# chemprop/chemprop

Hardware: AMD Instinct MI355X
Metric: million directed-edge-updates/sec (depth=3, hidden=300) (higher is better)
Workload: dtype f32 (exact 3-term f16 split of fp32 operands, fp32 accumulate); 1 GPU; qm9-shaped synthetic molecules, 512 mols/GPU/step, BondMessagePassing depth=3 hidden=300, forward (plan K0 + K1..K5); mols_per_gpu=512, directed_edges_per_gpu=9120, parallelism=dp1 (molecule shards, no data-path collective), launch=eager

## Files before the change

### chemprop_amd/_lib.py

```python
from __future__ import annotations

import ctypes as C
import os
import shutil
import subprocess
from typing import Optional

_HERE = os.path.dirname(os.path.abspath(__file__))
_ROOT = os.path.dirname(_HERE)
CSRC = os.path.join(_HERE, "csrc")
INCLUDE = os.path.join(_ROOT, "include")
LIB_PATH = os.environ.get("DMPNN_LIB") or os.path.join(_HERE, "libdmpnn_gfx950.so")
SOURCES = ["dmpnn_abi.hip", "dmpnn_prepare.hip", "dmpnn_segment.hip", "dmpnn_gemm.hip", "dmpnn_gemm_p1.hip",
           "dmpnn_gemm_p2.hip", "dmpnn_gemm_p3.hip", "dmpnn_gemm_p4.hip", "dmpnn_gemm_s1.hip", "dmpnn_mega.hip", "dmpnn_mega16.hip", "dmpnn_mega16_lp.hip", "dmpnn_mega16_bwd.hip", "dmpnn_rows16.hip", "dmpnn_step16.hip", "dmpnn_bstep16.hip", "dmpnn_backward.hip", "dmpnn_molagg.hip", "dmpnn_collate.hip", "dmpnn_tiles_large.hip", "dmpnn_optim.hip", "dmpnn_wgrad16.hip", "dmpnn_head.hip", "dmpnn_vd.hip"]
HEADERS = ["dmpnn_common.hpp", "dmpnn_spill_impl.hpp", "dmpnn_gemm_impl.hpp", "dmpnn_mega_impl.hpp", "dmpnn_mega16_impl.hpp", "dmpnn_mega16_bwd_impl.hpp", "dmpnn_rows16_impl.hpp", "dmpnn_seg16.hpp", "dmpnn_step16_impl.hpp"]
ABI_VERSION = 15
PLAN_NOFFSETS = 15

EXPORTS = [
    "dmpnn_version", "dmpnn_debug_timestamps", "dmpnn_last_error_string", "dmpnn_last_launch_count", "dmpnn_plan_bytes",
    "dmpnn_plan_layout", "dmpnn_prepare", "dmpnn_prepare_light", "dmpnn_prepare_tiles", "dmpnn_message_fwd", "dmpnn_aggregate_fwd",
    "dmpnn_linear_fwd", "dmpnn_linear16_wsplit_bytes", "dmpnn_linear16_ok", "dmpnn_linear16_fwd", "dmpnn_update_fwd", "dmpnn_forward", "dmpnn_forward_can_fuse", "dmpnn_forward_wsplit_bytes", "dmpnn_forward_keep_bits_bytes", "dmpnn_forward_spill_bytes", "dmpnn_backward_ws_bytes", "dmpnn_backward", "dmpnn_message_bwd",
    "dmpnn_aggregate_bwd", "dmpnn_linear_wgrad_ws_bytes", "dmpnn_linear_wgrad",
    "dmpnn_molagg_ws_bytes", "dmpnn_molagg_bounds", "dmpnn_molagg_fwd", "dmpnn_molagg_bwd", "dmpnn_gather_rows", "dmpnn_collate", "dmpnn_pack_tiles", "dmpnn_max_tiles",
    "dmpnn_prepare_tiles_from_table", "dmpnn_prepare_with_batch", "dmpnn_tile_plan_any_size", "dmpnn_split_row_floats", "dmpnn_forward_can_fuse16", "dmpnn_adam_step",
    "dmpnn_full_plan_keeps_tiles", "dmpnn_head_ws_bytes", "dmpnn_head", "dmpnn_train_step", "dmpnn_forward_tiles", "dmpnn_forward_route", "dmpnn_dropout_keep",
    "dmpnn_clip_grad", "dmpnn_clip_grad_ws_bytes", "dmpnn_train_route", "dmpnn_forward_h0_bytes", "dmpnn_tile_waves", "dmpnn_debug_lds_poison",
    "dmpnn_vd_ws_bytes", "dmpnn_vd_forward", "dmpnn_vd_backward",
]

ACT = {"none": 0, "relu": 1, "leakyrelu": 2, "prelu": 3, "tanh": 4, "elu": 5}
F_UNDIRECTED = 1
F_FUSED = 2
F_MEGA = 4
F_KEEP = 8
F_SPLIT16 = 16
F_WSPLIT_READY = 32
F_LOADER_TILES = 64
F_STORE16 = 128
F_ATOM = 1024
F_TILE_PLAN = 2048
F_H0_RESIDUAL = 256
F_ROW_FINALIZE = 512
ROUTES = ("general", "general16", "fused", "fused16", "mega", "mega16")
PLAN_NOMEGA_MASK = 15
PLAN_NOFUSE_MASK = 7


class GemmArgs(C.Structure):
    _fields_ = [
        ("M", C.c_int64), ("N", C.c_int64), ("K1", C.c_int64), ("K2", C.c_int64),
        ("A1", C.c_void_p), ("lda1", C.c_int64), ("gather1", C.c_void_p), ("gather1_rows", C.c_int64),
        ("A2", C.c_void_p), ("lda2", C.c_int64),
        ("W", C.c_void_p), ("ldw", C.c_int64),
        ("bias", C.c_void_p),
        ("Cadd", C.c_void_p), ("ldcadd", C.c_int64),
        ("C", C.c_void_p), ("ldc", C.c_int64),
        ("Zpre", C.c_void_p), ("ldz", C.c_int64),
        ("act", C.c_int), ("act_slope", C.c_float), ("act_slope_ptr", C.c_void_p),
    ]


class FwdArgs(C.Structure):
    _fields_ = [
        ("plan", C.c_void_p), ("n_atoms", C.c_int64), ("n_edges", C.c_int64),
        ("d_v", C.c_int64), ("d_e", C.c_int64), ("d_h", C.c_int64), ("d_vd", C.c_int64),
        ("depth", C.c_int32), ("flags", C.c_uint32),
        ("act", C.c_int32), ("act_slope", C.c_float), ("act_slope_ptr", C.c_void_p),
        ("V", C.c_void_p), ("ldv", C.c_int64),
        ("E", C.c_void_p), ("lde", C.c_int64),
        ("V_d", C.c_void_p), ("ldvd", C.c_int64),
        ("W_i", C.c_void_p), ("b_i", C.c_void_p),
        ("W_h", C.c_void_p), ("b_h", C.c_void_p),
        ("W_o", C.c_void_p), ("b_o", C.c_void_p),
        ("W_d", C.c_void_p), ("b_d", C.c_void_p),
        ("ldh", C.c_int64), ("H0", C.c_void_p), ("Hs", C.c_void_p), ("n_hslots", C.c_int32),
        ("Ms", C.c_void_p), ("n_mslots", C.c_int32),
        ("Mv", C.c_void_p), ("Hv", C.c_void_p),
        ("out", C.c_void_p), ("ldout", C.c_int64),
        ("wsplit", C.c_void_p), ("wsplit_bytes", C.c_size_t),
        ("edge_index", C.c_void_p), ("rev_edge_index", C.c_void_p),
        ("n_tiles_launch", C.c_int64),
        ("spill_ws", C.c_void_p), ("spill_bytes", C.c_size_t),
        ("msplit", C.c_void_p), ("msplit_bytes", C.c_size_t),
        ("dropout_p", C.c_float), ("dropout_seed", C.c_uint64),
        ("keep_bits", C.c_void_p), ("keep_bits_bytes", C.c_size_t),
        ("h0_bytes", C.c_size_t),
    ]


class BwdArgs(C.Structure):
    _fields_ = [
        ("f", FwdArgs), ("gout", C.c_void_p), ("ldgout", C.c_int64),
        ("gW_i", C.c_void_p), ("gb_i", C.c_void_p), ("gW_h", C.c_void_p), ("gb_h", C.c_void_p),
        ("gW_o", C.c_void_p), ("gb_o", C.c_void_p), ("gW_d", C.c_void_p), ("gb_d", C.c_void_p),
        ("ws", C.c_void_p), ("ws_bytes", C.c_size_t),
        ("g_edge", C.c_void_p), ("ld_gedge", C.c_int64),
    ]


MAX_FFN_LAYERS = 8
MAX_COMPONENTS = 8
DROP_SITE_FFN = 0x10000
LOSS = {"mse": 0, "mae": 1, "bce": 2, "ce": 3, "mve": 4, "evidential": 5, "quantile": 6}
STEP_FORWARD, STEP_BACKWARD, STEP_UPDATE = 1, 2, 4


class HeadArgs(C.Structure):
    _fields_ = [
        ("n_atoms", C.c_int64), ("n_mols", C.c_int64), ("d_h", C.c_int64),
        ("batch", C.c_void_p),
        ("agg_mode", C.c_int32), ("agg_norm", C.c_float),
        ("bn_weight", C.c_void_p), ("bn_bias", C.c_void_p), ("bn_running_mean", C.c_void_p), ("bn_running_var", C.c_void_p),
        ("bn_eps", C.c_float), ("bn_momentum", C.c_float), ("bn_training", C.c_int32),
        ("n_layers", C.c_int32), ("act", C.c_int32), ("act_slope", C.c_float),
        ("W", C.c_void_p * MAX_FFN_LAYERS), ("b", C.c_void_p * MAX_FFN_LAYERS), ("dims", C.c_int64 * (MAX_FFN_LAYERS + 1)),
        ("loss", C.c_int32),
        ("targets", C.c_void_p), ("weights", C.c_void_p), ("task_weights", C.c_void_p), ("lt_mask", C.c_void_p), ("gt_mask", C.c_void_p),
        ("preds", C.c_void_p), ("loss_out", C.c_void_p),
        ("gW", C.c_void_p * MAX_FFN_LAYERS), ("gb", C.c_void_p * MAX_FFN_LAYERS), ("g_bn_weight", C.c_void_p), ("g_bn_bias", C.c_void_p),
        ("gHv", C.c_void_p), ("ldg", C.c_int64),
        ("ws", C.c_void_p), ("ws_bytes", C.c_size_t),
        ("bn_num_batches_tracked", C.c_void_p),
        ("n_classes", C.c_int32),
        ("evid_v_kl", C.c_float), ("evid_eps", C.c_float), ("quantile_alpha", C.c_float),
        ("X_d", C.c_void_p), ("ld_xd", C.c_int64),
        ("n_components", C.c_int32),
        ("ffn_dropout_p", C.c_float), ("ffn_dropout_seed", C.c_uint64),
    ]


class TrainRouteInfo(C.Structure):
    _fields_ = [("plan_kind", C.c_int32), ("route", C.c_int32), ("keep_rows", C.c_int32), ("keep_bits", C.c_int32), ("lean", C.c_int32)]


class StepComponent(C.Structure):
    _fields_ = [
        ("edge_index", C.c_void_p), ("rev_edge_index", C.c_void_p), ("batch", C.c_void_p), ("plan_bytes", C.c_size_t), ("plan_ready", C.c_int32),
        ("bwd", BwdArgs),
    ]


class VdArgs(C.Structure):
    _fields_ = [
        ("n_atoms", C.c_int64), ("d_h", C.c_int64), ("d_vd", C.c_int64),
        ("Hv", C.c_void_p), ("ldhv", C.c_int64),
        ("V_d", C.c_void_p), ("ldvd", C.c_int64),
        ("W_d", C.c_void_p), ("b_d", C.c_void_p),
        ("out", C.c_void_p), ("ldout", C.c_int64),
        ("gout", C.c_void_p), ("ldgout", C.c_int64),
        ("gHv", C.c_void_p), ("ldghv", C.c_int64),
        ("gW_d", C.c_void_p), ("gb_d", C.c_void_p),
        ("ws", C.c_void_p), ("ws_bytes", C.c_size_t),
    ]


VD_MAX_WIDTH = 544


class StepArgs(C.Structure):
    _fields_ = [
        ("edge_index", C.c_void_p), ("rev_edge_index", C.c_void_p), ("batch", C.c_void_p), ("plan_bytes", C.c_size_t), ("plan_ready", C.c_int32),
        ("stages", C.c_int32),
        ("bwd", BwdArgs), ("head", HeadArgs),
        ("p", C.c_void_p), ("g", C.c_void_p), ("m", C.c_void_p), ("v", C.c_void_p), ("n_params", C.c_int64),
        ("lr", C.c_float), ("beta1", C.c_float), ("beta2", C.c_float), ("eps", C.c_float), ("weight_decay", C.c_float),
        ("bias_corr1", C.c_float), ("sqrt_bias_corr2", C.c_float), ("grad_scale", C.c_float), ("dev_scalars", C.c_void_p),
        ("clip_val", C.c_float), ("clip_mode", C.c_int32), ("clip_ws", C.c_void_p),
        ("n_extra", C.c_int32), ("extra", C.POINTER(StepComponent)),
        ("vd", C.POINTER(VdArgs)),
    ]


def sources() -> list[str]:
    return [os.path.join(CSRC, s) for s in SOURCES if os.path.isfile(os.path.join(CSRC, s))]


def _stale() -> bool:
    if os.environ.get("DMPNN_LIB"):
        return False
    if not os.path.isfile(LIB_PATH):
        return True
    t = os.path.getmtime(LIB_PATH)
    deps = sources() + [os.path.join(CSRC, h) for h in HEADERS] + [os.path.join(INCLUDE, "dmpnn.h")]
    return any(os.path.getmtime(d) > t for d in deps if os.path.isfile(d))


def build(force: bool = False, verbose: bool = False, defines=(), out: Optional[str] = None) -> str:
    lib_path = out or LIB_PATH
    if not force and not _stale() and out is None:
        return LIB_PATH
    hipcc = shutil.which("hipcc") or "/opt/rocm/bin/hipcc"
    if not os.path.isfile(hipcc):
        raise RuntimeError("hipcc not found: cannot build libdmpnn_gfx950.so")
    import concurrent.futures as cf
    import tempfile

    flags = ["--offload-arch=gfx950", "-O3", "-std=c++17", "-fPIC", f"-I{INCLUDE}", f"-I{CSRC}", *[f"-D{d}" for d in defines]]
    with tempfile.TemporaryDirectory(prefix="dmpnn_build_") as tmp:
        def cc(src):
            obj = os.path.join(tmp, os.path.basename(src) + ".o")
            cmd = [hipcc, *flags, "-c", src, "-o", obj]
            if verbose:
                print(" ".join(cmd))
            r = subprocess.run(cmd, capture_output=True, text=True)
            if r.returncode != 0:
                raise RuntimeError(f"hipcc failed on {src} ({r.returncode}):\n{r.stdout}\n{r.stderr}")
            return obj

        with cf.ThreadPoolExecutor(max_workers=8) as ex:
            objs = list(ex.map(cc, sources()))
        linked = os.path.join(os.path.dirname(objs[0]), "libdmpnn.so")
        cmd = [hipcc, "--offload-arch=gfx950", "-shared", "-fPIC", *objs, "-o", linked]
        if verbose:
            print(" ".join(cmd))
        r = subprocess.run(cmd, capture_output=True, text=True)
        if r.returncode != 0:
            raise RuntimeError(f"hipcc link failed ({r.returncode}):\n{r.stdout}\n{r.stderr}")
        shutil.copyfile(linked, lib_path + ".tmp")
        os.chmod(lib_path + ".tmp", 0o755)
    os.replace(lib_path + ".tmp", lib_path)
    _clean_unbundle_temporaries(lib_path)
    return lib_path


def _clean_unbundle_temporaries(lib_path: str) -> int:
    import glob

    n = 0
    for f in glob.glob(glob.escape(lib_path) + ".*"):
        tail = f[len(lib_path) + 1:]
        if tail.split(".", 1)[0].isdigit() and ("hipv4-" in tail or "host-" in tail):
            try:
                os.remove(f)
                n += 1
            except OSError:
                pass
    return n


_lib: Optional[C.CDLL] = None


def load() -> C.CDLL:
    global _lib
    if _lib is not None:
        return _lib
    import torch

    if _stale() and (shutil.which("hipcc") or os.path.isfile("/opt/rocm/bin/hipcc")):
        build()
    if not os.path.isfile(LIB_PATH):
        raise RuntimeError(
            f"{LIB_PATH} is missing: run `python -c 'import __graft_entry__ as g; g.build()'` "
            "(the MI355X engine has no CPU / eager fallback)")
    lib = C.CDLL(LIB_PATH)
    lib.dmpnn_version.restype = C.c_int
    lib.dmpnn_last_error_string.restype = C.c_char_p
    lib.dmpnn_last_launch_count.restype = C.c_int
    lib.dmpnn_plan_bytes.restype = C.c_size_t
    lib.dmpnn_plan_bytes.argtypes = [C.c_int64, C.c_int64]
    lib.dmpnn_plan_layout.argtypes = [C.c_int64, C.c_int64, C.POINTER(C.c_int64)]
    lib.dmpnn_forward_can_fuse.argtypes = [C.POINTER(FwdArgs)]
    lib.dmpnn_prepare.argtypes = [C.c_void_p, C.c_void_p, C.c_int64, C.c_int64, C.c_void_p, C.c_size_t, C.c_void_p]
    lib.dmpnn_prepare_light.argtypes = lib.dmpnn_prepare.argtypes
    lib.dmpnn_prepare_tiles.argtypes = [C.c_void_p, C.c_void_p, C.c_void_p, C.c_int64, C.c_int64, C.c_void_p, C.c_size_t, C.c_void_p]
    lib.dmpnn_message_fwd.argtypes = [C.c_void_p, C.c_int64, C.c_int64, C.c_int64, C.c_void_p, C.c_int64,
                                      C.c_void_p, C.c_int64, C.c_int, C.c_float, C.c_void_p, C.c_uint, C.c_void_p]
    lib.dmpnn_aggregate_fwd.argtypes = [C.c_void_p, C.c_int64, C.c_int64, C.c_int64, C.c_void_p, C.c_int64,
                                        C.c_void_p, C.c_int64, C.c_int, C.c_float, C.c_void_p, C.c_void_p]
    lib.dmpnn_linear_fwd.argtypes = [C.POINTER(GemmArgs), C.c_void_p]
    lib.dmpnn_update_fwd.argtypes = [C.c_void_p, C.c_int64, C.c_int64, C.c_int64, C.c_void_p, C.c_int64, C.c_void_p, C.c_int64,
                                     C.c_void_p, C.c_void_p, C.c_void_p, C.c_int64, C.c_void_p, C.c_int64, C.c_void_p,
                                     C.c_int64, C.c_int, C.c_float, C.c_void_p, C.c_void_p]
    lib.dmpnn_forward.argtypes = [C.POINTER(FwdArgs), C.c_void_p]
    lib.dmpnn_backward_ws_bytes.argtypes = [C.POINTER(FwdArgs)]
    lib.dmpnn_backward.argtypes = [C.POINTER(BwdArgs), C.c_void_p]
    lib.dmpnn_message_bwd.argtypes = [C.c_void_p, C.c_int64, C.c_int64, C.c_int64, C.c_void_p, C.c_int64,
                                      C.c_void_p, C.c_int64, C.c_void_p]
    lib.dmpnn_aggregate_bwd.argtypes = lib.dmpnn_message_bwd.argtypes
    lib.dmpnn_linear_wgrad_ws_bytes.argtypes = [C.c_int64, C.c_int64, C.c_int64, C.c_int]
    lib.dmpnn_linear_wgrad.argtypes = [C.POINTER(GemmArgs), C.c_void_p, C.c_int64, C.c_void_p, C.c_int64,
                                       C.c_void_p, C.c_void_p, C.c_size_t, C.c_void_p]
    size_t_fns = ("dmpnn_plan_bytes", "dmpnn_backward_ws_bytes", "dmpnn_linear_wgrad_ws_bytes", "dmpnn_forward_wsplit_bytes", "dmpnn_forward_spill_bytes",
                  "dmpnn_forward_keep_bits_bytes",
                  "dmpnn_molagg_ws_bytes", "dmpnn_linear16_wsplit_bytes", "dmpnn_head_ws_bytes", "dmpnn_clip_grad_ws_bytes", "dmpnn_forward_h0_bytes", "dmpnn_vd_ws_bytes")
    lib.dmpnn_linear16_wsplit_bytes.argtypes = [C.c_int64, C.c_int64]
    lib.dmpnn_linear16_ok.argtypes = [C.POINTER(GemmArgs)]
    lib.dmpnn_linear16_fwd.argtypes = [C.POINTER(GemmArgs), C.c_void_p, C.c_size_t, C.c_int, C.c_void_p]
    lib.dmpnn_gather_rows.argtypes = [C.c_void_p, C.c_int64, C.c_int64, C.c_void_p, C.c_int64, C.c_int64, C.c_void_p, C.c_int64,
                                      C.c_void_p]
    lib.dmpnn_pack_tiles.argtypes = [C.c_void_p, C.c_void_p, C.c_int64, C.c_void_p, C.c_void_p, C.c_int64]
    lib.dmpnn_pack_tiles.restype = C.c_int64
    lib.dmpnn_max_tiles.argtypes = [C.c_int64, C.c_int64]
    lib.dmpnn_prepare_with_batch.argtypes = [C.c_void_p, C.c_void_p, C.c_void_p, C.c_int64, C.c_int64, C.c_void_p, C.c_size_t, C.c_void_p]
    lib.dmpnn_prepare_with_batch.restype = C.c_int
    lib.dmpnn_tile_plan_any_size.argtypes = [C.c_int64, C.c_int64]
    lib.dmpnn_max_tiles.restype = C.c_int64
    lib.dmpnn_prepare_tiles_from_table.argtypes = [C.c_void_p, C.c_void_p, C.c_int64, C.c_int64, C.c_int64, C.c_void_p, C.c_size_t,
                                                   C.c_void_p]
    lib.dmpnn_collate.argtypes = [C.c_void_p, C.c_void_p, C.c_int64, C.c_void_p, C.c_void_p, C.c_void_p, C.c_int64, C.c_int64,
                                  C.c_void_p, C.c_void_p, C.c_void_p, C.c_void_p]
    lib.dmpnn_molagg_ws_bytes.argtypes = [C.c_int64]
    lib.dmpnn_molagg_bounds.argtypes = [C.c_void_p, C.c_int64, C.c_int64, C.c_void_p, C.c_size_t, C.c_void_p]
    lib.dmpnn_molagg_fwd.argtypes = [C.c_void_p, C.c_int64, C.c_int64, C.c_int64, C.c_int64, C.c_void_p, C.c_int, C.c_float,
                                     C.c_void_p, C.c_int64, C.c_void_p]
    lib.dmpnn_molagg_bwd.argtypes = [C.c_void_p, C.c_int64, C.c_void_p, C.c_int64, C.c_int64, C.c_int64, C.c_void_p, C.c_int,
                                     C.c_float, C.c_void_p, C.c_int64, C.c_void_p]
    lib.dmpnn_forward_wsplit_bytes.argtypes = [C.POINTER(FwdArgs)]
    lib.dmpnn_forward_keep_bits_bytes.argtypes = [C.POINTER(FwdArgs)]
    lib.dmpnn_forward_spill_bytes.argtypes = [C.POINTER(FwdArgs)]
    lib.dmpnn_forward_h0_bytes.argtypes = [C.POINTER(FwdArgs)]
    lib.dmpnn_forward_can_fuse16.argtypes = [C.POINTER(FwdArgs)]
    lib.dmpnn_adam_step.argtypes = [C.c_void_p, C.c_void_p, C.c_void_p, C.c_void_p, C.c_int64, C.c_float, C.c_float, C.c_float, C.c_float,
                                    C.c_float, C.c_float, C.c_float, C.c_float, C.c_void_p, C.c_void_p]
    lib.dmpnn_train_route.argtypes = [C.POINTER(FwdArgs), C.c_int64, C.c_int32, C.c_int32, C.c_int32, C.c_int32, C.c_int32, C.POINTER(TrainRouteInfo)]
    lib.dmpnn_clip_grad.argtypes = [C.c_void_p, C.c_int64, C.c_float, C.c_int32, C.c_float, C.c_void_p, C.c_void_p]
    lib.dmpnn_dropout_keep.argtypes = [C.c_uint64, C.c_int32, C.c_int64, C.c_int64, C.c_float]
    lib.dmpnn_forward_route.argtypes = [C.POINTER(FwdArgs), C.c_int, C.c_int, C.c_int, C.c_int]
    lib.dmpnn_tile_waves.restype = C.c_int
    lib.dmpnn_tile_waves.argtypes = [C.c_int64, C.c_int64, C.c_int64, C.c_int64]
    lib.dmpnn_forward_tiles.argtypes = [C.POINTER(FwdArgs), C.c_void_p, C.c_void_p, C.c_void_p, C.c_int64, C.c_size_t, C.c_void_p]
    lib.dmpnn_full_plan_keeps_tiles.argtypes = [C.c_int64, C.c_int64]
    lib.dmpnn_head_ws_bytes.argtypes = [C.POINTER(HeadArgs)]
    lib.dmpnn_head.argtypes = [C.POINTER(HeadArgs), C.c_void_p, C.c_int64, C.c_void_p]
    lib.dmpnn_train_step.argtypes = [C.POINTER(StepArgs), C.c_void_p]
    lib.dmpnn_vd_ws_bytes.argtypes = [C.POINTER(VdArgs)]
    lib.dmpnn_vd_forward.argtypes = [C.POINTER(VdArgs), C.c_void_p]
    lib.dmpnn_vd_backward.argtypes = [C.POINTER(VdArgs), C.c_void_p]
    lib.dmpnn_split_row_floats.argtypes = [C.c_int64]
    lib.dmpnn_split_row_floats.restype = C.c_int64
    lib.dmpnn_debug_timestamps.argtypes = [C.c_void_p]
    for name in size_t_fns:
        getattr(lib, name).restype = C.c_size_t
    for name in EXPORTS:
        if name != "dmpnn_last_error_string" and name not in size_t_fns and name not in ("dmpnn_pack_tiles", "dmpnn_max_tiles", "dmpnn_split_row_floats"):
            getattr(lib, name).restype = C.c_int
    if lib.dmpnn_version() != ABI_VERSION:
        raise RuntimeError(f"libdmpnn ABI version {lib.dmpnn_version()} != {ABI_VERSION} (stale build?)")
    _lib = lib
    return lib


_ENV_DATA = getattr(os.environ, "_data", None)
_ENV_KEYS: dict = {}


def opt(name: str, default: str) -> str:
    if _ENV_DATA is None or os.name != "posix":
        return os.environ.get(name, default)
    k = _ENV_KEYS.get(name)
    if k is None:
        k = _ENV_KEYS[name] = name.encode()
    v = _ENV_DATA.get(k)
    return default if v is None else v.decode()


class DmpnnError(RuntimeError):
    pass


def check(rc: int, what: str) -> None:
    if rc != 0:
        msg = load().dmpnn_last_error_string().decode(errors="replace")
        raise DmpnnError(f"{what} failed (code {rc}): {msg}")
```

### chemprop_amd/csrc/dmpnn_abi.hip

```cpp
#include <stdarg.h>
#include <stdlib.h>
#include <string.h>

#include "dmpnn_common.hpp"
#include "dmpnn_mega16_impl.hpp"

namespace dmpnn {

static thread_local char g_err[512] = "";
static thread_local int g_launches = 0;

void set_error(const char* fmt, ...) {
    va_list ap;
    va_start(ap, fmt);
    vsnprintf(g_err, sizeof(g_err), fmt, ap);
    va_end(ap);
}
static __global__ __launch_bounds__(1024) void k_debug_lds_poison(unsigned pat, unsigned* sink) {
    extern __shared__ unsigned lds_words[];
    constexpr int n = (160 * 1024 - 64) / 4;
    for (int i = threadIdx.x; i < n; i += 1024) lds_words[i] = pat;
    __syncthreads();
    if (sink && lds_words[(threadIdx.x * 7) % n] == 0x12345u) sink[0] = 1;
}
static int g_lds_poison = -1;
static void debug_lds_poison() {
    if (g_lds_poison < 0) {
        const char* e = getenv("DMPNN_DEBUG_LDS_POISON");
        g_lds_poison = (e && e[0] == '1') ? 1 : 0;
    }
    if (!g_lds_poison) return;
    static const bool attr = hipFuncSetAttribute(reinterpret_cast<const void*>(&k_debug_lds_poison), hipFuncAttributeMaxDynamicSharedMemorySize, 160 * 1024 - 64) == hipSuccess;
    if (!attr) return;
    hipLaunchKernelGGL(k_debug_lds_poison, dim3(768), dim3(1024), 160 * 1024 - 64, static_cast<hipStream_t>(nullptr), 0x7FC07FC0u, static_cast<unsigned*>(nullptr));
    (void)hipGetLastError();
}
void count_launch(const char* name) {
    ++g_launches;
    debug_lds_poison();
    static const bool trace = [] {
        const char* e = getenv("DMPNN_TRACE");
        return e && e[0] == '1';
    }();
    if (trace) {
        fprintf(stderr, "[dmpnn] launch %d: %s ... ", g_launches, name);
        fflush(stderr);
        const hipError_t e = hipDeviceSynchronize();
        fprintf(stderr, "%s\n", e == hipSuccess ? "ok" : hipGetErrorString(e));
        fflush(stderr);
    }
}

static int check_graph_sizes(int64_t nV, int64_t nE) {
    DMPNN_CHECK_ARG(nV >= 0 && nE >= 0, "negative graph size (n_atoms=%lld n_edges=%lld)", (long long)nV, (long long)nE);
    DMPNN_CHECK_ARG(nV < (int64_t(1) << 31) - 64 && nE < (int64_t(1) << 31) - 64,
                    "graph too large for int32 indices (n_atoms=%lld n_edges=%lld)", (long long)nV, (long long)nE);
    return DMPNN_OK;
}

}

using namespace dmpnn;
namespace dmpnn { extern thread_local long long* g_debug_stamps; }

extern "C" {

int dmpnn_version(void) { return DMPNN_ABI_VERSION; }
void dmpnn_debug_lds_poison(int on) { dmpnn::g_lds_poison = on ? 1 : 0; }
int dmpnn_dropout_keep(uint64_t seed, int32_t site, int64_t row, int64_t col, float p) {
    if (!(p > 0.f && p < 1.f)) return p <= 0.f ? 1 : 0;
    return drop_hash((unsigned)(seed & 0xFFFFFFFFull), (unsigned)(seed >> 32), (unsigned)site, (unsigned)row, (unsigned)col) >= drop_threshold(p) ? 1 : 0;
}
int dmpnn_debug_timestamps(void* device_buf) {
    g_debug_stamps = static_cast<long long*>(device_buf);
    return DMPNN_OK;
}
const char* dmpnn_last_error_string(void) { return g_err; }
int dmpnn_last_launch_count(void) { return g_launches; }

size_t dmpnn_plan_bytes(int64_t n_atoms, int64_t n_edges) {
    if (n_atoms < 0 || n_edges < 0) return 0;
    return (size_t)plan_layout(n_atoms, n_edges).words * sizeof(int);
}

int dmpnn_plan_layout(int64_t n_atoms, int64_t n_edges, int64_t off[DMPNN_PLAN_NOFFSETS]) {
    DMPNN_CHECK_ARG(off != nullptr, "plan_layout: null output");
    DMPNN_TRY(check_graph_sizes(n_atoms, n_edges));
    const PlanLayout L = plan_layout(n_atoms, n_edges);
    off[0] = L.src; off[1] = L.dst; off[2] = L.rev; off[3] = L.row_ptr; off[4] = L.perm;
    off[5] = L.inv; off[6] = L.srcp; off[7] = L.dstp; off[8] = L.revp;
    off[9] = L.tile_row; off[10] = L.tile_atom; off[11] = L.max_tiles;
    off[12] = L.mtile_row; off[13] = L.mtile_atom; off[14] = L.max_mtiles;
    return DMPNN_OK;
}

static int prepare_impl(const int64_t* edge_index, const int64_t* rev, int64_t n_atoms, int64_t n_edges, void* plan,
                        size_t plan_bytes, int light, void* stream) {
    DMPNN_TRY(check_graph_sizes(n_atoms, n_edges));
    DMPNN_CHECK_ARG(plan != nullptr, "prepare: null plan");
    DMPNN_CHECK_ARG(n_edges == 0 || (edge_index && rev), "prepare: null index arrays");
    if (plan_bytes < dmpnn_plan_bytes(n_atoms, n_edges)) {
        set_error("prepare: plan buffer too small (%zu < %zu bytes)", plan_bytes, dmpnn_plan_bytes(n_atoms, n_edges));
        return DMPNN_ENOSPC;
    }
    DMPNN_CHECK_ARG(aligned16(plan), "prepare: plan must be 16-byte aligned");
    return launch_prepare(edge_index, rev, n_atoms, n_edges, static_cast<int*>(plan), light, static_cast<hipStream_t>(stream));
}
int dmpnn_prepare(const int64_t* edge_index, const int64_t* rev, int64_t n_atoms, int64_t n_edges, void* plan,
                  size_t plan_bytes, void* stream) {
    return prepare_impl(edge_index, rev, n_atoms, n_edges, plan, plan_bytes, 0, stream);
}
int dmpnn_prepare_light(const int64_t* edge_index, const int64_t* rev, int64_t n_atoms, int64_t n_edges, void* plan,
                        size_t plan_bytes, void* stream) {
    return prepare_impl(edge_index, rev, n_atoms, n_edges, plan, plan_bytes, 1, stream);
}

int dmpnn_prepare_tiles(const int64_t* edge_index, const int64_t* rev, const int64_t* batch, int64_t n_atoms, int64_t n_edges,
                        void* plan, size_t plan_bytes, void* stream) {
    if (batch && n_atoms > 0 && small_plan_fits(n_atoms, n_edges)) {
        DMPNN_TRY(check_graph_sizes(n_atoms, n_edges));
        DMPNN_CHECK_ARG(plan != nullptr && aligned16(plan), "prepare_tiles: plan must be a 16-byte aligned buffer");
        DMPNN_CHECK_ARG(n_edges == 0 || edge_index, "prepare_tiles: null edge_index");
        if (plan_bytes < dmpnn_plan_bytes(n_atoms, n_edges)) {
            set_error("prepare_tiles: plan buffer too small (%zu < %zu bytes)", plan_bytes, dmpnn_plan_bytes(n_atoms, n_edges));
            return DMPNN_ENOSPC;
        }
        return launch_prepare_tiles_batch(edge_index, batch, n_atoms, n_edges, static_cast<int*>(plan), static_cast<hipStream_t>(stream));
    }
    if (batch && dmpnn_tile_plan_any_size(n_atoms, n_edges) && !small_plan_fits(n_atoms, n_edges)) {
        DMPNN_TRY(check_graph_sizes(n_atoms, n_edges));
        DMPNN_CHECK_ARG(plan != nullptr && aligned16(plan), "prepare_tiles: plan must be a 16-byte aligned buffer");
        DMPNN_CHECK_ARG(n_edges == 0 || edge_index, "prepare_tiles: null edge_index");
        if (plan_bytes < dmpnn_plan_bytes(n_atoms, n_edges)) {
            set_error("prepare_tiles: plan buffer too small (%zu < %zu bytes)", plan_bytes, dmpnn_plan_bytes(n_atoms, n_edges));
            return DMPNN_ENOSPC;
        }
        return launch_prepare_tiles_large(edge_index, batch, n_atoms, n_edges, static_cast<int*>(plan), static_cast<hipStream_t>(stream));
    }
    return prepare_impl(edge_index, rev, n_atoms, n_edges, plan, plan_bytes, 2, stream);
}

}
namespace dmpnn {
int prepare_tiles_and_bounds(const int64_t* edge_index, const int64_t* rev, const int64_t* batch, int64_t n_atoms, int64_t n_edges, void* plan,
                             size_t plan_bytes, int* mol_bounds, int64_t n_mols, void* stream, bool* wrote_bounds,
                             const dmpnn_fwd_args* split_for, bool* did_split) {
    if (wrote_bounds) *wrote_bounds = false;
    if (did_split) *did_split = false;
    if (mol_bounds && (n_mols <= 0 || n_mols >= (1 << 30))) mol_bounds = nullptr;
    if ((mol_bounds || split_for) && batch && n_atoms > 0 && small_plan_fits(n_atoms, n_edges) && check_graph_sizes(n_atoms, n_edges) == DMPNN_OK &&
        plan != nullptr && aligned16(plan) && (n_edges == 0 || edge_index) && plan_bytes >= dmpnn_plan_bytes(n_atoms, n_edges)) {
        DMPNN_TRY(launch_prepare_tiles_batch(edge_index, batch, n_atoms, n_edges, static_cast<int*>(plan), static_cast<hipStream_t>(stream), mol_bounds,
                                             mol_bounds ? n_mols : 0, split_for, did_split));
        if (wrote_bounds) *wrote_bounds = mol_bounds != nullptr;
        return DMPNN_OK;
    }
    return dmpnn_prepare_tiles(edge_index, rev, batch, n_atoms, n_edges, plan, plan_bytes, stream);
}
}
extern "C" {

int dmpnn_tile_plan_any_size(int64_t n_atoms, int64_t n_edges) { return tiles_large_fits(n_atoms, n_edges) ? 1 : 0; }
int dmpnn_full_plan_keeps_tiles(int64_t n_atoms, int64_t n_edges) {
    if (n_atoms <= 0 || n_edges <= 0) return 0;
    if (small_plan_fits(n_atoms, n_edges)) return 1;
    return (tiles_large_fits(n_atoms, n_edges) && prepare_can_keep_mtiles(n_atoms, n_edges)) ? 1 : 0;
}

int dmpnn_prepare_with_batch(const int64_t* edge_index, const int64_t* rev, const int64_t* batch, int64_t n_atoms, int64_t n_edges,
                             void* plan, size_t plan_bytes, void* stream) {
    if (!batch || n_atoms <= 0 || n_edges <= 0 || small_plan_fits(n_atoms, n_edges) || !tiles_large_fits(n_atoms, n_edges) ||
        !prepare_can_keep_mtiles(n_atoms, n_edges))
        return prepare_impl(edge_index, rev, n_atoms, n_edges, plan, plan_bytes, 0, stream);
    DMPNN_TRY(check_graph_sizes(n_atoms, n_edges));
    DMPNN_CHECK_ARG(plan != nullptr && aligned16(plan), "prepare_with_batch: plan must be a 16-byte aligned buffer");
    DMPNN_CHECK_ARG(edge_index && rev, "prepare_with_batch: null index arrays");
    if (plan_bytes < dmpnn_plan_bytes(n_atoms, n_edges)) {
        set_error("prepare_with_batch: plan buffer too small (%zu < %zu bytes)", plan_bytes, dmpnn_plan_bytes(n_atoms, n_edges));
        return DMPNN_ENOSPC;
    }
    DMPNN_TRY(launch_prepare_tiles_large(edge_index, batch, n_atoms, n_edges, static_cast<int*>(plan), static_cast<hipStream_t>(stream)));
    return launch_prepare(edge_index, rev, n_atoms, n_edges, static_cast<int*>(plan), 0, static_cast<hipStream_t>(stream), true);
}

int dmpnn_message_fwd(const void* plan, int64_t n_atoms, int64_t n_edges, int64_t d_h, const float* Hin,
                      int64_t ld_in, float* M, int64_t ld_m, int act_on_load, float act_slope,
                      const float* act_slope_ptr, unsigned flags, void* stream) {
    DMPNN_TRY(check_graph_sizes(n_atoms, n_edges));
    DMPNN_CHECK_ARG(plan && d_h >= 0 && ld_in >= d_h && ld_m >= d_h, "message_fwd: bad arguments");
    DMPNN_CHECK_ARG(n_edges == 0 || (Hin && M), "message_fwd: null tensor");
    DMPNN_CHECK_ARG(act_on_load != DMPNN_ACT_PRELU || act_slope_ptr, "message_fwd: PReLU needs act_slope_ptr");
    return launch_message(plan_view(plan, n_atoms, n_edges), n_atoms, n_edges, d_h, Hin, ld_in, M, ld_m,
                          act_on_load, act_slope, act_slope_ptr, flags, static_cast<hipStream_t>(stream));
}

int dmpnn_aggregate_fwd(const void* plan, int64_t n_atoms, int64_t n_edges, int64_t d_h, const float* Hin,
                        int64_t ld_in, float* Mv, int64_t ld_mv, int act_on_load, float act_slope,
                        const float* act_slope_ptr, void* stream) {
    DMPNN_TRY(check_graph_sizes(n_atoms, n_edges));
    DMPNN_CHECK_ARG(plan && d_h >= 0 && ld_in >= d_h && ld_mv >= d_h, "aggregate_fwd: bad arguments");
    DMPNN_CHECK_ARG(n_atoms == 0 || Mv, "aggregate_fwd: null output");
    DMPNN_CHECK_ARG(n_edges == 0 || Hin, "aggregate_fwd: null input");
    DMPNN_CHECK_ARG(act_on_load != DMPNN_ACT_PRELU || act_slope_ptr, "aggregate_fwd: PReLU needs act_slope_ptr");
    return launch_aggregate(plan_view(plan, n_atoms, n_edges), n_atoms, n_edges, d_h, Hin, ld_in, Mv, ld_mv,
                            act_on_load, act_slope, act_slope_ptr, static_cast<hipStream_t>(stream));
}

int dmpnn_linear_fwd(const dmpnn_gemm_args* a, void* stream) {
    DMPNN_CHECK_ARG(a != nullptr, "linear_fwd: null args");
    DMPNN_CHECK_ARG(a->act != DMPNN_ACT_PRELU || a->act_slope_ptr, "linear_fwd: PReLU needs act_slope_ptr");
    if (a->M > 0 && a->N > 0 && a->K1 >= 0 && a->K2 >= 0) DMPNN_TRY(check_linear_lds(*a, "linear_fwd"));
    return launch_linear(*a, static_cast<hipStream_t>(stream));
}

int dmpnn_update_fwd(const void* plan, int64_t n_atoms, int64_t n_edges, int64_t d_h, const float* M, int64_t ld_m,
                     const float* H0, int64_t ld_h0, const float* W_h, const float* b_h, float* H_out, int64_t ld_hout,
                     float* M_next, int64_t ld_mnext, float* Mv, int64_t ld_mv, int act, float act_slope,
                     const float* act_slope_ptr, void* stream) {
    DMPNN_TRY(check_graph_sizes(n_atoms, n_edges));
    DMPNN_CHECK_ARG(plan && d_h > 0, "update_fwd: bad arguments");
    DMPNN_CHECK_ARG(n_edges == 0 || (M && H0 && W_h), "update_fwd: null tensor");
    DMPNN_CHECK_ARG(M_next || Mv || H_out, "update_fwd: no output");
    DMPNN_CHECK_ARG(act != DMPNN_ACT_PRELU || act_slope_ptr, "update_fwd: PReLU needs act_slope_ptr");
    DMPNN_CHECK_ARG(d_h % 4 == 0 && d_h <= 320, "update_fwd: d_h must be a multiple of 4 and <= 320 (got %lld)", (long long)d_h);
    {
        const struct { const void* p; int64_t ld; const char* name; } t[] = {
            {M, ld_m, "M"}, {H0, ld_h0, "H0"}, {H_out, ld_hout, "H_out"}, {M_next, ld_mnext, "M_next"}, {Mv, ld_mv, "Mv"}};
        for (const auto& x : t)
            DMPNN_CHECK_ARG(!x.p || (x.ld >= d_h && x.ld % 4 == 0 && aligned16(x.p)),
                            "update_fwd: %s must be 16-byte aligned with a leading dimension >= d_h that is a multiple of 4 (ld %lld)", x.name,
                            (long long)x.ld);
// ... 2 lines not shown
    if (n_edges == 0) {
        if (Mv && n_atoms > 0) {
            for (int64_t v = 0; v < n_atoms; ++v)
                if (hipMemsetAsync(Mv + v * ld_mv, 0, (size_t)d_h * sizeof(float), static_cast<hipStream_t>(stream)) != hipSuccess) {
                    set_error("update_fwd: memset failed");
                    return DMPNN_EHIP;
                }
        }
        return DMPNN_OK;
    }
    const int* plan_i = static_cast<const int*>(plan);
    const PlanLayout L = plan_layout(n_atoms, n_edges);
    dmpnn_gemm_args g;
    memset(&g, 0, sizeof(g));
    g.M = n_edges; g.N = d_h; g.K1 = d_h;
    g.A1 = M; g.lda1 = ld_m;
    g.W = W_h; g.ldw = d_h; g.bias = b_h;
    g.Cadd = H0; g.ldcadd = ld_h0;
    g.C = H_out; g.ldc = ld_hout;
    g.act = act; g.act_slope = act_slope; g.act_slope_ptr = act_slope_ptr;
    GemmExtra x;
    memset(&x, 0, sizeof(x));
    x.seg = true;
    x.tile_row = plan_i + L.tile_row; x.tile_atom = plan_i + L.tile_atom; x.n_tiles = (int)L.max_tiles;
    x.row_ptr = plan_i + L.row_ptr; x.revp = plan_i + L.revp;
    x.Mout = M_next; x.ldm = ld_mnext; x.Sout = Mv; x.lds = ld_mv;
    return launch_linear_ex(g, x, static_cast<hipStream_t>(stream));
}

static size_t steps16_wsplit_bytes(const dmpnn_fwd_args& a) {
    const int64_t h = a.d_h;
    size_t n = linear16_wsplit_bytes(h, a.d_v + a.d_e) + linear16_wsplit_bytes(h, h) + linear16_wsplit_bytes(h, a.d_v + h);
    n += linear16_wsplit_bytes(h + a.d_vd, h + a.d_vd) * ((a.W_d && a.d_vd > 0) ? 1 : 0);
    n += linear16_wsplit_bytes(h, h) + linear16_wsplit_bytes(h, a.d_v);
    return n;
}

size_t dmpnn_forward_wsplit_bytes(const dmpnn_fwd_args* a) {
    if (!a || a->d_h <= 0 || a->d_v <= 0 || a->d_e < 0) return 0;
    return (a->flags & DMPNN_F_MEGA) ? mega16_wsplit_bytes(*a) : steps16_wsplit_bytes(*a);
}

static bool keep_bits_apply(const dmpnn_fwd_args& a) {
    const unsigned need = DMPNN_F_TILE_PLAN | DMPNN_F_KEEP | DMPNN_F_MEGA | DMPNN_F_SPLIT16 | DMPNN_F_FUSED;
    return (a.flags & need) == need && (a.act == DMPNN_ACT_NONE || a.act == DMPNN_ACT_RELU || a.act == DMPNN_ACT_LEAKYRELU) &&
           !(a.dropout_p > 0.f) && !a.W_d && a.n_atoms > 0 && a.n_edges > 0;
}
size_t dmpnn_forward_keep_bits_bytes(const dmpnn_fwd_args* a) {
    if (!a) return 0;
    if ((a->flags & (DMPNN_F_FUSED | DMPNN_F_SPLIT16)) == (DMPNN_F_FUSED | DMPNN_F_SPLIT16) && !(a->flags & DMPNN_F_MEGA)) return fused16_lean_bits_bytes(*a);
    if (!keep_bits_apply(*a)) return 0;
    return (size_t)a->depth * (size_t)plan_layout(a->n_atoms, a->n_edges).max_mtiles * 256u * 8u;
}

size_t dmpnn_forward_h0_bytes(const dmpnn_fwd_args* a) { return a ? fused16_h0q_bytes(*a) : 0; }

size_t dmpnn_forward_spill_bytes(const dmpnn_fwd_args* a) {
    if (!a || a->n_atoms < 0 || a->n_edges < 0 || a->ldh <= 0) return 0;
    return (size_t)(3 * a->n_edges + a->n_atoms) * (size_t)a->ldh * sizeof(float);
}

static bool al_ptr(const void* p, int bytes) { return (reinterpret_cast<uintptr_t>(p) & (uintptr_t)(bytes - 1)) == 0; }

int dmpnn_forward_can_fuse(const dmpnn_fwd_args* a) {
    if (!a) return 0;
    const int64_t h = a->d_h, dv = a->d_v, de = a->d_e;
    if (a->flags & DMPNN_F_UNDIRECTED) return 0;
    if (h <= 0 || h % 4 != 0 || h > 320 || a->ldh % 4 != 0) return 0;
    if (dv % 2 != 0 || de % 2 != 0 || a->ldv % 2 != 0 || a->lde % 2 != 0) return 0;
    if (!al_ptr(a->V, 8) || !al_ptr(a->E, 8) || !al_ptr(a->W_i, 8) || !al_ptr(a->W_h, 16)) return 0;
    if (!al_ptr(a->H0, 16) || !al_ptr(a->Ms, 16) || !al_ptr(a->Mv, 16) || (a->Hs && !al_ptr(a->Hs, 16))) return 0;
    if (a->n_atoms * a->ldv * 4 > 0x7FFFFFFF || a->n_edges * a->lde * 4 > 0x7FFFFFFF) return 0;
    return mega_shapes_ok(*a) ? 2 : 1;
}

static const int64_t kSteps16MinEdges = 20000, kFused16MinEdges = 2048;

int dmpnn_tile_waves(int64_t n_atoms, int64_t n_edges, int64_t d_h, int64_t n_tiles) {
    dmpnn_fwd_args t;
    memset(&t, 0, sizeof(t));
    t.n_atoms = n_atoms; t.n_edges = n_edges; t.d_h = d_h;
    return tile_waves(t, n_tiles > 0 ? (int)n_tiles : (int)plan_layout(n_atoms, n_edges).max_mtiles);
}

int dmpnn_forward_route(const dmpnn_fwd_args* a, int keep, int max_level, int plan_kind, int arith) {
    if (!a || max_level < 0 || plan_kind < 0 || plan_kind > 2 || arith < 0 || arith > 1) return -1;
    const bool undirected = (a->flags & DMPNN_F_UNDIRECTED) != 0;
    int level = undirected ? 0 : dmpnn_forward_can_fuse(a);
    if (level > max_level) level = max_level;
    if (plan_kind == 2) return (level == 2 && arith == 0 && !(keep && a->W_d)) ? DMPNN_ROUTE_MEGA16 : -1;
    if (plan_kind == 1 && keep) return -1;
    const int64_t nE = a->n_edges, h = a->d_h;
    if (!keep && !undirected && arith == 0 && nE >= kFused16MinEdges && (level == 1 || (level == 0 && h > 320 && max_level >= 1))) {
        dmpnn_fwd_args t = *a;
        t.flags &= ~(unsigned)(DMPNN_F_KEEP | DMPNN_F_STORE16);
        if (fused16_shapes_ok(t)) return DMPNN_ROUTE_FUSED16;
    }
    if (keep && level == 1 && arith == 0 && nE >= kSteps16MinEdges && plan_kind == 0) {
        dmpnn_fwd_args t = *a;
        t.flags = (t.flags | DMPNN_F_FUSED | DMPNN_F_SPLIT16) & ~(unsigned)(DMPNN_F_MEGA | DMPNN_F_STORE16);
        if (fused16_lean_shapes(t)) return DMPNN_ROUTE_FUSED16;
    }
    if (level == 1 && arith == 0 && nE >= kSteps16MinEdges && plan_kind != 1) level = 0;
    if (level == 2) return arith == 0 ? DMPNN_ROUTE_MEGA16 : DMPNN_ROUTE_MEGA;
    if (level == 1) return DMPNN_ROUTE_FUSED;
    if (plan_kind == 1) return -1;
    return (arith == 0 && (h > 320 || nE >= kSteps16MinEdges)) ? DMPNN_ROUTE_GENERAL16 : DMPNN_ROUTE_GENERAL;
}

int dmpnn_train_route(const dmpnn_fwd_args* a, int64_t n_mols, int32_t have, int32_t oversize, int32_t max_level, int32_t arith,
                      int32_t keep_rows, dmpnn_train_route_info* out) {
    DMPNN_CHECK_ARG(a && out && max_level >= 0 && (arith == 0 || arith == 1) && keep_rows >= -1 && keep_rows <= 1, "train_route: bad arguments");
    memset(out, 0, sizeof(*out));
    const int64_t nV = a->n_atoms, nE = a->n_edges, h = a->d_h;
    const bool undirected = (a->flags & DMPNN_F_UNDIRECTED) != 0, atom = (a->flags & DMPNN_F_ATOM) != 0;
    const bool relu_class = a->act == DMPNN_ACT_RELU || a->act == DMPNN_ACT_LEAKYRELU;
    const bool builtin = a->act == DMPNN_ACT_NONE || relu_class || a->act == DMPNN_ACT_TANH || a->act == DMPNN_ACT_ELU;
    bool tiles = !undirected && !a->W_d && builtin && max_level >= 2 && arith == 0 && nE > 0 && nV > 0 && oversize != 1;
    if (a->dropout_p > 0.f && !relu_class) tiles = false;
    if (!(h > 0 && h % 4 == 0 && h <= 320 && a->d_v % 2 == 0 && a->d_e % 2 == 0)) tiles = false;
    if (atom && !(a->d_e >= 2 && a->d_e <= 16) ) tiles = false;
    const bool small = small_plan_fits(nV, nE), table = (have & 2) != 0, large = (have & 1) != 0 && tiles_large_fits(nV, nE);
    if (!(small || table || large)) tiles = false;
    if (!(n_mols > 0 && nE <= 30 * n_mols && (table || large || small))) tiles = false;
    out->plan_kind = tiles ? 2 : 0;
    int cap = max_level;
    if (oversize == 1 && cap > 1) cap = 1;
    dmpnn_fwd_args t = *a;
    if (table || large) t.flags |= DMPNN_F_LOADER_TILES;
    out->route = dmpnn_forward_route(&t, 1, cap, out->plan_kind, arith);
    if (out->route < 0 && out->plan_kind == 2) {
        out->plan_kind = 0;
        out->route = dmpnn_forward_route(&t, 1, cap, 0, arith);
    }
    const int64_t n_steps = a->depth > 1 ? a->depth - 1 : 0;
    const bool rows = keep_rows == 1 || (keep_rows < 0 && nE * n_steps >= DMPNN_KEEP_ROWS_MIN);
    out->keep_rows = (!atom && n_steps > 0 && h > 0 && h <= 320 && rows) ? 1 : 0;
    if (out->route == DMPNN_ROUTE_MEGA16) {
        out->keep_bits = (out->plan_kind == 2 && (relu_class || a->act == DMPNN_ACT_NONE) && !(a->dropout_p > 0.f)) ? 1 : 0;
    } else if (out->route == DMPNN_ROUTE_FUSED16) {
        dmpnn_fwd_args l = *a;
        l.flags = (l.flags | DMPNN_F_FUSED | DMPNN_F_SPLIT16) & ~(unsigned)(DMPNN_F_MEGA | DMPNN_F_STORE16);
        out->lean = fused16_lean_shapes(l) ? 1 : 0;
        out->keep_bits = out->lean;
    }
    return DMPNN_OK;
}

int dmpnn_forward_tiles(const dmpnn_fwd_args* a, const int64_t* batch, const int* tile_row, const int* tile_atom, int64_t n_tiles,
                        size_t plan_bytes, void* stream) {
    DMPNN_CHECK_ARG(a != nullptr && a->plan != nullptr, "forward_tiles: null args / plan");
    void* plan = const_cast<void*>(a->plan);
    bool did_split = false;
    if (tile_row && tile_atom && n_tiles > 0) {
        const dmpnn::PlanLayout L = dmpnn::plan_layout(a->n_atoms, a->n_edges);
        const bool ok = a->n_atoms >= 0 && a->n_edges >= 0 && a->n_atoms < (1ll << 31) && a->n_edges < (1ll << 31) &&
                        plan_bytes >= (size_t)L.words * sizeof(int) && n_tiles <= L.max_mtiles;
        if (ok) DMPNN_TRY(launch_tiles_from_table_split(tile_row, tile_atom, n_tiles, a->n_atoms, a->n_edges, static_cast<int*>(plan),
                                                        static_cast<hipStream_t>(stream), a, &did_split));
        if (!did_split)
            DMPNN_TRY(dmpnn_prepare_tiles_from_table(tile_row, tile_atom, n_tiles, a->n_atoms, a->n_edges, plan, plan_bytes, stream));
    } else
        DMPNN_TRY(prepare_tiles_and_bounds(a->edge_index, a->rev_edge_index, batch, a->n_atoms, a->n_edges, plan, plan_bytes, nullptr, 0, stream, nullptr, a, &did_split));
    if (!did_split) return dmpnn_forward(a, stream);
    dmpnn_fwd_args f = *a;
    f.flags |= DMPNN_F_WSPLIT_READY;
    return dmpnn_forward(&f, stream);
}

int dmpnn_forward(const dmpnn_fwd_args* a, void* stream) {
    g_launches = 0;
    DMPNN_CHECK_ARG(a != nullptr, "forward: null args");
    DMPNN_TRY(check_graph_sizes(a->n_atoms, a->n_edges));
    const int64_t nV = a->n_atoms, nE = a->n_edges, h = a->d_h, dv = a->d_v, de = a->d_e;
    DMPNN_CHECK_ARG(a->plan, "forward: null plan");
    DMPNN_CHECK_ARG(h > 0 && dv > 0 && de >= 0 && a->d_vd >= 0 && a->depth >= 1, "forward: bad dimensions");
    DMPNN_CHECK_ARG(a->act >= DMPNN_ACT_RELU && a->act <= DMPNN_ACT_ELU,
                    "forward: activation %d is not built in (chain the row kernels instead)", a->act);
    DMPNN_CHECK_ARG(a->act != DMPNN_ACT_PRELU || a->act_slope_ptr, "forward: PReLU needs act_slope_ptr");
    DMPNN_CHECK_ARG(a->W_i && a->W_h && a->W_o && a->b_o, "forward: null weight");
    DMPNN_CHECK_ARG(a->ldh >= h && a->ldv >= dv && a->lde >= de, "forward: leading dimension too small");
    DMPNN_CHECK_ARG(nV == 0 || (a->V && a->Mv && a->out), "forward: null V / Mv / out");
    DMPNN_CHECK_ARG(nE == 0 || (a->E && (a->H0 || (a->flags & DMPNN_F_MEGA))), "forward: null E / H0");
    const bool has_vd = a->W_d != nullptr;
    DMPNN_CHECK_ARG(!has_vd || (a->d_vd > 0 && a->V_d && a->b_d && a->Hv && a->ldvd >= a->d_vd),
                    "forward: W_d given but V_d / b_d / Hv / d_vd missing");
    DMPNN_CHECK_ARG(a->ldout >= h + (has_vd ? a->d_vd : 0), "forward: ldout too small");
    const bool fused = a->flags & DMPNN_F_FUSED;
    DMPNN_CHECK_ARG(!(a->flags & DMPNN_F_STORE16) || (fused && (a->flags & DMPNN_F_SPLIT16) && !(a->flags & (DMPNN_F_KEEP | DMPNN_F_ATOM))),
                    "forward: DMPNN_F_STORE16 only goes with the fused routes on the f16 pipe (DMPNN_F_FUSED | DMPNN_F_SPLIT16 [| DMPNN_F_MEGA]), inference, bond messages");
    const bool lean16 = fused && (a->flags & DMPNN_F_SPLIT16) && (a->flags & DMPNN_F_KEEP) && !(a->flags & DMPNN_F_MEGA) && a->keep_bits;
    if (a->depth > 1 && nE > 0 && !(a->flags & DMPNN_F_MEGA) && !lean16) {
        DMPNN_CHECK_ARG(a->Ms && a->n_mslots >= 1, "forward: missing Ms workspace");
        DMPNN_CHECK_ARG(fused || (a->Hs && a->n_hslots >= 1), "forward: missing Hs workspace");
    }

    if (a->flags & DMPNN_F_ATOM) {
        DMPNN_CHECK_ARG((a->flags & DMPNN_F_FUSED) && (a->flags & DMPNN_F_MEGA) && (a->flags & DMPNN_F_SPLIT16) &&
                        !has_vd && de >= 1 && de <= 16 && a->dropout_p == 0.f,
                        "forward: DMPNN_F_ATOM (atom messages) runs on the whole-forward tile kernel only (DMPNN_F_FUSED | DMPNN_F_MEGA | "
                        "DMPNN_F_SPLIT16, 1 <= d_e <= 16, no W_d, no dropout inside the kernels) — chain the row kernels otherwise");
        DMPNN_CHECK_ARG(!(a->flags & DMPNN_F_KEEP) || (de % 2 == 0 && dv % 2 == 0 && h % 2 == 0 &&
                        (a->depth < 2 || nE == 0 || (a->msplit && aligned16(a->msplit) && a->msplit_bytes >= (size_t)(a->depth - 1) * (size_t)nE * 16 * sizeof(float)))),
                        "forward: DMPNN_F_ATOM | DMPNN_F_KEEP needs even d_v / d_e / d_h and `msplit` >= (depth - 1) * n_edges * 64 bytes, 16-byte aligned");
    }
    if (a->dropout_p != 0.f) {
        DMPNN_CHECK_ARG(a->dropout_p > 0.f && a->dropout_p < 1.f, "forward: dropout_p must lie in [0, 1)");
        const bool tile_train = (a->flags & DMPNN_F_MEGA) && (a->flags & DMPNN_F_SPLIT16) && (a->flags & DMPNN_F_KEEP);
        DMPNN_CHECK_ARG(tile_train && !has_vd && (a->act == DMPNN_ACT_RELU || a->act == DMPNN_ACT_LEAKYRELU),
                        "forward: dropout inside the kernels needs the training forward of the tile kernel (DMPNN_F_MEGA | DMPNN_F_SPLIT16 | "
                        "DMPNN_F_KEEP), a ReLU-class activation and no W_d — run dropout between the row kernels otherwise");
    }
    hipStream_t s = static_cast<hipStream_t>(stream);
    const PlanView pv = plan_view(a->plan, nV, nE);
    const int64_t slot = nE * a->ldh;
    const int* plan_i = static_cast<const int*>(a->plan);

    if (fused && (a->flags & DMPNN_F_SPLIT16) && !(a->flags & DMPNN_F_MEGA)) {
        DMPNN_CHECK_ARG(fused16_shapes_ok(*a), "forward: DMPNN_F_FUSED | DMPNN_F_SPLIT16 given but the shapes do not allow it "
                        "(directed, d_h %% 4 == 0, d_h <= 640, even d_v / d_e; with DMPNN_F_KEEP: depth - 1 kept H / M slots and `msplit`)");
        DMPNN_CHECK_ARG(nE == 0 || (a->H0 && ((a->flags & DMPNN_F_KEEP) ? (a->Ms || a->depth == 1 || lean16) : (a->Ms && a->n_mslots >= 2))),
                        "forward(fused16): H0 and two split message slots (training: `msplit` + the kept fp32 slots) are required");
        DMPNN_CHECK_ARG(a->wsplit && a->wsplit_bytes >= steps16_wsplit_bytes(*a), "forward(fused16): wsplit workspace missing or too small");
        SplitWView w[6];
        unsigned char* wp = static_cast<unsigned char*>(a->wsplit);
        const bool ready = (a->flags & DMPNN_F_WSPLIT_READY) != 0;
        const float* Ws[6] = {a->W_i, a->W_h, a->W_o, has_vd ? a->W_d : nullptr, a->W_o + dv, a->W_o};
        const int64_t Ns[6] = {h, h, h, h + a->d_vd, h, h}, Ks[6] = {dv + de, h, dv + h, h + a->d_vd, h, dv};
        const int64_t Ls[6] = {dv + de, h, dv + h, h + a->d_vd, dv + h, dv + h};
        SplitWJob jobs[6];
        SplitWView views[6];
        int idx[6], nj = 0;
        for (int i = 0; i < 6; ++i) {
            if (!Ws[i]) continue;
            if (ready) w[i] = split_weights_view_of(wp, Ns[i], Ks[i]);
            else { jobs[nj] = SplitWJob{Ws[i], Ls[i], Ns[i], Ks[i], 0, wp}; idx[nj++] = i; }
            wp += linear16_wsplit_bytes(Ns[i], Ks[i]);
        }
        mega16::SplitArgs sp;
        const bool pend = nj > 0 && split_weights_args(jobs, nj, views, &sp);
        for (int k = 0; k < nj; ++k) w[idx[k]] = views[k];
        DMPNN_TRY(launch_fused16_forward(*a, w, has_vd ? a->Hv : a->out, has_vd ? a->ldh : a->ldout, s, pend ? &sp : nullptr));
        if (has_vd) {
            dmpnn_gemm_args g;
            memset(&g, 0, sizeof(g));
            g.M = nV; g.N = h + a->d_vd; g.K1 = h; g.K2 = a->d_vd;
            g.A1 = a->Hv; g.lda1 = a->ldh;
            g.A2 = a->V_d; g.lda2 = a->ldvd;
            g.W = a->W_d; g.ldw = h + a->d_vd; g.bias = a->b_d;
            g.C = a->out; g.ldc = a->ldout; g.act = DMPNN_ACT_NONE;
            if (linear16_ok(g)) DMPNN_TRY(launch_linear16_view(g, w[3], nullptr, 0, s));
            else DMPNN_TRY(launch_linear(g, s));
        }
        return DMPNN_OK;
    }
    if (fused) {
        DMPNN_CHECK_ARG(dmpnn_forward_can_fuse(a), "forward: DMPNN_F_FUSED given but the shapes / alignment do not allow it "
                        "(d_h %% 4, d_h <= 320, even d_v / d_e, directed); call dmpnn_forward_can_fuse first");
        const PlanLayout L = plan_layout(nV, nE);
        DMPNN_CHECK_ARG((a->flags & DMPNN_F_MEGA) || a->depth <= 2 || a->n_mslots >= 2,
                        "forward(fused): depth > 2 needs at least two message slots");
        if (a->flags & DMPNN_F_MEGA) {
            DMPNN_CHECK_ARG(mega_shapes_ok(*a), "forward: DMPNN_F_MEGA given but the shapes do not allow it");
            DMPNN_CHECK_ARG(!a->keep_bits || (keep_bits_apply(*a) && aligned16(a->keep_bits) && a->keep_bits_bytes >= dmpnn_forward_keep_bits_bytes(a)),
                            "forward: keep_bits needs DMPNN_F_TILE_PLAN | DMPNN_F_KEEP on the tile kernel (f16 pipe), a ReLU-class activation, no "
                            "dropout, no W_d, and dmpnn_forward_keep_bits_bytes() bytes");
            DMPNN_CHECK_ARG(!(a->flags & DMPNN_F_KEEP) || a->depth == 1 || nE == 0 ||
                            (a->Hs && a->n_hslots >= a->depth - 1 && a->n_mslots >= a->depth - 1),
                            "forward(mega, keep): needs depth-1 H and M slots");
            if (nV > 0) {
                if (a->flags & DMPNN_F_SPLIT16) DMPNN_TRY(launch_mega16_forward(*a, has_vd ? a->Hv : a->out, has_vd ? a->ldh : a->ldout, s));
                else DMPNN_TRY(launch_mega_forward(*a, has_vd ? a->Hv : a->out, has_vd ? a->ldh : a->ldout, s));
            }
            if (has_vd) {
                dmpnn_gemm_args g;
                memset(&g, 0, sizeof(g));
                g.M = nV; g.N = h + a->d_vd; g.K1 = h; g.K2 = a->d_vd;
                g.A1 = a->Hv; g.lda1 = a->ldh;
                g.A2 = a->V_d; g.lda2 = a->ldvd;
                g.W = a->W_d; g.ldw = h + a->d_vd; g.bias = a->b_d;
                g.C = a->out; g.ldc = a->ldout; g.act = DMPNN_ACT_NONE;
                DMPNN_TRY(launch_linear(g, s));
            }
            return DMPNN_OK;
        }
        GemmExtra x;
        memset(&x, 0, sizeof(x));
        x.seg = true;
        x.tile_row = plan_i + L.tile_row; x.tile_atom = plan_i + L.tile_atom; x.n_tiles = nE > 0 ? (int)L.max_tiles : 0;
        x.row_ptr = plan_i + L.row_ptr; x.revp = plan_i + L.revp;
        const int T = a->depth;
        if (nE == 0 && nV > 0) {
            hipError_t e = hipMemsetAsync(a->Mv, 0, (size_t)nV * a->ldh * sizeof(float), s);
            if (e != hipSuccess) { set_error("forward: memset failed: %s", hipGetErrorString(e)); return DMPNN_EHIP; }
        }
        if (nE > 0) {
            dmpnn_gemm_args g;
            memset(&g, 0, sizeof(g));
            g.M = nE; g.N = h; g.K1 = dv; g.K2 = de;
            g.A1 = a->V; g.lda1 = a->ldv; g.gather1 = plan_i + L.srcp; g.gather1_rows = nV;
            g.A2 = a->E; g.lda2 = a->lde;
            g.W = a->W_i; g.ldw = dv + de; g.bias = a->b_i;
            g.Zpre = a->H0; g.ldz = a->ldh;
            g.act = a->act; g.act_slope = a->act_slope; g.act_slope_ptr = a->act_slope_ptr;
            GemmExtra xi = x;
            xi.gather2 = plan_i + L.perm; xi.gather2_rows = nE;
            if (T > 1) { xi.Mout = a->Ms; xi.ldm = a->ldh; }
            else { xi.Sout = a->Mv; xi.lds = a->ldh; }
            DMPNN_TRY(launch_linear_ex(g, xi, s));
            for (int t = 1; t < T; ++t) {
                memset(&g, 0, sizeof(g));
                g.M = nE; g.N = h; g.K1 = h;
                g.A1 = a->Ms + ((t - 1) % a->n_mslots) * slot; g.lda1 = a->ldh;
                g.W = a->W_h; g.ldw = h; g.bias = a->b_h;
                g.Cadd = a->H0; g.ldcadd = a->ldh;
                g.C = a->Hs ? a->Hs + ((t - 1) % a->n_hslots) * slot : nullptr; g.ldc = a->ldh;
                g.act = a->act; g.act_slope = a->act_slope; g.act_slope_ptr = a->act_slope_ptr;
                GemmExtra xu = x;
                if (t < T - 1) { xu.Mout = a->Ms + (t % a->n_mslots) * slot; xu.ldm = a->ldh; }
                else { xu.Sout = a->Mv; xu.lds = a->ldh; }
// ... 111 lines not shown
```

### chemprop_amd/csrc/dmpnn_mega16.hip

```cpp
#include <algorithm>
#include <cstdlib>

#include "dmpnn_mega16_impl.hpp"

namespace dmpnn {
namespace mega16 {
DMPNN_DEFINE_MEGA16(1, true, true)
DMPNN_DEFINE_MEGA16(1, true, false)
DMPNN_DEFINE_MEGA16(1, false, true)
DMPNN_DEFINE_MEGA16(1, false, false)
DMPNN_DEFINE_MEGA16(2, true, true)
DMPNN_DEFINE_MEGA16(2, true, false)
DMPNN_DEFINE_MEGA16(2, false, true)
DMPNN_DEFINE_MEGA16(2, false, false)
DMPNN_DEFINE_MEGA16(5, true, true)
DMPNN_DEFINE_MEGA16(5, true, false)
DMPNN_DEFINE_MEGA16(5, false, true)
DMPNN_DEFINE_MEGA16(5, false, false)
DMPNN_DEFINE_MEGA16_NW(5, true, true, 8)
DMPNN_DEFINE_MEGA16_NW(5, true, false, 8)
DMPNN_DEFINE_MEGA16_NW(5, false, true, 8)
DMPNN_DEFINE_MEGA16_NW(5, false, false, 8)
#define DMPNN_DECLARE_MEGA16_LP(WN, SA, NW) template <> int launch_mega16<WN, SA, false, NW, true>(const Mega16K& g, int n_tiles, hipStream_t s);
DMPNN_DECLARE_MEGA16_LP(1, true, 4) DMPNN_DECLARE_MEGA16_LP(1, false, 4) DMPNN_DECLARE_MEGA16_LP(2, true, 4) DMPNN_DECLARE_MEGA16_LP(2, false, 4)
DMPNN_DECLARE_MEGA16_LP(5, true, 4) DMPNN_DECLARE_MEGA16_LP(5, false, 4) DMPNN_DECLARE_MEGA16_LP(5, true, 8) DMPNN_DECLARE_MEGA16_LP(5, false, 8)
#undef DMPNN_DECLARE_MEGA16_LP
}

thread_local long long* g_debug_stamps = nullptr;
thread_local AggRide g_agg_ride = {nullptr, 0, nullptr, nullptr, 0, 0, 0.f, false};

namespace {
inline size_t al256(size_t x) { return (x + 255) & ~size_t(255); }
struct WsLayout {
    size_t wi, wh, wom, wov, sc_i, sc_h, sc_o, whe, sc_e, total;
    int nc_i, nc_h, nc_v;
};
WsLayout ws_layout(const dmpnn_fwd_args& a) {
    WsLayout L;
    const size_t N = (size_t)a.d_h;
    const bool atom = (a.flags & DMPNN_F_ATOM) != 0;
    L.nc_i = (int)((a.d_v + (atom ? 0 : a.d_e) + 31) / 32); L.nc_h = (int)((a.d_h + 31) / 32); L.nc_v = (int)((a.d_v + 31) / 32);
    size_t o = 0;
    const size_t NT = (N + 15) / 16;
    L.wi = o; o += al256(NT * L.nc_i * 2048);
    L.wh = o; o += al256(NT * L.nc_h * 2048);
    L.wom = o; o += al256(NT * L.nc_h * 2048);
    L.wov = o; o += al256(NT * L.nc_v * 2048);
    L.sc_i = o; o += al256(N * 4);
    L.sc_h = o; o += al256(N * 4);
    L.sc_o = o; o += al256(N * 4);
    L.whe = o; o += atom ? al256(NT * 1 * 2048) : 0;
    L.sc_e = o; o += atom ? al256(N * 4) : 0;
    L.total = o;
    return L;
}
}

size_t mega16_wsplit_bytes(const dmpnn_fwd_args& a) {
    return ws_layout(a).total + ((a.flags & DMPNN_F_KEEP) ? mega16_bwd_wsplit_bytes(a.d_h) : 0);
}
size_t mega16_fwd_wsplit_bytes(const dmpnn_fwd_args& a) { return ws_layout(a).total; }

bool mega16_split_args(const dmpnn_fwd_args& a, mega16::SplitArgs* spp) {
    const WsLayout W = ws_layout(a);
    if (!a.wsplit || a.wsplit_bytes < W.total) return false;
    unsigned char* ws = static_cast<unsigned char*>(a.wsplit);
    const int N = (int)a.d_h, dv = (int)a.d_v, de = (int)a.d_e;
    mega16::SplitArgs& sp = *spp;
    memset(&sp, 0, sizeof(sp));
    sp.N = N; sp.n_jobs = 4;
    const bool atom = (a.flags & DMPNN_F_ATOM) != 0;
    const int ki = atom ? dv : dv + de, ldwh = atom ? N + de : N;
    sp.job[0] = mega16::SplitJob{a.W_i, ki, 0, ki, 0, ki, ws + W.wi, W.nc_i, reinterpret_cast<float*>(ws + W.sc_i)};
    sp.job[1] = mega16::SplitJob{a.W_h, ldwh, 0, N, 0, N, ws + W.wh, W.nc_h, reinterpret_cast<float*>(ws + W.sc_h)};
    sp.job[2] = mega16::SplitJob{a.W_o, dv + N, dv, N, 0, dv + N, ws + W.wom, W.nc_h, reinterpret_cast<float*>(ws + W.sc_o)};
    sp.job[3] = mega16::SplitJob{a.W_o, dv + N, 0, dv, 0, dv + N, ws + W.wov, W.nc_v, nullptr};
    if ((a.flags & DMPNN_F_KEEP) && a.wsplit_bytes >= W.total + mega16_bwd_wsplit_bytes(N)) {
        const size_t NT = (size_t)(N + 15) / 16, nch = (size_t)(N + 31) / 32;
        const size_t one = al256(NT * nch * 2048) + al256((size_t)N * 4);
        unsigned char* wb = ws + W.total;
        sp.job[4] = mega16::SplitJob{a.W_o + dv, dv + N, 0, N, 0, N, wb, (int)nch, reinterpret_cast<float*>(wb + al256(NT * nch * 2048)), 1};
        sp.job[5] = mega16::SplitJob{a.W_h, ldwh, 0, N, 0, N, wb + one, (int)nch, reinterpret_cast<float*>(wb + one + al256(NT * nch * 2048)), 1};
        sp.n_jobs = 6;
    }
    if (atom) {
        sp.job[sp.n_jobs] = mega16::SplitJob{a.W_h, ldwh, N, de, N, de, ws + W.whe, 1, reinterpret_cast<float*>(ws + W.sc_e)};
        ++sp.n_jobs;
    }
    return true;
}

bool mega16_keeps_rows(const dmpnn_fwd_args& a) {
    const unsigned need = DMPNN_F_FUSED | DMPNN_F_MEGA | DMPNN_F_SPLIT16 | DMPNN_F_KEEP;
    if ((a.flags & need) != need || (a.flags & DMPNN_F_ATOM) || a.depth < 2 || a.n_edges <= 0 || a.d_h > 320) return false;
    const size_t bytes = (size_t)(a.depth - 1) * (size_t)a.n_edges * (size_t)(split_row_floats(a.d_h) * 4);
    return a.msplit && aligned16(a.msplit) && a.msplit_bytes >= bytes;
}

int tile_waves(const dmpnn_fwd_args& a, int n_tiles) {
    static const int forced = [] { const char* e = getenv("DMPNN_TILE_WAVES"); return e ? atoi(e) : 0; }();
    if (forced == 4 || forced == 8) return forced;
    if (a.d_h <= 128 || a.d_h > 320) return 4;
    static const int n_cu = [] {
        int dev = 0, n = 0;
        if (hipGetDevice(&dev) != hipSuccess || hipDeviceGetAttribute(&n, hipDeviceAttributeMultiprocessorCount, dev) != hipSuccess || n <= 0) n = 256;
        return n;
    }();
    if (n_tiles <= n_cu) return 8;
    const int64_t est = std::max<int64_t>((a.n_edges + 39) / 40, (a.n_atoms + 19) / 20);
    return est + est / 16 <= n_cu ? 8 : 4;
}

int launch_mega16_forward(const dmpnn_fwd_args& a, float* out, int64_t ldout, hipStream_t s) {
    const int64_t nV = a.n_atoms, nE = a.n_edges;
    const WsLayout W = ws_layout(a);
    if (!a.wsplit || a.wsplit_bytes < W.total) {
        set_error("forward(split16): wsplit workspace missing or too small (%zu < %zu bytes)", a.wsplit_bytes, W.total);
        return DMPNN_ENOSPC;
    }
    unsigned char* ws = static_cast<unsigned char*>(a.wsplit);
    const int N = (int)a.d_h, dv = (int)a.d_v, de = (int)a.d_e;
    if (!(a.flags & DMPNN_F_WSPLIT_READY)) {
        mega16::SplitArgs sp;
        if (!mega16_split_args(a, &sp)) { set_error("forward(split16): wsplit workspace missing or too small"); return DMPNN_ENOSPC; }
        hipLaunchKernelGGL(mega16::k_split_weights, dim3((unsigned)(((N + 15) / 16) * 4 * sp.n_jobs)), dim3(256), 0, s, sp);
        DMPNN_CHECK_LAUNCH("k_split_weights");
    }

    const PlanLayout L = plan_layout(nV, nE);
    const int* plan_i = static_cast<const int*>(a.plan);
    mega16::Mega16K G;
    memset(&G, 0, sizeof(G));
    mega::MegaK& g = G.m;
    g.mtile_row = plan_i + L.mtile_row; g.mtile_atom = plan_i + L.mtile_atom; g.row_ptr = plan_i + L.row_ptr;
    g.srcp = plan_i + L.srcp; g.perm = plan_i + L.perm; g.revp = plan_i + L.revp;
    g.flags = plan_i + DMPNN_HDR_FLAGS; g.poison_mask = kPlanNoMega;
    g.nV = (int)nV; g.nE = (int)nE; g.d_v = dv; g.d_e = (a.flags & DMPNN_F_ATOM) ? 0 : de; g.h = N; g.depth = a.depth;
    g.V = a.V; g.ldv = (int)a.ldv; g.E = a.E ? a.E : a.V; g.lde = (int)a.lde;
    g.v_bytes = (unsigned)(nV * a.ldv * 4); g.e_bytes = a.E ? (unsigned)(nE * a.lde * 4) : 0u;
    g.W_i = a.W_i; g.b_i = a.b_i; g.W_h = a.W_h; g.b_h = a.b_h; g.W_o = a.W_o; g.b_o = a.b_o;
    g.act = a.act; g.slope = a.act_slope; g.slope_ptr = a.act_slope_ptr;
    g.out = out; g.ldout = (int)ldout;
    g.ldh = (int)a.ldh; g.slot = (long long)nE * a.ldh;
    if (a.flags & DMPNN_F_KEEP) { g.H0 = a.H0; g.Hs = a.Hs; g.Ms = a.Ms; g.Mv = a.Mv; }
    if ((a.flags & DMPNN_F_KEEP) && a.keep_bits) {
        G.keep_bits = static_cast<unsigned long long*>(a.keep_bits);
        G.bits_slot = (long long)L.max_mtiles * 256;
    }
    g.spill = (a.spill_ws && a.spill_bytes >= dmpnn_forward_spill_bytes(&a) && aligned16(a.spill_ws)) ? a.spill_ws : nullptr;
    G.Wi = mega16::SplitW{ws + W.wi, reinterpret_cast<const float*>(ws + W.sc_i), W.nc_i};
    G.Wh = mega16::SplitW{ws + W.wh, reinterpret_cast<const float*>(ws + W.sc_h), W.nc_h};
    G.WoM = mega16::SplitW{ws + W.wom, reinterpret_cast<const float*>(ws + W.sc_o), W.nc_h};
    G.WoV = mega16::SplitW{ws + W.wov, reinterpret_cast<const float*>(ws + W.sc_o), W.nc_v};
    if (a.flags & DMPNN_F_ATOM) {
        G.WhE = mega16::SplitW{ws + W.whe, reinterpret_cast<const float*>(ws + W.sc_e), 1};
        G.atom_de = de;
        if ((a.flags & DMPNN_F_KEEP) && a.depth > 1 && nE > 0) {
            G.atom_me = static_cast<float*>(a.msplit);
            G.me_slot = (long long)nE * mega16::kAtomK;
        }
    }
    if (mega16_keeps_rows(a)) {
        G.Mrows = static_cast<unsigned char*>(a.msplit);
        G.tsr = (int)(split_row_floats(a.d_h) * 4);
        G.mrow_slot = (long long)nE * G.tsr;
    }
    g.dbg = g_debug_stamps;
    if ((a.flags & DMPNN_F_KEEP) && g_agg_ride.Hm && g_agg_ride.n_mols > 0 && out == a.out && N % 4 == 0) {
        G.agg_Hm = g_agg_ride.Hm; G.agg_ld = g_agg_ride.ld; G.agg_batch = reinterpret_cast<const long long*>(g_agg_ride.batch);
        G.agg_bounds = g_agg_ride.table; G.agg_done = g_agg_ride.table + 2 * g_agg_ride.n_mols + 4; G.agg_n_mols = g_agg_ride.n_mols;
        G.agg_mode = g_agg_ride.mode; G.agg_norm = g_agg_ride.norm;
        g_agg_ride.taken = true;
    }
    if (a.dropout_p > 0.f && a.dropout_p < 1.f) {
        g.drop_thr = drop_threshold(a.dropout_p); g.drop_scale = 1.f / (1.f - a.dropout_p);
        g.seed_lo = (unsigned)(a.dropout_seed & 0xFFFFFFFFull); g.seed_hi = (unsigned)(a.dropout_seed >> 32);
    }
    g.edge_index = reinterpret_cast<const long long*>(a.edge_index);
    g.rev64 = reinterpret_cast<const long long*>(a.rev_edge_index);
    const int n_tiles = (a.n_tiles_launch > 0 && a.n_tiles_launch < L.max_mtiles) ? (int)a.n_tiles_launch : (int)L.max_mtiles;
    const bool sa = !(a.act == DMPNN_ACT_TANH || a.act == DMPNN_ACT_ELU), kp = (a.flags & DMPNN_F_KEEP) != 0;
    const int wn = a.d_h <= 64 ? 1 : (a.d_h <= 128 ? 2 : 5);
    if (a.flags & DMPNN_F_STORE16) {
        if (wn == 1) return sa ? mega16::launch_mega16<1, true, false, 4, true>(G, n_tiles, s) : mega16::launch_mega16<1, false, false, 4, true>(G, n_tiles, s);
        if (wn == 2) return sa ? mega16::launch_mega16<2, true, false, 4, true>(G, n_tiles, s) : mega16::launch_mega16<2, false, false, 4, true>(G, n_tiles, s);
        if (tile_waves(a, n_tiles) == 8)
            return sa ? mega16::launch_mega16<5, true, false, 8, true>(G, n_tiles, s) : mega16::launch_mega16<5, false, false, 8, true>(G, n_tiles, s);
        return sa ? mega16::launch_mega16<5, true, false, 4, true>(G, n_tiles, s) : mega16::launch_mega16<5, false, false, 4, true>(G, n_tiles, s);
    }
#define DMPNN_PICK(WN) (sa ? (kp ? mega16::launch_mega16<WN, true, true>(G, n_tiles, s) : mega16::launch_mega16<WN, true, false>(G, n_tiles, s)) \
                           : (kp ? mega16::launch_mega16<WN, false, true>(G, n_tiles, s) : mega16::launch_mega16<WN, false, false>(G, n_tiles, s)))
    if (wn == 1) return DMPNN_PICK(1);
    if (wn == 2) return DMPNN_PICK(2);
    if (tile_waves(a, n_tiles) == 8)
        return sa ? (kp ? mega16::launch_mega16<5, true, true, 8>(G, n_tiles, s) : mega16::launch_mega16<5, true, false, 8>(G, n_tiles, s))
                  : (kp ? mega16::launch_mega16<5, false, true, 8>(G, n_tiles, s) : mega16::launch_mega16<5, false, false, 8>(G, n_tiles, s));
    return DMPNN_PICK(5);
#undef DMPNN_PICK
}

}
```

### chemprop_amd/csrc/dmpnn_mega16_impl.hpp

```cpp
#pragma once

#include <type_traits>

#include "dmpnn_mega_impl.hpp"

namespace dmpnn {
namespace mega16 {

using gemm::BK;
using gemm::f32x4;
using gemm::kOOB;
using gemm::kThreads;
using gemm::rsrc_t;
using gemm::u32x4;
using gemm::u32x2;
using mega::RT_A;
using mega::RT_E;

typedef _Float16 h8 __attribute__((ext_vector_type(8)));
typedef _Float16 h4 __attribute__((ext_vector_type(4)));
typedef _Float16 h2 __attribute__((ext_vector_type(2)));


struct SplitW {
    const unsigned char* p;
    const float* inv_scale;
    int nc;
};

struct Mega16K {
    mega::MegaK m;
    SplitW Wi, Wh, WoM, WoV;
    SplitW WhE; int atom_de;
    float* atom_me; long long me_slot;
    unsigned char* Mrows; int tsr; long long mrow_slot;
    unsigned long long* keep_bits; long long bits_slot;
    float* agg_Hm; int agg_ld; const long long* agg_batch; const int* agg_bounds; int* agg_done; int agg_n_mols; int agg_mode; float agg_norm;
};

template <int I, int N, class F>
__device__ __forceinline__ void static_for(F&& f) {
    if constexpr (I < N) {
        f(std::integral_constant<int, I>{});
        static_for<I + 1, N>(f);
    }
}

__device__ __forceinline__ float scale_for(float maxabs) {
    if (!(maxabs > 0.f) || !(maxabs < 3.0e38f)) return 1.f;
    int e;
    frexpf(maxabs, &e);
    const int k = 14 - e;
    return ldexpf(1.f, k > 126 ? 126 : (k < -126 ? -126 : k));
}
__device__ __forceinline__ void store_keep4(float* p, float4 v) {
#if defined(DMPNN_NT_KEEP)
    __builtin_nontemporal_store(f32x4{v.x, v.y, v.z, v.w}, reinterpret_cast<f32x4*>(p));
#else
    *reinterpret_cast<float4*>(p) = v;
#endif
}
__device__ __forceinline__ void split2(float x0, float x1, float s, unsigned& hi, unsigned& lo) {
    const float a = x0 * s, b = x1 * s;
    const h2 h = h2{(_Float16)a, (_Float16)b};
    const h2 l = h2{(_Float16)(a - (float)h[0]), (_Float16)(b - (float)h[1])};
    hi = __builtin_bit_cast(unsigned, h); lo = __builtin_bit_cast(unsigned, l);
}
__device__ __forceinline__ void split4(float4 x, float s, h4& hi, h4& lo) {
    unsigned h0, l0, h1, l1;
    split2(x.x, x.y, s, h0, l0);
    split2(x.z, x.w, s, h1, l1);
    hi = __builtin_bit_cast(h4, u32x2{h0, h1});
    lo = __builtin_bit_cast(h4, u32x2{l0, l1});
}
__device__ __forceinline__ float rcp_pow2_exact(float s) { return __uint_as_float(0x7F000000u - __float_as_uint(s)); }

struct SplitJob {
    const float* W; int ldw; int col0; int K;
    int scale_col0, scale_K;
    unsigned char* out; int nc; float* inv_scale;
    int tr;
    int N;
};
struct SplitArgs {
    SplitJob job[8];
    int n_jobs, N;
};
__device__ __forceinline__ void split_weights_wave(const SplitArgs& a, int wave, int lane) {
    const int Np = (a.N + 15) & ~15;
    const int j = wave / Np, n = wave - j * Np;
    if (j >= a.n_jobs) return;
    const SplitJob& J = a.job[j];
    const int NJ = J.N > 0 ? J.N : a.N;
    if (n >= ((NJ + 15) & ~15)) return;
    const bool live = n < NJ;
    const long long rs = J.tr ? 1 : J.ldw, ks = J.tr ? J.ldw : 1;
    const float* row = J.W + (long long)(live ? n : 0) * rs;
    float mx = 0.f;
    for (int k = lane; k < J.scale_K; k += 64) mx = fmaxf(mx, fabsf(row[(J.scale_col0 + k) * ks]));
    for (int off = 32; off > 0; off >>= 1) mx = fmaxf(mx, __shfl_xor(mx, off));
    const float s = live ? scale_for(mx) : 0.f;
    if (lane == 0 && J.inv_scale && live) J.inv_scale[n] = 1.f / s;
    _Float16* out = reinterpret_cast<_Float16*>(J.out);
    const int T = n >> 4, li = n & 15;
    for (int k = lane; k < J.nc * 32; k += 64) {
        const float x = (k < J.K && live) ? row[(J.col0 + k) * ks] * s : 0.f;
        const _Float16 hi = (_Float16)x;
        const _Float16 lo = (_Float16)(x - (float)hi);
        const int c = k >> 5, kk = k & 31, lg = kk >> 3, j = kk & 7;
        const long long base = (((long long)T * J.nc + c) * 2) * 512 + (lg * 16 + li) * 8 + j;
        out[base] = hi;
        out[base + 512] = lo;
    }
}
static __global__ __launch_bounds__(256) void k_split_weights(SplitArgs a) {
    split_weights_wave(a, blockIdx.x * 4 + (threadIdx.x >> 6), threadIdx.x & 63);
}

__device__ __forceinline__ void rows_to_sr(const float* src, long long ld, long long row0, int nrows, int N, unsigned char* dst, int ts,
                                           int wave, int lane, int n_waves) {
    for (int r = wave; r < nrows; r += n_waves) {
        const float* x = src + (row0 + r) * ld;
        float v[8];
        float mx = 0.f;
#pragma unroll
        for (int j = 0; j < 8; ++j) {
            const int c = lane + 64 * j;
            v[j] = c < N ? x[c] : 0.f;
            mx = fmaxf(mx, fabsf(v[j]));
        }
        for (int off = 32; off > 0; off >>= 1) mx = fmaxf(mx, __shfl_xor(mx, off));
        const float sc = scale_for(mx);
        unsigned char* o = dst + (row0 + r) * ts;
#pragma unroll
        for (int j = 0; j < 8; ++j) {
            const int c = lane + 64 * j;
            if (c < N) {
                const float y = v[j] * sc;
                const _Float16 hi = (_Float16)y;
                *reinterpret_cast<_Float16*>(o + (c >> 5) * 128 + (c & 31) * 2) = hi;
                *reinterpret_cast<_Float16*>(o + (c >> 5) * 128 + 64 + (c & 31) * 2) = (_Float16)(y - (float)hi);
            }
        }
        if (lane == 0) *reinterpret_cast<float4*>(o + (ts - 16)) = make_float4(sc, mx > 0.f ? 0.f : 1.f, 0.f, 0.f);
    }
}

#if !defined(DMPNN_TILE8_BRING)
#define DMPNN_TILE8_BRING 1
#endif
template <int WN>
constexpr size_t tile_region_bytes() {
    constexpr size_t ts = 64 * WN * 4 + 16, tsg = 4 * 128 + 16;
    return (size_t)kMegaBM * (ts > tsg ? ts : tsg);
}
constexpr int kAtomK = 16;
constexpr size_t kAtomLds = (size_t)(kMegaBM + kMegaBA) * kAtomK * sizeof(float);
template <int WN>
constexpr size_t lds_bytes() {
    return tile_region_bytes<WN>() + (size_t)(3 * kMegaBM + kMegaBA + 24) * sizeof(int) + 10 * 64 * 16;
}
template <int WN>
constexpr size_t lds_bytes_atom() { return lds_bytes<WN>() + kAtomLds; }

template <int WN, bool SA, bool KEEP, int NW = 4, bool LP = false>
__global__ __launch_bounds__(64 * NW, 2) void k_mpnn_tile16(Mega16K G) {
    static_assert(!(LP && KEEP), "the hi-halves-alone form is inference only");
    static_assert(NW == 4 || (NW == 8 && WN == 5), "the 8-wave form splits 20 column tiles 3+3+3+3+2+2+2+2");
    const mega::MegaK& g = G.m;
    constexpr int KT = 64 * NW;
    constexpr int JR = 16 / NW;
    constexpr int BM = kMegaBM, BA = kMegaBA, BN = 64 * WN, LDC = BN + 4, QN = BN / 4;
    constexpr int TS = BN * 4 + 16;
    constexpr int ITEMS = (BM * QN + KT - 1) / KT;
    extern __shared__ __attribute__((aligned(16))) unsigned char lds[];
    unsigned char* T16 = lds;
    static_assert(LDC * 4 == TS, "the fp32 tile and the split A tile have the same footprint");
    constexpr int META_OFF = (int)tile_region_bytes<WN>();
    float* T = reinterpret_cast<float*>(lds);
    int* revl = reinterpret_cast<int*>(lds + META_OFF);
    int* aor = revl + BM;
    int* asrc = aor + BM;
    int* rp = asrc + BM;
    unsigned* maxbits = reinterpret_cast<unsigned*>(rp + BA + 1);
    h8* cfrag = reinterpret_cast<h8*>(lds + META_OFF + (((3 * BM + BA + 1 + 8) * 4 + 15) / 16) * 16);

    using T_ = std::true_type;
    using F_ = std::false_type;
    int tid = threadIdx.x, lane = tid & 63, wave = tid >> 6;
    int li = lane & 15, lg = lane >> 4;
    int kq = tid & 7;
    auto launder = [&]() {
        asm volatile("" : "+v"(tid));
        lane = tid & 63; wave = tid >> 6; li = lane & 15; lg = lane >> 4; kq = tid & 7;
    };
#if !defined(DMPNN_NO_KERNARG_WARM)
    warm_kernargs<(int)sizeof(Mega16K)>();
#endif
    int n_stamp = 0;
    auto stamp = [&]() {
        if (g.dbg && blockIdx.x == 0 && threadIdx.x == 0 && n_stamp < 32) g.dbg[n_stamp] = (long long)__builtin_readcyclecounter();
        ++n_stamp;
    };
    stamp();
    const int t = blockIdx.x;
    int rs = g.mtile_row[t], re = g.mtile_row[t + 1];
    int va = g.mtile_atom[t], vb = g.mtile_atom[t + 1];
    int hdr_light = g.flags[DMPNN_HDR_LIGHT], hdr_flags = g.flags[0], hdr_tiles = g.flags[DMPNN_HDR_NMTILES];
    asm volatile("" : "+v"(rs), "+v"(re), "+v"(va), "+v"(vb), "+v"(hdr_light), "+v"(hdr_flags), "+v"(hdr_tiles));
    rs = __builtin_amdgcn_readfirstlane(rs); re = __builtin_amdgcn_readfirstlane(re);
    va = __builtin_amdgcn_readfirstlane(va); vb = __builtin_amdgcn_readfirstlane(vb);
    hdr_light = __builtin_amdgcn_readfirstlane(hdr_light); hdr_flags = __builtin_amdgcn_readfirstlane(hdr_flags);
    hdr_tiles = __builtin_amdgcn_readfirstlane(hdr_tiles);
    const int nrows = re - rs, na = vb - va;
    const int N = g.h, qn = N >> 2;
    const bool lean = hdr_light == 2;
    const bool poison = (hdr_flags & (lean ? kPlanNoMegaLean : g.poison_mask)) != 0 || (lean && g.nE > 0 && (!g.edge_index || !g.rev64)) ||
                        hdr_tiles > (int)gridDim.x;
    if (poison) {
        const float nanv = __int_as_float(0x7fc00000);
        const long long total = (long long)g.nV * N;
        for (long long i = (long long)blockIdx.x * KT + tid; i < total; i += (long long)gridDim.x * KT)
            g.out[(i / N) * g.ldout + (i % N)] = nanv;
        return;
    }
    if (na <= 0 || nrows < 0 || va < 0 || vb > g.nV || rs < 0 || re > g.nE) return;
    if (nrows > BM || na > BA) {
        if (NW > 4 && threadIdx.x >= kThreads) return;
        const mega::MegaK& gs = spill::fresh_kernargs<Mega16K>()->m;
        if ((KEEP && gs.drop_thr) || G.atom_de) {
            const float nanv = __int_as_float(0x7fc00000);
            for (int i = tid; i < na * N; i += kThreads) gs.out[(long long)(va + i / N) * gs.ldout + (i % N)] = nanv;
            if constexpr (KEEP) {
                if (gs.Hs)
                    for (int i = tid; i < nrows * N; i += kThreads)
                        for (int sl = 0; sl < gs.depth - 1; ++sl) gs.Hs[(long long)sl * gs.slot + (long long)(rs + i / N) * gs.ldh + (i % N)] = nanv;
            }
            return;
        }
        spill::forward(mega::spill_view(gs, gs.flags[DMPNN_HDR_LIGHT] == 2, rs, nrows, va, na, gs.slope_ptr ? *gs.slope_ptr : gs.slope),
                       reinterpret_cast<float*>(lds));
        if constexpr (KEEP) {
            const Mega16K& Gs = *spill::fresh_kernargs<Mega16K>();
            if (Gs.Mrows && gs.Ms) {
                __threadfence_block();
                __syncthreads();
                for (int sl = 0; sl < gs.depth - 1; ++sl)
                    rows_to_sr(gs.Ms + (long long)sl * gs.slot, gs.ldh, rs, nrows, gs.h, Gs.Mrows + (long long)sl * Gs.mrow_slot, Gs.tsr,
                               (int)(threadIdx.x >> 6), (int)(threadIdx.x & 63), kThreads / 64);
            }
        }
        return;
    }
    const float slope = g.slope_ptr ? *g.slope_ptr : g.slope;
    const float neg_slope = g.act == DMPNN_ACT_NONE ? 1.f : (g.act == DMPNN_ACT_RELU ? 0.f : slope);
    constexpr bool simple_act = SA;

    int revl_v = 0, rp_v = 0, aor_v = 0, asrc_v = 0;
    bool row_bad = false;
    unsigned ro1[JR * RT_E], ro2[JR * RT_E];
    {
        int i1[JR * RT_E], i2[JR * RT_E];
        if (lean && nrows > 0) {
            const int e = rs + (tid < nrows ? tid : 0);
            const long long es = g.edge_index[e], ed = g.edge_index[(long long)g.nE + e], er = g.rev64[e];
            const long long r_l = er - rs, d_l = ed - va, s_l = es - va;
            row_bad = tid < nrows && (r_l < 0 || r_l >= nrows || d_l < 0 || d_l >= na || s_l < 0 || s_l >= na);
            revl_v = (tid < nrows && !row_bad) ? (int)r_l : 0;
            aor_v = (tid < nrows && !row_bad) ? (int)d_l : 0;
            asrc_v = (tid < nrows && !row_bad) ? (int)s_l : 0;
#pragma unroll
            for (int j = 0; j < JR * RT_E; ++j) {
                const int r = wave + NW * j;
                const long long sj = g.edge_index[r < nrows ? rs + r : rs];
                i1[j] = (sj >= 0 && sj < g.nV) ? (int)sj : 0;
                i2[j] = rs + r;
            }
        } else if (lean) {
#pragma unroll
            for (int j = 0; j < JR * RT_E; ++j) { i1[j] = 0; i2[j] = 0; }
        } else {
            revl_v = tid < nrows ? g.revp[rs + tid] - rs : 0;
            rp_v = g.row_ptr[va + (tid <= na ? tid : na)] - rs;
#pragma unroll
            for (int j = 0; j < JR * RT_E; ++j) {
                const int r = wave + NW * j;
                i1[j] = g.srcp[r < nrows ? rs + r : 0];
                i2[j] = g.perm[r < nrows ? rs + r : 0];
            }
        }
#pragma unroll
        for (int j = 0; j < JR * RT_E; ++j) {
            const bool ok = wave + NW * j < nrows;
            ro1[j] = ok ? (unsigned)i1[j] * (unsigned)g.ldv * 4u : kOOB;
            ro2[j] = ok ? (unsigned)i2[j] * (unsigned)g.lde * 4u : kOOB;
        }
    }
    const rsrc_t rVg = gemm::make_rsrc(g.V, g.v_bytes), rEg = gemm::make_rsrc(g.E, g.e_bytes);
    u32x2 a_grp[JR * RT_E];
    {
        const int k = lane * 2;
        const unsigned k1o = k < g.d_v ? (unsigned)k * 4u : kOOB;
        const unsigned k2o = (k >= g.d_v && k < g.d_v + g.d_e) ? (unsigned)(k - g.d_v) * 4u : kOOB;
#pragma unroll
        for (int j = 0; j < JR * RT_E; ++j)
            a_grp[j] = __builtin_amdgcn_raw_buffer_load_b64(rVg, gemm::join_off(ro1[j], k1o), 0, 0) |
                       __builtin_amdgcn_raw_buffer_load_b64(rEg, gemm::join_off(ro2[j], k2o), 0, 0);
    }
    unsigned pf_word[4] = {0u, 0u, 0u, 0u};
#if defined(DMPNN_META_STAMPS)
    stamp();
#endif
    if (tid < BM) { revl[tid] = revl_v; asrc[tid] = asrc_v; if (lean) aor[tid] = aor_v; }
    if (tid <= BA) rp[tid] = rp_v;
    if (tid < 8) maxbits[tid] = 0u;
    __syncthreads();
#if defined(DMPNN_META_STAMPS)
    stamp();
#endif
    if (row_bad) atomicOr(&maxbits[5], 1u);
    if (!lean && tid < na)
        for (int r = rp[tid]; r < rp[tid + 1]; ++r) aor[r] = tid;
    __syncthreads();
#if defined(DMPNN_META_STAMPS)
    stamp();
#endif
    int ar[12];
    {
        const int4 q0 = *reinterpret_cast<const int4*>(aor + lg * 4), q1 = *reinterpret_cast<const int4*>(aor + 16 + lg * 4),
                   q2 = *reinterpret_cast<const int4*>(aor + 32 + lg * 4);
        const int qa[12] = {q0.x, q0.y, q0.z, q0.w, q1.x, q1.y, q1.z, q1.w, q2.x, q2.y, q2.z, q2.w};
#pragma unroll
        for (int i = 0; i < 12; ++i) ar[i] = ((i >> 2) * 16 + lg * 4 + (i & 3)) < nrows ? qa[i] : -2;
    }
    for (int f = wave; f < 10; f += NW) {
        const bool agg = f >= 6;
        const int ff = agg ? f - 6 : f, jt = ff >> 1, ks = ff & 1;
        const int j = jt * 16 + li;
        int a_t = -1, rv = -1;
        if (agg) {
            a_t = j < na ? j : -1;
        } else if (j < nrows) {
            rv = revl[j];
            a_t = lean ? asrc[j] : aor[rv];
        }
        if (G.atom_de) rv = -1;
        unsigned hb[8];
#pragma unroll
        for (int sl = 0; sl < 8; ++sl) {
            const int row = ks == 0 ? (sl < 4 ? lg * 4 + sl : 16 + lg * 4 + (sl - 4)) : (sl < 4 ? 32 + lg * 4 + sl : -2);
            const int av = ks == 0 ? ar[sl] : (sl < 4 ? ar[8 + sl] : -2);
            const bool in = av == a_t, isrev = row == rv;
            hb[sl] = in ? (isrev ? 0u : 0x3C00u) : (isrev ? 0xBC00u : 0u);
        }
        const u32x4 pk = {hb[0] | (hb[1] << 16), hb[2] | (hb[3] << 16), hb[4] | (hb[5] << 16), hb[6] | (hb[7] << 16)};
        cfrag[f * 64 + lane] = __builtin_bit_cast(h8, pk);
    }
    __syncthreads();

    auto wave_max = [&](float v) -> float {
        int u = (int)__float_as_uint(v);
        u = max(u, __builtin_amdgcn_update_dpp(0, u, 0xB1, 0xf, 0xf, true));
        u = max(u, __builtin_amdgcn_update_dpp(0, u, 0x4E, 0xf, 0xf, true));
        u = max(u, __builtin_amdgcn_update_dpp(0, u, 0x141, 0xf, 0xf, true));
        u = max(u, __builtin_amdgcn_update_dpp(0, u, 0x140, 0xf, 0xf, true));
        const int m = max(max(__builtin_amdgcn_readlane(u, 0), __builtin_amdgcn_readlane(u, 16)),
                          max(__builtin_amdgcn_readlane(u, 32), __builtin_amdgcn_readlane(u, 48)));
        return __uint_as_float((unsigned)m);
    };
    int scale_phase = 0;
    float tile_mx = 0.f;
    auto tile_scale = [&](float local_max) -> float {
        const int slot = scale_phase & 3;
        local_max = wave_max(local_max);
        if (lane == 0) atomicMax(&maxbits[slot], __float_as_uint(local_max));
        __syncthreads();
        const float mx = __uint_as_float(maxbits[slot]);
        tile_mx = mx;
// ... 288 lines not shown
    };
    auto store_bits = [&](auto rt_c, const f32x4 (&y)[decltype(rt_c)::value][WL], int slot) {
        constexpr int RT = decltype(rt_c)::value;
        static_assert(RT * WL * 4 <= 64, "one word per lane");
        unsigned lo = 0u, hi = 0u;
        static_for<0, RT * WL * 4>([&](auto ic) {
            constexpr int idx = decltype(ic)::value, r = idx & 3, ct = (idx >> 2) % WL, rt = (idx >> 2) / WL;
            const unsigned long long b = __ballot(y[rt][ct][r] > 0.f);
            unsigned l = lo, h = hi;
            const unsigned bl = (unsigned)b, bh = (unsigned)(b >> 32);
            asm volatile("s_nop 4\n\tv_writelane_b32 %0, %1, %2" : "+v"(l) : "s"(bl), "n"(idx));
            asm volatile("v_writelane_b32 %0, %1, %2" : "+v"(h) : "s"(bh), "n"(idx));
            lo = l; hi = h;
        });
        launder();
        if (lane < RT * WL * 4) {
            const int q = lane >> 2, gct = ct0() + q % WL, rt_ = q / WL;
            const int word = NW == 4 ? wave * 64 + lane : (gct / WN) * 64 + (rt_ * WN + gct % WN) * 4 + (lane & 3);
            G.keep_bits[(long long)slot * G.bits_slot + (long long)t * 256 + word] = ((unsigned long long)hi << 32) | lo;
        }
    };
    auto tile_to_global = [&](float* dst, long long row0, int ld, int n_r) {
        launder();
#pragma unroll
        for (int j = 0; j < ITEMS; ++j) {
            const int it = tid + KT * j;
            const int r = it / QN, q = it - r * QN;
            if (r < n_r && q < qn)
                store_keep4(dst + (row0 + r) * ld + 4 * q, *reinterpret_cast<const float4*>(T + r * LDC + 4 * q));
        }
    };
    static_assert(RT_E == 3 && RT_A == 2, "segment MFMAs are laid out for 48-row / 32-atom tiles");
    auto segment_mfma = [&](const f32x4 (&H)[RT_E][WL], bool last, float* keep, int keep_ld, unsigned char* keep_rows) -> float {
        launder();
        float hm = 0.f;
#pragma unroll
        for (int rt = 0; rt < RT_E; ++rt)
#pragma unroll
            for (int ct = 0; ct < WL; ++ct)
#pragma unroll
                for (int r = 0; r < 4; ++r) hm = fmaxf(hm, fabsf(H[rt][ct][r]));
        const float sH = scale_for(wave_max(hm));
        const h8* Cf = cfrag + lane + (last ? 6 * 64 : 0);
        h8 cf[RT_E][2];
#pragma unroll
        for (int jt = 0; jt < RT_E; ++jt)
#pragma unroll
            for (int ks = 0; ks < 2; ++ks) cf[jt][ks] = Cf[((jt < RT_A || !last ? jt : 0) * 2 + ks) * 64];
        f32x4 m[WL][RT_E];
#pragma unroll
        for (int ct = 0; ct < WL; ++ct) {
            h8 ah0, al0, ah1, al1;
            {
                unsigned wh0[4], wl0[4], wh1[4] = {0u, 0u, 0u, 0u}, wl1[4] = {0u, 0u, 0u, 0u};
                split2(H[0][ct][0], H[0][ct][1], sH, wh0[0], wl0[0]);
                split2(H[0][ct][2], H[0][ct][3], sH, wh0[1], wl0[1]);
                split2(H[1][ct][0], H[1][ct][1], sH, wh0[2], wl0[2]);
                split2(H[1][ct][2], H[1][ct][3], sH, wh0[3], wl0[3]);
                split2(H[2][ct][0], H[2][ct][1], sH, wh1[0], wl1[0]);
                split2(H[2][ct][2], H[2][ct][3], sH, wh1[1], wl1[1]);
                ah0 = __builtin_bit_cast(h8, u32x4{wh0[0], wh0[1], wh0[2], wh0[3]}); al0 = __builtin_bit_cast(h8, u32x4{wl0[0], wl0[1], wl0[2], wl0[3]});
                ah1 = __builtin_bit_cast(h8, u32x4{wh1[0], wh1[1], wh1[2], wh1[3]}); al1 = __builtin_bit_cast(h8, u32x4{wl1[0], wl1[1], wl1[2], wl1[3]});
            }
#pragma unroll
            for (int jt = 0; jt < RT_E; ++jt) {
                f32x4 z = f32x4{0.f, 0.f, 0.f, 0.f};
                if (jt < RT_A || !last) {
                    z = __builtin_amdgcn_mfma_f32_16x16x32_f16(ah0, cf[jt][0], z, 0, 0, 0);
                    z = __builtin_amdgcn_mfma_f32_16x16x32_f16(ah1, cf[jt][1], z, 0, 0, 0);
                    if constexpr (!LP) {
                        z = __builtin_amdgcn_mfma_f32_16x16x32_f16(al0, cf[jt][0], z, 0, 0, 0);
                        z = __builtin_amdgcn_mfma_f32_16x16x32_f16(al1, cf[jt][1], z, 0, 0, 0);
                    }
                }
                m[ct][jt] = z;
            }
        }
        stamp();
        const float isH = rcp_pow2_exact(sH);
        float mx = 0.f;
#pragma unroll
        for (int ct = 0; ct < WL; ++ct)
#pragma unroll
            for (int jt = 0; jt < RT_E; ++jt)
#pragma unroll
                for (int r = 0; r < 4; ++r) {
                    m[ct][jt][r] *= isH;
                    mx = fmaxf(mx, fabsf(m[ct][jt][r]));
                }
        const float s = tile_scale(mx);
        stamp();
        const int n_keep = last ? na : nrows;
        const long long keep0 = last ? va : rs;
#pragma unroll
        for (int ct = 0; ct < WL; ++ct) {
            const int col4 = (ct0() + ct) * 16 + lg * 4;
#pragma unroll
            for (int jt = 0; jt < RT_E; ++jt) {
                if (jt < RT_A || !last) {
                    const int row = jt * 16 + li;
                    const float4 v = make_float4(m[ct][jt][0], m[ct][jt][1], m[ct][jt][2], m[ct][jt][3]);
                    h4 hi, lo;
                    split4(v, s, hi, lo);
                    unsigned char* p = T16 + row * TS + (col4 >> 5) * 128 + (col4 & 31) * 2;
                    *reinterpret_cast<h4*>(p) = hi;
                    if constexpr (!LP) *reinterpret_cast<h4*>(p + 64) = lo;
                    if constexpr (KEEP) {
                        if (!keep_rows && keep && row < n_keep && col4 < N) store_keep4(keep + (keep0 + row) * keep_ld + col4, v);
                    }
                }
            }
        }
        if constexpr (KEEP) {
            if (keep_rows) {
                if (wave == 0 && lg == 0) {
#pragma unroll
                    for (int jt = 0; jt < RT_E; ++jt)
                        *reinterpret_cast<float4*>(T16 + (jt * 16 + li) * TS + (TS - 16)) = make_float4(s, tile_mx > 0.f ? 0.f : 1.f, 0.f, 0.f);
                }
                rows_pending = keep_rows + keep0 * TS;
                rows_pending_n = n_keep;
            }
        }
        return s;
    };

    using RE = std::integral_constant<int, RT_E>;
    using RA = std::integral_constant<int, RT_A>;
    const int T_steps = g.depth;

    f32x4 h0[RT_E][WL];
    {
        stamp();
        const ColConst cc = col_consts(G.Wi.inv_scale, g.b_i);
        zero_acc(RE{}, h0);
        float s_prev = 0.f;
        for (int grp = 0; grp * 4 < G.Wi.nc; ++grp) {
            if (grp > 0) ga_load(RE{}, T_{}, grp, g.d_v, g.d_e, rVg, rEg, ro1, ro2, a_grp);
            s_prev = ga_stage(RE{}, h0, a_grp, s_prev);
            if (grp == 0) stamp();
            const int ncg = G.Wi.nc - grp * 4 < 4 ? G.Wi.nc - grp * 4 : 4;
            contract(RE{}, h0, Ag, TSG, ncg, grp * 4, G.Wi);
        }
        unscale(RE{}, h0, rcp_pow2_exact(s_prev), cc);
        stamp();
    }
#if !defined(DMPNN_NO_L2_WARM)
#if !defined(DMPNN_L2_WARM_MIN_TILES)
#define DMPNN_L2_WARM_MIN_TILES 96
#define DMPNN_L2_WARM_MAX_TILES 256
#endif
    if (g.depth > 1 && hdr_tiles >= DMPNN_L2_WARM_MIN_TILES && hdr_tiles <= DMPNN_L2_WARM_MAX_TILES && t < 256) {
        launder();
        const unsigned nl = (unsigned)(((N + 15) / 16) * G.Wh.nc * 16);
        const rsrc_t rWh = gemm::make_rsrc(G.Wh.p, nl * 128u), rWo = gemm::make_rsrc(G.WoM.p, nl * 128u);
        const unsigned share = (unsigned)(((hdr_tiles < 256 ? hdr_tiles : 256) + 7) >> 3) * (unsigned)KT;
        unsigned line = (unsigned)(t >> 3) * (unsigned)KT + (unsigned)tid;
#pragma unroll
        for (int k = 0; k < 2; ++k, line += share) {
            const unsigned oh = line < nl ? line * 128u : kOOB, oo = (line >= nl && line < 2u * nl) ? (line - nl) * 128u : kOOB;
            pf_word[2 * k] = __builtin_bit_cast(unsigned, __builtin_amdgcn_raw_buffer_load_b32(rWh, oh, 0, 0));
            pf_word[2 * k + 1] = __builtin_bit_cast(unsigned, __builtin_amdgcn_raw_buffer_load_b32(rWo, oo, 0, 0));
        }
    }
#endif
    if (KEEP && G.keep_bits) {
        store_bits(RE{}, h0, 0);
    } else if (KEEP && g.H0) {
        __syncthreads();
        frag_to_tile(RE{}, h0);
        __syncthreads();
        tile_to_global(g.H0, rs, g.ldh, nrows);
    }
    float sA;
    {
        f32x4 y[RT_E][WL];
#pragma unroll
        for (int rt = 0; rt < RT_E; ++rt)
#pragma unroll
            for (int ct = 0; ct < WL; ++ct) y[rt][ct] = h0[rt][ct];
        act_frags(RE{}, F_{}, y, y);
        sA = segment_mfma(y, T_steps == 1, T_steps == 1 ? g.Mv : (G.Mrows ? nullptr : g.Ms), g.ldh, T_steps == 1 ? nullptr : G.Mrows);
    }
    stamp();
    if (G.atom_de) {
        const int de = G.atom_de;
        float* Et = reinterpret_cast<float*>(cfrag + 10 * 64);
        float* SE = Et + BM * kAtomK;
        for (int i = tid; i < BM * kAtomK; i += KT) {
            const int r = i / kAtomK, k = i - r * kAtomK;
            float v = 0.f;
            if (r < nrows && k < de) {
                const long long e = lean ? (long long)(rs + r) : (long long)g.perm[rs + r];
                v = g.E[e * g.lde + k];
            }
            Et[i] = v;
        }
        __syncthreads();
        for (int i = tid; i < BA * kAtomK; i += KT) {
            const int a_ = i / kAtomK, k = i - a_ * kAtomK;
            float sum = 0.f;
            if (a_ < na && k < de)
                for (int r = 0; r < nrows; ++r)
                    if (aor[r] == a_) sum += Et[r * kAtomK + k];
            SE[i] = sum;
        }
        __syncthreads();
        launder();
        if constexpr (KEEP) {
            if (G.atom_me) {
                for (int i = tid; i < nrows * kAtomK; i += KT) {
                    const int r = i / kAtomK, k = i - r * kAtomK;
                    const float v = SE[(lean ? asrc[r] : aor[revl[r]]) * kAtomK + k];
                    for (int sl = 0; sl < T_steps - 1; ++sl) G.atom_me[(long long)sl * G.me_slot + (long long)(rs + r) * kAtomK + k] = v;
                }
            }
        }
        float xv[RT_E][8];
        float mx = 0.f;
#pragma unroll
        for (int rt = 0; rt < RT_E; ++rt) {
            const int row = rt * 16 + li;
            const int a_s = row < nrows ? (lean ? asrc[row] : aor[revl[row]]) : -1;
#pragma unroll
            for (int j = 0; j < 8; ++j) {
                const int k = lg * 8 + j;
                xv[rt][j] = (a_s >= 0 && k < kAtomK) ? SE[a_s * kAtomK + (k < kAtomK ? k : 0)] : 0.f;
                mx = fmaxf(mx, fabsf(xv[rt][j]));
            }
        }
        const float sE = tile_scale(mx);
        h8 eh[RT_E], el[RT_E];
#pragma unroll
        for (int rt = 0; rt < RT_E; ++rt)
#pragma unroll
            for (int j = 0; j < 8; ++j) {
                const float x = xv[rt][j] * sE;
                const _Float16 hi = (_Float16)x;
                eh[rt][j] = hi; el[rt][j] = (_Float16)(x - (float)hi);
            }
        unsigned offE[WL];
        bfrag_offsets(G.WhE, offE);
        h8 wh[WL], wl[WL];
        load_bfrags(gemm::make_rsrc(G.WhE.p, (unsigned)(((N + 15) / 16) * G.WhE.nc * 2048)), offE, 0, wh, wl);
        const ColConst ce = col_consts(G.WhE.inv_scale, nullptr);
#pragma unroll
        for (int ct = 0; ct < WL; ++ct)
#pragma unroll
            for (int rt = 0; rt < RT_E; ++rt) {
                f32x4 z = f32x4{0.f, 0.f, 0.f, 0.f};
                z = __builtin_amdgcn_mfma_f32_16x16x32_f16(eh[rt], wh[ct], z, 0, 0, 0);
                z = __builtin_amdgcn_mfma_f32_16x16x32_f16(eh[rt], wl[ct], z, 0, 0, 0);
                z = __builtin_amdgcn_mfma_f32_16x16x32_f16(el[rt], wh[ct], z, 0, 0, 0);
                const float isw = ce.isw[ct] / sE;
#pragma unroll
                for (int r = 0; r < 4; ++r) h0[rt][ct][r] += z[r] * isw;
            }
    }

    for (int step = 1; step < T_steps; ++step) {
        f32x4 acc[RT_E][WL];
        zero_acc(RE{}, acc);
        const ColConst cc = col_consts(G.Wh.inv_scale, g.b_h);
        contract(RE{}, acc, T16, TS, (N + BK - 1) / BK, 0, G.Wh);
        stamp();
        unscale(RE{}, acc, rcp_pow2_exact(sA), cc);
        act_frags(RE{}, T_{}, acc, h0);
        dropout_frags(RE{}, acc, (unsigned)(step - 1), rs, true);
        stamp();
        if (KEEP && G.keep_bits) {
            store_bits(RE{}, acc, step);
        } else if (KEEP && g.Hs) {
            __syncthreads();
            frag_to_tile(RE{}, acc);
            __syncthreads();
            tile_to_global(g.Hs + (long long)(step - 1) * g.slot, rs, g.ldh, nrows);
        }
        const bool last = step == T_steps - 1;
        sA = segment_mfma(acc, last, last ? g.Mv : ((g.Ms && !G.Mrows) ? g.Ms + (long long)step * g.slot : nullptr), g.ldh,
                          (last || !G.Mrows) ? nullptr : G.Mrows + (long long)step * G.mrow_slot);
        stamp();
    }

    {
        f32x4 acc[RT_A][WL];
        zero_acc(RA{}, acc);
        const ColConst cc = col_consts(G.WoM.inv_scale, g.b_o);
        const rsrc_t rV = gemm::make_rsrc(g.V + (long long)va * g.ldv, (unsigned)(na * g.ldv) * 4u);
        const rsrc_t rnull = gemm::make_rsrc(g.W_o, 0);
        unsigned rov[JR * RT_A];
#pragma unroll
        for (int j = 0; j < JR * RT_A; ++j) rov[j] = wave + NW * j < na ? (unsigned)(wave + NW * j) * (unsigned)g.ldv * 4u : kOOB;
        u32x2 v_grp[JR * RT_A];
        ga_load(RA{}, F_{}, 0, g.d_v, 0, rV, rnull, rov, rov, v_grp);
        contract(RA{}, acc, T16, TS, (N + BK - 1) / BK, 0, G.WoM);
        stamp();
        float sV = sA;
        for (int grp = 0; grp * 4 < G.WoV.nc; ++grp) {
            if (grp > 0) ga_load(RA{}, F_{}, grp, g.d_v, 0, rV, rnull, rov, rov, v_grp);
            sV = ga_stage(RA{}, acc, v_grp, sV);
            if (grp == 0) stamp();
            const int ncg = G.WoV.nc - grp * 4 < 4 ? G.WoV.nc - grp * 4 : 4;
            contract(RA{}, acc, Ag, TSG, ncg, grp * 4, G.WoV);
        }
        stamp();
        unscale(RA{}, acc, rcp_pow2_exact(sV), cc);
        act_frags(RA{}, F_{}, acc, acc);
        dropout_frags(RA{}, acc, (unsigned)(T_steps - 1), va, false);
        if (maxbits[5]) {
#pragma unroll
            for (int rt = 0; rt < RT_A; ++rt)
#pragma unroll
                for (int ct = 0; ct < WL; ++ct) acc[rt][ct] = f32x4{__int_as_float(0x7fc00000), __int_as_float(0x7fc00000), __int_as_float(0x7fc00000), __int_as_float(0x7fc00000)};
        }
        if ((pf_word[0] ^ pf_word[1] ^ pf_word[2] ^ pf_word[3]) == 0x7fdead01u) maxbits[7] = 1u;
        __syncthreads();
        frag_to_tile(RA{}, acc);
        __syncthreads();
        tile_to_global(g.out, va, g.ldout, na);
        stamp();
        if constexpr (KEEP) {
            if (G.agg_Hm) {
                const long long m0 = G.agg_batch[va], m1 = G.agg_batch[vb - 1];
                if (m0 >= 0 && m1 < G.agg_n_mols && m1 - m0 < BA) {
                    const int nm = (int)(m1 - m0) + 1;
                    for (int it = tid; it < nm * QN; it += KT) {
                        const int ml = it / QN, q = it - ml * QN;
                        if (q >= qn) continue;
                        const long long m = m0 + ml;
                        const int f = G.agg_bounds[m] - va, e = G.agg_bounds[G.agg_n_mols + m] - va;
                        if (f < 0 || e > na || e <= f) continue;
                        float4 sacc = *reinterpret_cast<const float4*>(T + f * LDC + 4 * q);
                        for (int a = f + 1; a < e; ++a) {
                            const float4 x = *reinterpret_cast<const float4*>(T + a * LDC + 4 * q);
                            sacc.x += x.x; sacc.y += x.y; sacc.z += x.z; sacc.w += x.w;
                        }
                        if (G.agg_mode == DMPNN_MOLAGG_MEAN) { const float n = (float)(e - f); sacc.x /= n; sacc.y /= n; sacc.z /= n; sacc.w /= n; }
                        if (G.agg_mode == DMPNN_MOLAGG_NORM) { sacc.x /= G.agg_norm; sacc.y /= G.agg_norm; sacc.z /= G.agg_norm; sacc.w /= G.agg_norm; }
                        *reinterpret_cast<float4*>(G.agg_Hm + m * G.agg_ld + 4 * q) = sacc;
                        if (q == 0) G.agg_done[m] = 1;
                    }
                }
            }
        }
    }
    };
    if constexpr (NW == 4) {
        body(std::integral_constant<int, WN>{});
    } else {
        if (__builtin_amdgcn_readfirstlane((int)(threadIdx.x >> 6)) < 4) body(std::integral_constant<int, 3>{});
        else body(std::integral_constant<int, 2>{});
    }
}

template <int WN, bool SA, bool KEEP, int NW = 4, bool LP = false>
int launch_mega16(const Mega16K& g, int n_tiles, hipStream_t s);

#define DMPNN_DEFINE_MEGA16(WN, SA, KEEP) DMPNN_DEFINE_MEGA16_NW(WN, SA, KEEP, 4)
#define DMPNN_DEFINE_MEGA16_NW(WN, SA, KEEP, NW) DMPNN_DEFINE_MEGA16_LP(WN, SA, KEEP, NW, false)
#define DMPNN_DEFINE_MEGA16_LP(WN, SA, KEEP, NW, LP)                                                       \
    template <>                                                                                            \
    int launch_mega16<WN, SA, KEEP, NW, LP>(const Mega16K& g, int n_tiles, hipStream_t s) {                \
        const size_t lds = g.atom_de ? lds_bytes_atom<WN>() : lds_bytes<WN>();                             \
        static bool attr_set = false;                                                                      \
        if (!attr_set) {                                                                                   \
            hipError_t e = hipFuncSetAttribute(reinterpret_cast<const void*>(&k_mpnn_tile16<WN, SA, KEEP, NW, LP>),      \
                                               hipFuncAttributeMaxDynamicSharedMemorySize, (int)lds_bytes_atom<WN>()); \
            if (e != hipSuccess) {                                                                         \
                set_error("hipFuncSetAttribute(k_mpnn_tile16<%d>, %zu B LDS): %s", WN, lds, hipGetErrorString(e)); \
                return DMPNN_EHIP;                                                                         \
            }                                                                                              \
            attr_set = true;                                                                               \
        }                                                                                                  \
        hipLaunchKernelGGL((k_mpnn_tile16<WN, SA, KEEP, NW, LP>), dim3((unsigned)n_tiles), dim3(64 * NW), lds, s, g);   \
        DMPNN_CHECK_LAUNCH("k_mpnn_tile16");                                                               \
        return DMPNN_OK;                                                                                   \
    }

}
}
```

### chemprop_amd/csrc/dmpnn_prepare.hip

```cpp
#include <atomic>
#include <limits.h>

#include "dmpnn_common.hpp"
#include "dmpnn_mega16_impl.hpp"

namespace dmpnn {

extern thread_local long long* g_debug_stamps;

namespace {

constexpr int kBlock = 256;

__global__ void k_plan_init(int* __restrict__ plan, int64_t cursor_off, int nV, int nE, int keep_mtiles) {
    const int64_t tid = blockIdx.x * (int64_t)blockDim.x + threadIdx.x;
    if (tid < DMPNN_HDR_WORDS) {
        int v = 0;
        if (tid == DMPNN_HDR_NATOMS) v = nV;
        if (tid == DMPNN_HDR_NEDGES) v = nE;
        if (keep_mtiles) {
            if (tid == DMPNN_HDR_FLAGS) v = plan[tid] & PLAN_NO_PIECE_TILES;
            if (tid == DMPNN_HDR_NMTILES || tid == DMPNN_HDR_NSPILL) v = plan[tid];
        }
        plan[tid] = v;
// ... 107 lines not shown
    if (e < nE) {
        const int d = plan[L.dst + e];
        const int pos = atomicAdd(&plan[L.cursor + d], 1);
        plan[L.perm + pos] = e;
    }
}

__global__ void k_sort_rows(int* __restrict__ plan, PlanLayout L, int nV) {
    const int v = blockIdx.x * blockDim.x + threadIdx.x;
    int n = 0;
    if (v < nV) {
        const int b = plan[L.row_ptr + v];
        n = plan[L.row_ptr + v + 1] - b;
        int* row = plan + L.perm + b;
        for (int i = 1; i < n; ++i) {
            const int key = row[i];
            int j = i - 1;
            while (j >= 0 && row[j] > key) {
                row[j + 1] = row[j];
                --j;
            }
            row[j + 1] = key;
        }
    }
    int m = n;
    for (int off = 32; off > 0; off >>= 1) m = max(m, __shfl_xor(m, off));
    if ((threadIdx.x & 63) == 0 && m > 0) atomicMax(&plan[DMPNN_HDR_MAXDEG], m);
}

__global__ void k_inverse(int* __restrict__ plan, PlanLayout L, int nE) {
    const int i = blockIdx.x * blockDim.x + threadIdx.x;
    if (i < nE) plan[L.inv + plan[L.perm + i]] = i;
}

struct TileGeom {
    int b0, n_tiles;
};
__device__ __forceinline__ TileGeom tile_geom(int maxdeg, int nE) {
    TileGeom g;
    const int md = maxdeg < 1 ? 1 : maxdeg;
    g.b0 = kFusedBM - md + 1;
    g.n_tiles = (md > kFusedMaxDeg || nE == 0) ? 0 : (nE + g.b0 - 1) / g.b0;
    return g;
}
__device__ __forceinline__ int tile_of(int row_start, const TileGeom& g) {
    const int t = row_start / g.b0;
    return t < g.n_tiles - 1 ? t : g.n_tiles - 1;
}
__device__ __forceinline__ void write_tiles(int* __restrict__ plan, const PlanLayout& L, const int* __restrict__ row_ptr,
                                            int nV, int nE, const TileGeom& g, int i, int n_threads) {
    int* tile_row = plan + L.tile_row;
    int* tile_atom = plan + L.tile_atom;
    const int slots = (int)L.max_tiles + 2;
    if (g.n_tiles == 0) {
        for (int t = i; t < slots; t += n_threads) { tile_row[t] = nE; tile_atom[t] = nV; }
        return;
    }
    for (int v = i; v < nV; v += n_threads) {
        const int rs = row_ptr[v];
        const int tv = tile_of(rs, g);
        const int tp = v == 0 ? -1 : tile_of(row_ptr[v - 1], g);
        for (int t = tp + 1; t <= tv; ++t) { tile_row[t] = rs; tile_atom[t] = v; }
    }
    const int tl = nV > 0 ? tile_of(row_ptr[nV - 1], g) : -1;
    for (int t = tl + 1 + i; t < slots; t += n_threads) { tile_row[t] = nE; tile_atom[t] = nV; }
}

__global__ void k_rows_tiles(int* __restrict__ plan, PlanLayout L, int nV, int nE, int keep_mtiles) {
    const int i = blockIdx.x * blockDim.x + threadIdx.x;
    const int n_threads = gridDim.x * blockDim.x;
    const int maxdeg = plan[DMPNN_HDR_MAXDEG];
    const TileGeom g = tile_geom(maxdeg, nE);
    for (int r = i; r < nE; r += n_threads) {
        const int e = plan[L.perm + r];
        plan[L.srcp + r] = plan[L.src + e];
        plan[L.dstp + r] = plan[L.dst + e];
        plan[L.revp + r] = plan[L.inv + plan[L.rev + e]];
        plan[L.ident + r] = r;
    }
    write_tiles(plan, L, plan + L.row_ptr, nV, nE, g, i, n_threads);
    if (keep_mtiles) {
        const int* matom = plan + L.mtile_atom;
        const int* mrow = plan + L.mtile_row;
        const int* row_ptr = plan + L.row_ptr;
        const int nmt = plan[DMPNN_HDR_NMTILES];
        int bad = 0;
        for (int t = i; t < (int)L.max_mtiles + 2; t += n_threads) {
            const int a = matom[t];
            if (a < 0 || a > nV || mrow[t] != row_ptr[a]) bad = 1;
        }
        if (nmt > 0) {
            for (int r = i; r < nE; r += n_threads) {
                const int e = plan[L.perm + r];
                const int d = plan[L.dst + e], sa = plan[L.src + e];
                int lo = 0, hi = nmt;
                while (hi - lo > 1) {
                    const int mid = (lo + hi) >> 1;
                    if (matom[mid] <= d) lo = mid; else hi = mid;
                }
                if (sa < matom[lo] || sa >= matom[lo + 1]) bad = 1;
            }
        }
        if (bad) atomicOr(&plan[DMPNN_HDR_FLAGS], PLAN_NO_PIECE_TILES);
    } else {
        for (int t = i; t < (int)L.max_mtiles + 2; t += n_threads) { plan[L.mtile_row + t] = nE; plan[L.mtile_atom + t] = nV; }
    }
    if (i == 0) {
        plan[DMPNN_HDR_NTILES] = g.n_tiles;
        plan[DMPNN_HDR_TILE_STRIDE] = g.b0;
        if (!keep_mtiles) plan[DMPNN_HDR_NMTILES] = 0;
        atomicOr(&plan[DMPNN_HDR_FLAGS], (keep_mtiles ? 0 : PLAN_NO_PIECE_TILES) | (maxdeg > kFusedMaxDeg ? PLAN_HUGE_DEGREE : 0));
    }
}

constexpr int kSmallThreads = 1024;
constexpr int kSmallMaxAtoms = 6144;
constexpr int kSmallMaxEdges = 10240;
constexpr int kSmallItems = kSmallMaxAtoms / kSmallThreads;
constexpr int kSmallEPT = kSmallMaxEdges / kSmallThreads;
typedef unsigned short u16;


template <bool MAX>
__device__ __forceinline__ void block_scan_inclusive(int* a, int n, int* wave_tot, int tid) {
    const int lane = tid & 63, wid = tid >> 6;
    int v[kSmallItems];
    const int i0 = tid * kSmallItems;
    int run = MAX ? INT_MIN : 0;
#pragma unroll
    for (int j = 0; j < kSmallItems; ++j) {
        const int x = (i0 + j < n) ? a[i0 + j] : (MAX ? INT_MIN : 0);
        run = MAX ? max(run, x) : run + x;
        v[j] = run;
    }
    int inc = run;
#pragma unroll
    for (int off = 1; off < 64; off <<= 1) {
        const int t = __shfl_up(inc, off);
        if (lane >= off) inc = MAX ? max(inc, t) : inc + t;
    }
    __syncthreads();
    if (lane == 63) wave_tot[wid] = inc;
    __syncthreads();
    int base = MAX ? INT_MIN : 0;
    for (int w = 0; w < wid; ++w) base = MAX ? max(base, wave_tot[w]) : base + wave_tot[w];
    const int prev = __shfl_up(inc, 1);
    const int excl = lane == 0 ? base : (MAX ? max(base, prev) : base + prev);
#pragma unroll
    for (int j = 0; j < kSmallItems; ++j)
        if (i0 + j < n) a[i0 + j] = MAX ? max(excl, v[j]) : excl + v[j];
    __syncthreads();
}

template <class RowOf, class Other>
__device__ __forceinline__ int pack_pieces(int* __restrict__ plan, const PlanLayout& L, const int* X, int np, RowOf&& row_of,
                                           int* Y, int* bad_s, int* spill_s, int nV, int nE, int tid, Other&& other_work,
                                           long long* dbg, int n_st) {
    auto stamp = [&]() {
        if (dbg && tid == 0 && n_st < 12) dbg[n_st] = (long long)__builtin_readcyclecounter();
        ++n_st;
    };
    int* mrow = plan + L.mtile_row;
    int* matom = plan + L.mtile_atom;
    const int slots = (int)L.max_mtiles + 2;
    int nx[kSmallItems];
#pragma unroll
    for (int j = 0; j < kSmallItems; ++j) {
        const int p = tid + kSmallThreads * j;
        nx[j] = np;
        if (p < np) {
            const int v = X[p], r0 = row_of(p);
            int q = p + 1;
#if !defined(DMPNN_PACK_ROWS)
#define DMPNN_PACK_ROWS kMegaBM
#endif
            if (X[q] - v > kMegaBA || row_of(q) - r0 > kMegaBM) {
                atomicAdd(spill_s, 1);
            } else {
                while (q < np && X[q + 1] - v <= kMegaBA && row_of(q + 1) - r0 <= DMPNN_PACK_ROWS) ++q;
            }
            nx[j] = q;
        }
    }
    __syncthreads();
#pragma unroll
    for (int j = 0; j < kSmallItems; ++j) {
        const int p = tid + kSmallThreads * j;
        if (p <= np) Y[p] = (p < np ? nx[j] : np);
    }
    __syncthreads();
    stamp();
    constexpr int kMaxBlocks = kSmallMaxAtoms / 64 + 1;
    __shared__ int ntile_s;
    __shared__ int blk_cnt[kMaxBlocks];
    __shared__ unsigned long long blk_mask[kMaxBlocks];
    if (tid == 0) ntile_s = 0;
    __syncthreads();
    const int lane = tid & 63, wave = __builtin_amdgcn_readfirstlane(tid >> 6);
    const int nblk = (np + 63) >> 6;
    const bool walk = *bad_s == 0;
    if (walk) {
        for (int blk = wave; blk < nblk; blk += kSmallThreads / 64) {
            const int base = blk * 64, p = base + lane;
            const int my_nx = p < np ? Y[p] : np;
            const int lim = (base + 64 < np ? base + 64 : np);
            unsigned long long mask = 0ull;
            int es = base;
            while (es < lim) {
                mask |= 1ull << (es - base);
                es = __builtin_amdgcn_readlane(my_nx, es - base);
            }
            if (lane == 0) { blk_mask[blk] = mask; blk_cnt[blk] = __popcll(mask); }
        }
    }
#if defined(DMPNN_K0_STAMPS2)
    stamp();
#endif
    __syncthreads();
#if defined(DMPNN_K0_STAMPS2)
    stamp();
#endif
    if (walk) {
        for (int blk = wave; blk < nblk; blk += kSmallThreads / 64) {
            int rank = 0;
            for (int b2 = lane; b2 < blk; b2 += 64) rank += blk_cnt[b2];
            for (int off = 32; off > 0; off >>= 1) rank += __shfl_xor(rank, off);
            const unsigned long long mask = blk_mask[blk];
            const int p = blk * 64 + lane;
            const bool on = (mask >> lane) & 1ull;
            const int r = rank + __popcll(mask & ((1ull << lane) - 1ull));
            if (on && r < (int)L.max_mtiles) {
                mrow[r] = row_of(p);
                matom[r] = X[p];
            }
            if (blk == nblk - 1 && lane == 0) {
                const int total = rank + __popcll(mask);
                if (total > (int)L.max_mtiles) atomicOr(bad_s, 1);
                ntile_s = total;
            }
        }
    }
#if defined(DMPNN_K0_STAMPS2)
    stamp();
#endif
    other_work(tid, kSmallThreads);
#if defined(DMPNN_K0_STAMPS2)
    stamp();
#endif
    __syncthreads();
    stamp();
    const int n_tiles = ntile_s;
    const bool bad = *bad_s != 0;
    if (bad) {
        for (int t = tid; t < slots; t += kSmallThreads) { mrow[t] = nE; matom[t] = nV; }
        return -1;
    }
    for (int t = n_tiles + tid; t < slots; t += kSmallThreads) { mrow[t] = nE; matom[t] = nV; }
    return n_tiles;
}

template <class Other>
__device__ __forceinline__ int build_piece_tiles(int* __restrict__ plan, const PlanLayout& L, const int* rowp, int* X,
                                                 int* Y, int* wave_tot, int* bad_s, int* spill_s, int nV, int nE, int tid,
                                                 Other&& other_work, long long* dbg = nullptr) {
    int n_st = 0;
    auto stamp = [&]() {
        if (dbg && tid == 0 && n_st < 12) dbg[n_st] = (long long)__builtin_readcyclecounter();
        ++n_st;
    };
    stamp();
    const int n_words = (nV + 31) >> 5;
    const unsigned char* covb = reinterpret_cast<const unsigned char*>(Y);
    unsigned* stw = reinterpret_cast<unsigned*>(Y + (nV + 3) / 4 + 1);
    int* wrank = reinterpret_cast<int*>(stw) + 2 * ((nV + 63) >> 6);
    for (int u0 = (tid >> 6) * 64; u0 < nV; u0 += kSmallThreads) {
        const int u = u0 + (tid & 63);
        const unsigned long long m = __ballot(u < nV && covb[u] == 0);
        if ((tid & 63) == 0) { stw[u0 >> 5] = (unsigned)m; stw[(u0 >> 5) + 1] = (unsigned)(m >> 32); }
    }
    __syncthreads();
    const unsigned my_starts = tid < n_words ? stw[tid] : 0u;
    stamp();
    __shared__ int np_s;
    {
        const int lane = tid & 63, w = tid >> 6;
        const int pc = __popc(my_starts);
        int inc = pc;
#pragma unroll
        for (int off = 1; off < 64; off <<= 1) {
            const int t = __shfl_up(inc, off);
            if (lane >= off) inc += t;
        }
        if (lane == 63) wave_tot[w] = inc;
        __syncthreads();
        int base = 0;
        for (int k = 0; k < w; ++k) base += wave_tot[k];
        if (tid < n_words) wrank[tid] = base + inc - pc;
        if (tid == n_words - 1) np_s = base + inc;
        if (n_words == 0 && tid == 0) np_s = 0;
    }
    __syncthreads();
    stamp();
    const int np = np_s;
    if (tid < n_words) {
        int p = wrank[tid];
        unsigned bits = my_starts;
        while (bits) {
            const int bpos = __ffs(bits) - 1;
            bits &= bits - 1u;
            X[p++] = tid * 32 + bpos;
        }
    }
    if (tid == 0) X[np] = nV;
    __syncthreads();
    stamp();
    return pack_pieces(plan, L, X, np, [&](int p) { return rowp[X[p]]; }, Y, bad_s, spill_s, nV, nE, tid, other_work, dbg, n_st);
}

__global__ __launch_bounds__(kSmallThreads) void k_prepare_small(const int64_t* __restrict__ edge_index,
                                                                const int64_t* __restrict__ rev64,
                                                                int* __restrict__ plan, PlanLayout L, int nV, int nE,
                                                                int light, long long* dbg) {
    extern __shared__ __attribute__((aligned(16))) int lds_i[];
    int n_stamp = 0;
    auto stamp = [&]() {
        if (dbg && threadIdx.x == 0 && n_stamp < 16) dbg[n_stamp] = (long long)__builtin_readcyclecounter();
        ++n_stamp;
    };
    stamp();
    int* cnt = lds_i;
    int* rowp = lds_i + nV + 2;
    u16* src16 = reinterpret_cast<u16*>(rowp + nV + 2);
    u16* dst16 = src16 + nE;
    u16* rev16 = dst16 + nE;
    u16* perm16 = rev16 + nE;
    u16* inv16 = perm16 + nE;
    int* Ybuf = reinterpret_cast<int*>(lds_i) + 2 * (nV + 2) + (5 * nE + 1) / 2;
    __shared__ int wave_tot[kSmallThreads / 64];
    __shared__ int flags_s, maxdeg_s, piece_bad_s, spill_s;
    const int tid = threadIdx.x, lane = tid & 63, wid = tid >> 6;
    for (int i = tid; i < nV; i += kSmallThreads) cnt[i] = 0;
    if (tid == 0) { flags_s = 0; maxdeg_s = 0; piece_bad_s = 0; spill_s = 0; }
    const bool lean = light == 2;
    unsigned char* covb = reinterpret_cast<unsigned char*>(Ybuf);
    if (lean)
        for (int w = tid; w < (nV + 3) / 4 + 1; w += kSmallThreads) Ybuf[w] = 0;

    int64_t s64[kSmallEPT], d64[kSmallEPT], r64[kSmallEPT];
#pragma unroll
    for (int j = 0; j < kSmallEPT; ++j) { s64[j] = 0; d64[j] = 0; r64[j] = 0; }
    if (nE > 0) {
#pragma unroll
        for (int j = 0; j < kSmallEPT; ++j) {
            const int e = tid + kSmallThreads * j;
            const int ec = e < nE ? e : 0;
            s64[j] = edge_index[ec];
            d64[j] = edge_index[(int64_t)nE + ec];
            if (light != 2) r64[j] = rev64[ec];
        }
    }
    __syncthreads();
    stamp();
    int bad = 0;
#pragma unroll
    for (int j = 0; j < kSmallEPT; ++j) {
        const int e = tid + kSmallThreads * j;
        int64_t s = s64[j], d = d64[j], r = r64[j];
        if (e < nE) {
            if (s < 0 || s >= nV || d < 0 || d >= nV || r < 0 || r >= nE) {
                bad |= PLAN_RANGE_ERROR | PLAN_ASYMMETRIC;
                s = s < 0 ? 0 : (s >= nV ? nV - 1 : s);
                d = d < 0 ? 0 : (d >= nV ? nV - 1 : d);
                r = r < 0 ? 0 : (r >= nE ? nE - 1 : r);
            }
            atomicAdd(&cnt[(int)d], 1);
            src16[e] = (u16)s;
            dst16[e] = (u16)d;
            rev16[e] = (u16)r;
        }
    }
    __syncthreads();
    if (lean) {
        for (int e = tid; e < nE; e += kSmallThreads) {
            const int sa = src16[e], da = dst16[e];
            if (sa < da) {
                for (int u = sa + 1; u <= da; ++u) covb[u] = 1;
            }
        }
    }
    stamp();
    if (!lean)
        for (int e = tid; e < nE; e += kSmallThreads) {
            const int r = rev16[e];
            if (rev16[r] != e || src16[r] != dst16[e] || dst16[r] != src16[e]) bad |= PLAN_ASYMMETRIC;
        }
    if (lean) bad &= ~PLAN_ASYMMETRIC;
    if (bad) atomicOr(&flags_s, bad);
    stamp();
    {
        int v[kSmallItems];
        int tot = 0;
        const int i0 = tid * kSmallItems;
#pragma unroll
        for (int j = 0; j < kSmallItems; ++j) {
            v[j] = (i0 + j < nV) ? cnt[i0 + j] : 0;
            tot += v[j];
        }
        int inc = tot;
#pragma unroll
        for (int off = 1; off < 64; off <<= 1) {
            const int t = __shfl_up(inc, off);
            if (lane >= off) inc += t;
        }
        if (lane == 63) wave_tot[wid] = inc;
        __syncthreads();
        int wave_base = 0;
        for (int w = 0; w < wid; ++w) wave_base += wave_tot[w];
        int run = wave_base + inc - tot;
        int md = 0;
#pragma unroll
        for (int j = 0; j < kSmallItems; ++j) {
            if (i0 + j < nV) {
                rowp[i0 + j] = run;
                cnt[i0 + j] = run;
                if (!lean) plan[L.row_ptr + i0 + j] = run;
            }
            run += v[j];
            md = max(md, v[j]);
        }
        if (tid == kSmallThreads - 1) { rowp[nV] = run; if (!lean) plan[L.row_ptr + nV] = run; }
        for (int off = 32; off > 0; off >>= 1) md = max(md, __shfl_xor(md, off));
        if (lane == 0 && md > 0) atomicMax(&maxdeg_s, md);
    }
    __syncthreads();
    stamp();
    if (!lean) {
    for (int w = tid; w < (nV + 3) / 4 + 1; w += kSmallThreads) Ybuf[w] = 0;
    for (int e = tid; e < nE; e += kSmallThreads) {
        const int pos = atomicAdd(&cnt[dst16[e]], 1);
        perm16[pos] = (u16)e;
    }
    }
    __syncthreads();
    stamp();
    if (!lean)
    for (int v = tid; v < nV; v += kSmallThreads) {
        const int b = rowp[v];
        const int n = rowp[v + 1] - b;
        u16* row = perm16 + b;
        int far = v;
        if (n <= 4) {
            const int last = n > 0 ? n - 1 : 0;
            unsigned e0 = row[0 <= last ? 0 : last], e1 = row[1 <= last ? 1 : last], e2 = row[2 <= last ? 2 : last], e3 = row[3 <= last ? 3 : last];
            e0 = n > 0 ? e0 : 0xffffu; e1 = n > 1 ? e1 : 0xffffu; e2 = n > 2 ? e2 : 0xffffu; e3 = n > 3 ? e3 : 0xffffu;
            unsigned t;
#define DMPNN_CSWAP(x, y) t = min(x, y); y = max(x, y); x = t
            DMPNN_CSWAP(e0, e1); DMPNN_CSWAP(e2, e3); DMPNN_CSWAP(e0, e2); DMPNN_CSWAP(e1, e3); DMPNN_CSWAP(e1, e2);
#undef DMPNN_CSWAP
            const unsigned ee[4] = {e0, e1, e2, e3};
#pragma unroll
            for (int k = 0; k < 4; ++k) {
                if (k < n) {
                    row[k] = (u16)ee[k];
                    inv16[ee[k]] = (u16)(b + k);
                    far = max(far, (int)src16[ee[k]]);
                }
            }
        } else {
            for (int i = 1; i < n; ++i) {
                const u16 key = row[i];
                int j = i - 1;
                while (j >= 0 && row[j] > key) {
                    row[j + 1] = row[j];
                    --j;
                }
                row[j + 1] = key;
            }
            for (int k = 0; k < n; ++k) {
                inv16[row[k]] = (u16)(b + k);
                far = max(far, (int)src16[row[k]]);
            }
        }
        for (int u = v + 1; u <= far; ++u) covb[u] = 1;
    }
    __syncthreads();
    stamp();
    stamp();
    TileGeom g = tile_geom(maxdeg_s, nE);
    if (lean) g.n_tiles = 0;
    auto outputs = [&](int i0, int n_thr) {
        for (int i = i0; i < (lean ? 0 : nE); i += n_thr) {
            const int e = perm16[i];
            plan[L.perm + i] = e;
            plan[L.srcp + i] = src16[e];
            plan[L.revp + i] = inv16[rev16[e]];
            if (!light) {
                plan[L.src + i] = src16[i];
                plan[L.dst + i] = dst16[i];
                plan[L.rev + i] = rev16[i];
                plan[L.inv + i] = inv16[i];
                plan[L.dstp + i] = dst16[e];
                plan[L.ident + i] = i;
            }
        }
        write_tiles(plan, L, rowp, nV, nE, g, i0, n_thr);
    };
    stamp();
    stamp();
    const int n_mtiles = build_piece_tiles(plan, L, rowp, cnt, Ybuf, wave_tot, &piece_bad_s, &spill_s, nV, nE, tid, outputs, dbg ? dbg + 16 : nullptr);
    stamp();
    if (tid < DMPNN_HDR_WORDS) {
        int v = 0;
        if (tid == DMPNN_HDR_FLAGS) v = flags_s | (maxdeg_s > kFusedMaxDeg ? PLAN_HUGE_DEGREE : 0) | (n_mtiles < 0 ? PLAN_NO_PIECE_TILES : 0) | (lean ? PLAN_TILES_ONLY : 0);
        if (tid == DMPNN_HDR_NMTILES) v = n_mtiles < 0 ? 0 : n_mtiles;
        if (tid == DMPNN_HDR_NSPILL) v = n_mtiles < 0 ? 0 : spill_s;
        if (tid == DMPNN_HDR_LIGHT) v = light;
        if (tid == DMPNN_HDR_MAXDEG) v = maxdeg_s;
        if (tid == DMPNN_HDR_NATOMS) v = nV;
        if (tid == DMPNN_HDR_NEDGES) v = nE;
        if (tid == DMPNN_HDR_NTILES) v = g.n_tiles;
        if (tid == DMPNN_HDR_TILE_STRIDE) v = g.b0;
        plan[tid] = v;
    }
}


__device__ __forceinline__ void tiles_batch_finish(int* fa, int* fe, int* Y, int nm, int* bad_sp, int* flags_sp, int* spill_sp, int* __restrict__ plan,
                                                   const PlanLayout& L, int nV, int nE, long long* dbg, int n_stamp, int* __restrict__ mol_bounds,
                                                   int n_mols_out);
__device__ __forceinline__ void prepare_tiles_batch_body(int* lds_i, const int64_t* __restrict__ edge_index,
                                                         const int64_t* __restrict__ batch,
                                                         int* __restrict__ plan, const PlanLayout& L, int nV, int nE,
                                                         long long* dbg, int* __restrict__ mol_bounds, int n_mols_out) {
    int n_stamp = 0;
    auto stamp = [&]() {
        if (dbg && threadIdx.x == 0 && n_stamp < 16) dbg[n_stamp] = (long long)__builtin_readcyclecounter();
        ++n_stamp;
    };
    stamp();
    int* fa = lds_i;
    int* fe = fa + nV + 2;
    int* Y = fe + nV + 2;
    u16* bm = reinterpret_cast<u16*>(Y + nV + 2);
    u16* mb = bm + nV + (nV & 1);
    __shared__ int bad_s, flags_s, nm_s, spill_s;
    const int tid = threadIdx.x;
    if (tid == 0) { bad_s = 0; flags_s = 0; nm_s = 0; spill_s = 0; }
    int64_t d64[kSmallEPT], b64[kSmallItems];
    int bad = 0;
#pragma unroll
    for (int j = 0; j < kSmallItems; ++j) {
        const int v = tid + kSmallThreads * j;
        b64[j] = batch[v < nV ? v : 0];
    }
#pragma unroll
    for (int j = 0; j < kSmallEPT; ++j) d64[j] = 0;
    if (nE > 0) {
#pragma unroll
        for (int j = 0; j < kSmallEPT; ++j) {
            const int e = tid + kSmallThreads * j;
            d64[j] = edge_index[(int64_t)nE + (e < nE ? e : 0)];
        }
    }
#pragma unroll
    for (int j = 0; j < kSmallItems; ++j) {
        const int v = tid + kSmallThreads * j;
        if (v < nV) {
            if (b64[j] < 0 || b64[j] >= nV) { bad |= PLAN_RANGE_ERROR; b64[j] = 0; }
            bm[v] = (u16)b64[j];
        }
    }
    __syncthreads();
#pragma unroll
    for (int j = 0; j < kSmallEPT; ++j) {
        const int e = tid + kSmallThreads * j;
        if (e < nE) {
            const bool ok = d64[j] >= 0 && d64[j] < nV;
            if (!ok) bad |= PLAN_RANGE_ERROR;
            mb[e] = bm[ok ? (int)d64[j] : 0];
        }
    }
    __syncthreads();
    stamp();
    for (int v = tid + 1; v < nV; v += kSmallThreads)
        if (bm[v] < bm[v - 1]) bad |= PLAN_NO_PIECE_TILES;
    for (int e = tid + 1; e < nE; e += kSmallThreads)
        if (mb[e] < mb[e - 1]) bad |= PLAN_NO_PIECE_TILES;
    if (bad) atomicOr(&flags_s, bad);
    if (tid == 0) nm_s = nV > 0 ? (int)bm[nV - 1] + 1 : 0;
    __syncthreads();
    stamp();
    const int nm = nm_s;
    for (int m = tid; m <= nm; m += kSmallThreads) {
        int lo = 0, hi = nV, lo2 = 0, hi2 = nE;
        while (lo < hi || lo2 < hi2) {
            const int mid = (lo + hi) >> 1, mid2 = (lo2 + hi2) >> 1;
            const int x = lo < hi ? (int)bm[mid] : 0, y = lo2 < hi2 ? (int)mb[mid2] : 0;
            if (lo < hi) { if (x < m) lo = mid + 1; else hi = mid; }
            if (lo2 < hi2) { if (y < m) lo2 = mid2 + 1; else hi2 = mid2; }
        }
        fa[m] = lo;
        fe[m] = lo2;
    }
    if ((flags_s & (PLAN_NO_PIECE_TILES | PLAN_RANGE_ERROR)) && tid == 0) bad_s = 1;
    __syncthreads();
    stamp();
    tiles_batch_finish(fa, fe, Y, nm, &bad_s, &flags_s, &spill_s, plan, L, nV, nE, dbg, n_stamp, mol_bounds, n_mols_out);
}

__device__ __forceinline__ void tiles_batch_finish(int* fa, int* fe, int* Y, int nm, int* bad_sp, int* flags_sp, int* spill_sp, int* __restrict__ plan,
                                                   const PlanLayout& L, int nV, int nE, long long* dbg, int n_stamp, int* __restrict__ mol_bounds,
                                                   int n_mols_out) {
    const int tid = threadIdx.x;
    auto stamp = [&]() {
        if (dbg && threadIdx.x == 0 && n_stamp < 16) dbg[n_stamp] = (long long)__builtin_readcyclecounter();
        ++n_stamp;
    };
    int& bad_s = *bad_sp; int& flags_s = *flags_sp; int& spill_s = *spill_sp;
    if (mol_bounds) {
        for (int m = tid; m < n_mols_out; m += kSmallThreads) {
            mol_bounds[m] = m <= nm ? fa[m] : nV;
            mol_bounds[n_mols_out + m] = m + 1 <= nm ? fa[m + 1] : nV;
            mol_bounds[2 * n_mols_out + 4 + m] = 0;
        }
        if (tid == 0)
            mol_bounds[2 * n_mols_out] = ((flags_s & PLAN_RANGE_ERROR) || nm > n_mols_out ? 1 : 0) | ((flags_s & PLAN_NO_PIECE_TILES) ? 2 : 0);
    }
    TileGeom g;
    g.b0 = kFusedBM; g.n_tiles = 0;
    auto rest = [&](int i0, int n_thr) { write_tiles(plan, L, fe, nV, nE, g, i0, n_thr); };
    const int n_mtiles = pack_pieces(plan, L, fa, nm, [&](int p) { return fe[p]; }, Y, &bad_s, &spill_s, nV, nE, tid, rest, dbg ? dbg + 16 : nullptr, 3);
    stamp();
    if (tid < DMPNN_HDR_WORDS) {
        int v = 0;
        if (tid == DMPNN_HDR_FLAGS) v = (flags_s & PLAN_RANGE_ERROR) | (n_mtiles < 0 ? PLAN_NO_PIECE_TILES : 0) | PLAN_TILES_ONLY;
        if (tid == DMPNN_HDR_NMTILES) v = n_mtiles < 0 ? 0 : n_mtiles;
        if (tid == DMPNN_HDR_NSPILL) v = n_mtiles < 0 ? 0 : spill_s;
        if (tid == DMPNN_HDR_LIGHT) v = 2;
        if (tid == DMPNN_HDR_NATOMS) v = nV;
        if (tid == DMPNN_HDR_NEDGES) v = nE;
        if (tid == DMPNN_HDR_TILE_STRIDE) v = g.b0;
        plan[tid] = v;
    }
}
__global__ __launch_bounds__(kSmallThreads) void k_prepare_tiles_batch(const int64_t* __restrict__ edge_index, const int64_t* __restrict__ batch,
                                                                      int* __restrict__ plan, PlanLayout L, int nV, int nE,
                                                                      long long* dbg, int* __restrict__ mol_bounds, int n_mols_out) {
    extern __shared__ __attribute__((aligned(16))) int lds_i[];
    prepare_tiles_batch_body(lds_i, edge_index, batch, plan, L, nV, nE, dbg, mol_bounds, n_mols_out);
}
__global__ __launch_bounds__(kSmallThreads) void k_prepare_tiles_batch_split(const int64_t* __restrict__ edge_index, const int64_t* __restrict__ batch,
                                                                            int* __restrict__ plan, PlanLayout L, int nV, int nE,
                                                                            long long* dbg, int* __restrict__ mol_bounds, int n_mols_out,
                                                                            mega16::SplitArgs sp) {
    extern __shared__ __attribute__((aligned(16))) int lds_i[];
    if (blockIdx.x == 0) prepare_tiles_batch_body(lds_i, edge_index, batch, plan, L, nV, nE, dbg, mol_bounds, n_mols_out);
    else mega16::split_weights_wave(sp, ((int)blockIdx.x - 1) * (kSmallThreads / 64) + (int)(threadIdx.x >> 6), (int)(threadIdx.x & 63));
}


constexpr unsigned kBoundsTag = 0x6b30a11du;
constexpr int kBoundsMaxSpins = 4096;
struct MultiScratch { int64_t aoff, eoff, done, end; int n_bounds; unsigned tag; };
static MultiScratch multi_scratch(const PlanLayout& L, int64_t nV, int64_t nE) {
    MultiScratch S;
    S.n_bounds = (int)(((nV > nE ? nV : nE) + 1 + kSmallThreads - 1) / kSmallThreads);
    S.tag = 0u;
    int64_t o = (L.src + 1) & ~int64_t(1);
    S.aoff = o; o += align4(2 * (nV + 2));
    S.eoff = o; o += align4(2 * (nV + 2));
    S.done = o; o += align4(2 * (int64_t)S.n_bounds);
    S.end = o;
    return S;
}
__device__ __forceinline__ void st_agent(int* p, int v) { __hip_atomic_store(p, v, __ATOMIC_RELAXED, __HIP_MEMORY_SCOPE_AGENT); }
__device__ __forceinline__ int ld_agent(const int* p) { return __hip_atomic_load(p, __ATOMIC_RELAXED, __HIP_MEMORY_SCOPE_AGENT); }
__device__ __forceinline__ void st_tagged(int* base, int m, unsigned tag, int v) {
    __hip_atomic_store(reinterpret_cast<unsigned long long*>(base) + m, ((unsigned long long)tag << 32) | (unsigned)v, __ATOMIC_RELAXED, __HIP_MEMORY_SCOPE_AGENT);
}

__device__ __forceinline__ void tiles_bounds_block(const int64_t* __restrict__ edge_index, const int64_t* __restrict__ batch, int* __restrict__ plan,
                                                   const MultiScratch& S, int nV, int nE, int b) {
    __shared__ int bad_blk;
    if (threadIdx.x == 0) bad_blk = 0;
    __syncthreads();
    const int i = b * kSmallThreads + (int)threadIdx.x;
    const int64_t last = batch[nV - 1];
    const int n_mols = last < 0 ? 0 : (last >= nV ? nV : (int)last + 1);
    int* aoff = plan + S.aoff;
    int* eoff = plan + S.eoff;
    const int64_t* dst = edge_index + nE;
    int bad = 0;
    auto clampm = [&](int64_t m) -> int { return m < 0 ? 0 : (m >= n_mols ? (n_mols > 0 ? n_mols - 1 : 0) : (int)m); };
    const int64_t bm = i < nV ? batch[i] : 0, bp = (i > 0 && i < nV) ? batch[i - 1] : -1;
    int64_t d = (i < nE) ? dst[i] : 0, dp = (i > 0 && i <= nE && nE > 0) ? dst[i - 1] : 0;
    if (i < nE && (d < 0 || d >= nV)) { bad |= PLAN_RANGE_ERROR; d = 0; }
    if (dp < 0 || dp >= nV) dp = 0;
    const int64_t em64 = i < nE ? batch[d] : 0, ep64 = (i > 0 && i <= nE && nE > 0) ? batch[dp] : -1;
    if (i < nV) {
        if (bm < 0 || bm >= nV) bad |= PLAN_RANGE_ERROR;
        if (bm < bp || bm > last) bad |= PLAN_NO_PIECE_TILES;
        const int m = clampm(bm), pm = i > 0 ? clampm(bp) : -1;
        for (int mm = pm + 1; mm <= m; ++mm) st_tagged(aoff, mm, S.tag, i);
    } else if (i == nV) {
        st_tagged(aoff, n_mols, S.tag, nV);
    }
    if (i < nE) {
        if (em64 < ep64) bad |= PLAN_NO_PIECE_TILES;
        const int m = clampm(em64), pm = i > 0 ? clampm(ep64) : -1;
        for (int mm = pm + 1; mm <= m; ++mm) st_tagged(eoff, mm, S.tag, i);
    } else if (i == nE) {
        const int pm = nE > 0 ? clampm(ep64) : -1;
        for (int mm = pm + 1; mm <= n_mols; ++mm) st_tagged(eoff, mm, S.tag, nE);
    }
    if (bad) atomicOr(&bad_blk, bad);
    asm volatile("s_waitcnt vmcnt(0)" ::: "memory");
    __syncthreads();
    if (threadIdx.x == 0)
        __hip_atomic_store(reinterpret_cast<unsigned long long*>(plan + S.done) + b, ((unsigned long long)S.tag << 32) | (unsigned)bad_blk,
                           __ATOMIC_RELAXED, __HIP_MEMORY_SCOPE_AGENT);
}

__device__ __forceinline__ void tiles_pack_block(int* lds_i, const int64_t* __restrict__ batch, int* __restrict__ plan, const PlanLayout& L,
                                                 const MultiScratch& S, int nV, int nE, long long* dbg, int* __restrict__ mol_bounds, int n_mols_out) {
    int n_stamp = 0;
    auto stamp = [&]() {
        if (dbg && threadIdx.x == 0 && n_stamp < 16) dbg[n_stamp] = (long long)__builtin_readcyclecounter();
        ++n_stamp;
    };
    stamp();
    int* fa = lds_i;
    int* fe = fa + nV + 2;
    int* Y = fe + nV + 2;
    __shared__ int bad_s, flags_s, spill_s;
    const int tid = threadIdx.x;
    if (tid == 0) { bad_s = 0; flags_s = 0; spill_s = 0; }
    const int64_t last = batch[nV - 1];
    const int nm = last < 0 ? 0 : (last >= nV ? nV : (int)last + 1);
    __syncthreads();
    unsigned long long* done = reinterpret_cast<unsigned long long*>(plan + S.done);
    {
        unsigned long long* a64 = reinterpret_cast<unsigned long long*>(plan + S.aoff);
        unsigned long long* e64 = reinterpret_cast<unsigned long long*>(plan + S.eoff);
        for (int m = tid; m <= nm; m += kSmallThreads) {
            unsigned long long wa = 0ull, we = 0ull;
            int spins = 0;
            for (;;) {
                wa = __hip_atomic_load(a64 + m, __ATOMIC_RELAXED, __HIP_MEMORY_SCOPE_AGENT);
                we = __hip_atomic_load(e64 + m, __ATOMIC_RELAXED, __HIP_MEMORY_SCOPE_AGENT);
                if (((unsigned)(wa >> 32) == S.tag && (unsigned)(we >> 32) == S.tag) || ++spins >= kBoundsMaxSpins) break;
                __builtin_amdgcn_s_sleep(2);
            }
            const bool ok = (unsigned)(wa >> 32) == S.tag && (unsigned)(we >> 32) == S.tag;
            if (!ok) atomicOr(&flags_s, PLAN_NO_PIECE_TILES);
            fa[m] = ok ? (int)(unsigned)wa : 0;
            fe[m] = ok ? (int)(unsigned)we : 0;
            __hip_atomic_store(a64 + m, 0ull, __ATOMIC_RELAXED, __HIP_MEMORY_SCOPE_AGENT);
            __hip_atomic_store(e64 + m, 0ull, __ATOMIC_RELAXED, __HIP_MEMORY_SCOPE_AGENT);
        }
    }
    __syncthreads();
    stamp();
    __syncthreads();
    stamp();
    {
        int bad = 0;
        for (int m = tid; m <= nm; m += kSmallThreads) {
            const int a = fa[m], e = fe[m];
            if (a < 0 || a > nV || e < 0 || e > nE) bad = 1;
            if (m > 0 && (fa[m - 1] > a || fe[m - 1] > e)) bad = 1;
        }
        if (bad) atomicOr(&flags_s, PLAN_NO_PIECE_TILES);
    }
    __syncthreads();
    if ((flags_s & (PLAN_NO_PIECE_TILES | PLAN_RANGE_ERROR)) && tid == 0) bad_s = 1;
    __syncthreads();
    stamp();
    unsigned long long w_early = 0ull;
    if (tid < S.n_bounds) w_early = __hip_atomic_load(done + tid, __ATOMIC_RELAXED, __HIP_MEMORY_SCOPE_AGENT);
    tiles_batch_finish(fa, fe, Y, nm, &bad_s, &flags_s, &spill_s, plan, L, nV, nE, dbg, n_stamp, mol_bounds, n_mols_out);
    __shared__ int late_s;
    if (tid == 0) late_s = 0;
    __syncthreads();
    if (tid < S.n_bounds) {
        unsigned long long w = w_early;
        int spins = 0;
        while ((unsigned)(w >> 32) != S.tag && ++spins < kBoundsMaxSpins) {
            __builtin_amdgcn_s_sleep(8);
            w = __hip_atomic_load(done + tid, __ATOMIC_RELAXED, __HIP_MEMORY_SCOPE_AGENT);
        }
        if ((unsigned)(w >> 32) != S.tag) atomicOr(&late_s, PLAN_NO_PIECE_TILES);
        else if ((unsigned)w) atomicOr(&late_s, (int)((unsigned)w & (PLAN_NO_PIECE_TILES | PLAN_RANGE_ERROR)));
        __hip_atomic_store(done + tid, 0ull, __ATOMIC_RELAXED, __HIP_MEMORY_SCOPE_AGENT);
    }
    __syncthreads();
    if (tid == 0 && (late_s & ~flags_s)) {
        plan[DMPNN_HDR_FLAGS] |= late_s & (PLAN_NO_PIECE_TILES | PLAN_RANGE_ERROR);
        if (late_s & PLAN_NO_PIECE_TILES) { plan[DMPNN_HDR_NMTILES] = 0; plan[DMPNN_HDR_NSPILL] = 0; }
        if (mol_bounds) mol_bounds[2 * n_mols_out] |= ((late_s & PLAN_RANGE_ERROR) ? 1 : 0) | ((late_s & PLAN_NO_PIECE_TILES) ? 2 : 0);
    }
}

__global__ __launch_bounds__(kSmallThreads) void k_prepare_tiles_batch_multi(const int64_t* __restrict__ edge_index, const int64_t* __restrict__ batch,
                                                                            int* __restrict__ plan, PlanLayout L, MultiScratch S, int nV, int nE,
                                                                            long long* dbg, int* __restrict__ mol_bounds, int n_mols_out,
                                                                            mega16::SplitArgs sp) {
    extern __shared__ __attribute__((aligned(16))) int lds_i[];
    const int b = (int)blockIdx.x;
    if (b < S.n_bounds) tiles_bounds_block(edge_index, batch, plan, S, nV, nE, b);
    else if (b + 1 < (int)gridDim.x) mega16::split_weights_wave(sp, (b - S.n_bounds) * (kSmallThreads / 64) + (int)(threadIdx.x >> 6), (int)(threadIdx.x & 63));
    else tiles_pack_block(lds_i, batch, plan, L, S, nV, nE, dbg, mol_bounds, n_mols_out);
}

__global__ __launch_bounds__(256) void k_tiles_from_table_split(const int* __restrict__ tile_row, const int* __restrict__ tile_atom, int n_tiles,
                                                                int nV, int nE, int* __restrict__ plan, PlanLayout L, mega16::SplitArgs sp) {
    if (blockIdx.x == 0) tiles_from_table_body(tile_row, tile_atom, n_tiles, nV, nE, plan, L);
    else mega16::split_weights_wave(sp, ((int)blockIdx.x - 1) * 4 + (int)(threadIdx.x >> 6), (int)(threadIdx.x & 63));
}

}

int launch_tiles_from_table_split(const int* tile_row, const int* tile_atom, int64_t n_tiles, int64_t nV, int64_t nE, int* plan, hipStream_t s,
                                  const dmpnn_fwd_args* split_for, bool* did_split) {
    *did_split = false;
    mega16::SplitArgs sp;
    if (!split_for || !(split_for->flags & DMPNN_F_MEGA) || !(split_for->flags & DMPNN_F_SPLIT16) || (split_for->flags & DMPNN_F_WSPLIT_READY) ||
        !mega16_split_args(*split_for, &sp))
        return DMPNN_OK;
    const PlanLayout L = plan_layout(nV, nE);
    const int waves = ((sp.N + 15) & ~15) * sp.n_jobs;
    hipLaunchKernelGGL(k_tiles_from_table_split, dim3((unsigned)(1 + (waves + 3) / 4)), dim3(256), 0, s, tile_row, tile_atom, (int)n_tiles, (int)nV,
                       (int)nE, plan, L, sp);
    DMPNN_CHECK_LAUNCH("k_tiles_from_table_split");
    *did_split = true;
    return DMPNN_OK;
}

static size_t tiles_batch_lds_bytes(int64_t nV, int64_t nE) {
    return ((size_t)(3 * (nV + 2)) * 4 + (size_t)(nV + 1 + nE + 2) * 2 + 31) & ~size_t(15);
}

int launch_prepare_tiles_batch(const int64_t* edge_index, const int64_t* batch, int64_t nV64, int64_t nE64, int* plan, hipStream_t s,
                               int* mol_bounds, int64_t n_mols, const dmpnn_fwd_args* split_for, bool* did_split) {
    const int nV = (int)nV64, nE = (int)nE64;
    const PlanLayout L = plan_layout(nV, nE);
    if (did_split) *did_split = false;
    mega16::SplitArgs sp;
    {
        const char* k0e = getenv("DMPNN_K0_SINGLE");
        const bool multi_off = k0e && atoi(k0e) != 0;
        MultiScratch S = multi_scratch(L, nV, nE);
        static std::atomic<unsigned> launch_no{0u};
        S.tag = kBoundsTag ^ (launch_no.fetch_add(1u, std::memory_order_relaxed) * 0x9E3779B1u);
        if (S.tag == 0u) S.tag = kBoundsTag;
        if (!multi_off && nV > 0 && S.end <= L.tile_row) {
            const bool split = split_for && did_split && (split_for->flags & DMPNN_F_MEGA) && (split_for->flags & DMPNN_F_SPLIT16) &&
                               !(split_for->flags & DMPNN_F_WSPLIT_READY) && mega16_split_args(*split_for, &sp);
            if (!split) memset(&sp, 0, sizeof(sp));
            static bool attr3_set = false;
            if (!attr3_set) {
                hipError_t e = hipFuncSetAttribute(reinterpret_cast<const void*>(&k_prepare_tiles_batch_multi),
                                                   hipFuncAttributeMaxDynamicSharedMemorySize, 160 * 1024 - 2048);
                if (e != hipSuccess) {
                    set_error("hipFuncSetAttribute(k_prepare_tiles_batch_multi): %s", hipGetErrorString(e));
                    return DMPNN_EHIP;
                }
                attr3_set = true;
            }
            const int waves = split ? ((sp.N + 15) & ~15) * sp.n_jobs : 0, wpb = kSmallThreads / 64;
            const size_t lds = ((size_t)(3 * (nV + 2)) * 4 + 31) & ~size_t(15);
            hipLaunchKernelGGL(k_prepare_tiles_batch_multi, dim3((unsigned)(S.n_bounds + (waves + wpb - 1) / wpb + 1)), dim3(kSmallThreads), lds, s,
                               edge_index, batch, plan, L, S, nV, nE, g_debug_stamps ? g_debug_stamps + 32 : nullptr, mol_bounds, (int)n_mols, sp);
            DMPNN_CHECK_LAUNCH("k_prepare_tiles_batch_multi");
            if (split) *did_split = true;
            return DMPNN_OK;
        }
    }
    if (split_for && did_split && (split_for->flags & DMPNN_F_MEGA) && (split_for->flags & DMPNN_F_SPLIT16) && !(split_for->flags & DMPNN_F_WSPLIT_READY) &&
        mega16_split_args(*split_for, &sp)) {
        static bool attr2_set = false;
        if (!attr2_set) {
            hipError_t e = hipFuncSetAttribute(reinterpret_cast<const void*>(&k_prepare_tiles_batch_split),
                                               hipFuncAttributeMaxDynamicSharedMemorySize, 160 * 1024 - 2048);
            if (e != hipSuccess) {
                set_error("hipFuncSetAttribute(k_prepare_tiles_batch_split): %s", hipGetErrorString(e));
                return DMPNN_EHIP;
            }
            attr2_set = true;
        }
        const int waves = ((sp.N + 15) & ~15) * sp.n_jobs, wpb = kSmallThreads / 64;
        hipLaunchKernelGGL(k_prepare_tiles_batch_split, dim3((unsigned)(1 + (waves + wpb - 1) / wpb)), dim3(kSmallThreads), tiles_batch_lds_bytes(nV, nE), s,
                           edge_index, batch, plan, L, nV, nE, g_debug_stamps ? g_debug_stamps + 32 : nullptr, mol_bounds, (int)n_mols, sp);
        DMPNN_CHECK_LAUNCH("k_prepare_tiles_batch_split");
        *did_split = true;
        return DMPNN_OK;
    }
    static bool attr_set = false;
    if (!attr_set) {
        hipError_t e = hipFuncSetAttribute(reinterpret_cast<const void*>(&k_prepare_tiles_batch),
                                           hipFuncAttributeMaxDynamicSharedMemorySize, 160 * 1024 - 2048);
        if (e != hipSuccess) {
            set_error("hipFuncSetAttribute(k_prepare_tiles_batch): %s", hipGetErrorString(e));
            return DMPNN_EHIP;
        }
        attr_set = true;
    }
    hipLaunchKernelGGL(k_prepare_tiles_batch, dim3(1), dim3(kSmallThreads), tiles_batch_lds_bytes(nV, nE), s, edge_index, batch, plan,
                       L, nV, nE, g_debug_stamps ? g_debug_stamps + 32 : nullptr, mol_bounds, (int)n_mols);
    DMPNN_CHECK_LAUNCH("k_prepare_tiles_batch");
    return DMPNN_OK;
}

bool prepare_can_keep_mtiles(int64_t nV, int64_t nE) {
    const PlanLayout L = plan_layout(nV, nE);
    return (nV + kScanThreads * kScanItems - 1) / (kScanThreads * kScanItems) <= L.max_tiles + 2;
}

int launch_prepare(const int64_t* edge_index, const int64_t* rev, int64_t nV64, int64_t nE64,
                   int* plan, int light, hipStream_t s, bool keep_mtiles) {
    const int nV = (int)nV64, nE = (int)nE64;
    const PlanLayout L = plan_layout(nV, nE);
    if (small_plan_fits(nV, nE)) {
        const size_t lds = small_plan_lds_bytes(nV, nE);
        static bool attr_set = false;
        if (!attr_set) {
            hipError_t e = hipFuncSetAttribute(reinterpret_cast<const void*>(&k_prepare_small),
                                               hipFuncAttributeMaxDynamicSharedMemorySize, 160 * 1024 - 2048);
            if (e != hipSuccess) {
                set_error("hipFuncSetAttribute(k_prepare_small): %s", hipGetErrorString(e));
                return DMPNN_EHIP;
            }
            attr_set = true;
        }
        hipLaunchKernelGGL(k_prepare_small, dim3(1), dim3(kSmallThreads), lds, s, edge_index, rev, plan, L, nV, nE, light,
                           g_debug_stamps ? g_debug_stamps + 32 : nullptr);
        DMPNN_CHECK_LAUNCH("k_prepare_small");
        return DMPNN_OK;
    }
    {
        const int64_t n = nV > DMPNN_HDR_WORDS ? nV : DMPNN_HDR_WORDS;
        int grid = (int)((n + kBlock - 1) / kBlock);
        if (grid > 2048) grid = 2048;
        hipLaunchKernelGGL(k_plan_init, dim3(grid), dim3(kBlock), 0, s, plan, L.cursor, nV, nE, keep_mtiles ? 1 : 0);
        DMPNN_CHECK_LAUNCH("k_plan_init");
    }
    if (nE > 0) {
        const int grid = (nE + kBlock - 1) / kBlock;
        hipLaunchKernelGGL(k_convert_count, dim3(grid), dim3(kBlock), 0, s, edge_index, rev, plan, L, nV, nE);
        DMPNN_CHECK_LAUNCH("k_convert_count");
    }
    {
        const int nblk = nV > 0 ? (nV + kScanThreads * kScanItems - 1) / (kScanThreads * kScanItems) : 1;
        int* part = plan + (keep_mtiles ? L.tile_row : L.mtile_row);
        if (nblk > 1) {
            hipLaunchKernelGGL(k_scan_totals, dim3(nblk), dim3(kScanThreads), 0, s, plan, L, nV, part);
            DMPNN_CHECK_LAUNCH("k_scan_totals");
        }
        hipLaunchKernelGGL(k_scan, dim3(nblk), dim3(kScanThreads), 0, s, plan, L, nV, part);
        DMPNN_CHECK_LAUNCH("k_scan");
    }
    if (nE > 0) {
        const int grid = (nE + kBlock - 1) / kBlock;
        hipLaunchKernelGGL(k_fill, dim3(grid), dim3(kBlock), 0, s, plan, L, nE);
        DMPNN_CHECK_LAUNCH("k_fill");
        const int gridv = (nV + kBlock - 1) / kBlock;
        hipLaunchKernelGGL(k_sort_rows, dim3(gridv), dim3(kBlock), 0, s, plan, L, nV);
        DMPNN_CHECK_LAUNCH("k_sort_rows");
        hipLaunchKernelGGL(k_inverse, dim3(grid), dim3(kBlock), 0, s, plan, L, nE);
        DMPNN_CHECK_LAUNCH("k_inverse");
    }
    {
        const int64_t n = nV > nE ? nV : nE;
// ... 11 lines not shown
```

### include/dmpnn.h

```cpp
#ifndef DMPNN_H
#define DMPNN_H

#include <stddef.h>
#include <stdint.h>

#ifdef __cplusplus
extern "C" {
#endif

#define DMPNN_ABI_VERSION 15

enum dmpnn_status {
    DMPNN_OK = 0,
    DMPNN_EINVAL = -1,
    DMPNN_EHIP = -2,
    DMPNN_ENOSPC = -3
};

enum dmpnn_activation {
    DMPNN_ACT_NONE = 0,
    DMPNN_ACT_RELU = 1,
    DMPNN_ACT_LEAKYRELU = 2,
    DMPNN_ACT_PRELU = 3,
    DMPNN_ACT_TANH = 4,
// ... 114 lines not shown
                        size_t plan_bytes, void* stream);
int dmpnn_forward_can_fuse(const dmpnn_fwd_args* a);
enum dmpnn_route { DMPNN_ROUTE_GENERAL = 0, DMPNN_ROUTE_GENERAL16 = 1, DMPNN_ROUTE_FUSED = 2, DMPNN_ROUTE_FUSED16 = 3,
                   DMPNN_ROUTE_MEGA = 4, DMPNN_ROUTE_MEGA16 = 5 };
int dmpnn_forward_route(const dmpnn_fwd_args* a, int keep, int max_level, int plan_kind, int arith);
int dmpnn_tile_waves(int64_t n_atoms, int64_t n_edges, int64_t d_h, int64_t n_tiles);

#define DMPNN_KEEP_ROWS_MIN 4096
typedef struct dmpnn_train_route_info {
    int32_t plan_kind;
    int32_t route;
    int32_t keep_rows;
    int32_t keep_bits;
    int32_t lean;
} dmpnn_train_route_info;
int dmpnn_train_route(const dmpnn_fwd_args* a, int64_t n_mols, int32_t have, int32_t oversize, int32_t max_level, int32_t arith,
                      int32_t keep_rows, dmpnn_train_route_info* out);

typedef struct dmpnn_bwd_args {
    dmpnn_fwd_args f;
    const float* gout; int64_t ldgout;
    float* gW_i; float* gb_i; float* gW_h; float* gb_h;
    float* gW_o; float* gb_o; float* gW_d; float* gb_d;
    float* ws; size_t ws_bytes;
    const float* g_edge; int64_t ld_gedge;
} dmpnn_bwd_args;
size_t dmpnn_backward_ws_bytes(const dmpnn_fwd_args* f);
int dmpnn_backward(const dmpnn_bwd_args* a, void* stream);

int dmpnn_message_bwd(const void* plan, int64_t n_atoms, int64_t n_edges, int64_t d_h,
                      const float* gM, int64_t ld_gm, float* gH, int64_t ld_gh, void* stream);
int dmpnn_aggregate_bwd(const void* plan, int64_t n_atoms, int64_t n_edges, int64_t d_h,
                        const float* gMv, int64_t ld_gmv, float* gH, int64_t ld_gh, void* stream);
size_t dmpnn_linear_wgrad_ws_bytes(int64_t M, int64_t N, int64_t K, int has_bias);
int dmpnn_linear_wgrad(const dmpnn_gemm_args* g, const float* gZ, int64_t ldgz, float* gW, int64_t ldgw,
                       float* gb, void* ws, size_t ws_bytes, void* stream);

enum dmpnn_molagg_mode { DMPNN_MOLAGG_SUM = 0, DMPNN_MOLAGG_MEAN = 1, DMPNN_MOLAGG_NORM = 2 };
size_t dmpnn_molagg_ws_bytes(int64_t n_mols);
int dmpnn_molagg_bounds(const int64_t* batch, int64_t n_atoms, int64_t n_mols, void* ws, size_t ws_bytes, void* stream);
int dmpnn_molagg_fwd(const float* H, int64_t ldh, int64_t n_atoms, int64_t d_h, int64_t n_mols, const void* ws, int mode,
                     float norm, float* out, int64_t ldo, void* stream);
int dmpnn_molagg_bwd(const float* gout, int64_t ldg, const int64_t* batch, int64_t n_atoms, int64_t d_h, int64_t n_mols,
                     const void* ws, int mode, float norm, float* gH, int64_t ldgh, void* stream);

int dmpnn_gather_rows(const float* X, int64_t ldx, int64_t n_src, const int* idx, int64_t n_out, int64_t d,
                      float* out, int64_t ldo, void* stream);

int dmpnn_collate(const int* atom_off, const int* edge_off, int64_t n_mols, const int* src, const int* dst, const int* rev,
                  int64_t n_atoms, int64_t n_edges, int64_t* edge_index, int64_t* rev_edge_index, int64_t* batch,
                  void* stream);

int64_t dmpnn_pack_tiles(const int* atom_off, const int* edge_off, int64_t n_mols, int* tile_row, int* tile_atom, int64_t cap);
int64_t dmpnn_max_tiles(int64_t n_atoms, int64_t n_edges);
int dmpnn_prepare_tiles_from_table(const int* tile_row, const int* tile_atom, int64_t n_tiles, int64_t n_atoms,
                                   int64_t n_edges, void* plan, size_t plan_bytes, void* stream);

int dmpnn_adam_step(float* p, const float* g, float* m, float* v, int64_t n, float lr, float beta1, float beta2, float eps,
                    float weight_decay, float bias_corr1, float sqrt_bias_corr2, float grad_scale, const float* dev_scalars,
                    void* stream);

enum dmpnn_clip_mode { DMPNN_CLIP_NORM = 0, DMPNN_CLIP_VALUE = 1 };
size_t dmpnn_clip_grad_ws_bytes(void);
int dmpnn_clip_grad(float* g, int64_t n, float clip_val, int32_t mode, float grad_scale, float* ws, void* stream);

#define DMPNN_MAX_FFN_LAYERS 8
#define DMPNN_MAX_COMPONENTS 8
#define DMPNN_DROP_SITE_FFN 0x10000
enum dmpnn_loss { DMPNN_LOSS_MSE = 0, DMPNN_LOSS_MAE = 1,
                  DMPNN_LOSS_BCE = 2,
                  DMPNN_LOSS_CE = 3,
                  DMPNN_LOSS_MVE = 4,
                  DMPNN_LOSS_EVIDENTIAL = 5,
                  DMPNN_LOSS_QUANTILE = 6  };
typedef struct dmpnn_head_args {
    int64_t n_atoms, n_mols, d_h;
    const int64_t* batch;
    int32_t agg_mode; float agg_norm;
    const float* bn_weight; const float* bn_bias;
    float* bn_running_mean; float* bn_running_var;
    float bn_eps, bn_momentum; int32_t bn_training;
    int32_t n_layers; int32_t act; float act_slope;
    const float* W[DMPNN_MAX_FFN_LAYERS];
    const float* b[DMPNN_MAX_FFN_LAYERS];
    int64_t dims[DMPNN_MAX_FFN_LAYERS + 1];
    int32_t loss;
    const float* targets;
    const float* weights;
    const float* task_weights;
    const unsigned char* lt_mask; const unsigned char* gt_mask;
    float* preds;
    float* loss_out;
    float* gW[DMPNN_MAX_FFN_LAYERS]; float* gb[DMPNN_MAX_FFN_LAYERS];
    float* g_bn_weight; float* g_bn_bias;
    float* gHv; int64_t ldg;
    void* ws; size_t ws_bytes;
    int64_t* bn_num_batches_tracked;
    int32_t n_classes;
    float evid_v_kl, evid_eps;
    float quantile_alpha;
    const float* X_d; int64_t ld_xd;
    int32_t n_components;
    float ffn_dropout_p; uint64_t ffn_dropout_seed;
} dmpnn_head_args;
size_t dmpnn_head_ws_bytes(const dmpnn_head_args* h);
int dmpnn_head(const dmpnn_head_args* h, const float* Hv, int64_t ldhv, void* stream);

enum dmpnn_step_stage {
    DMPNN_STEP_FORWARD = 1,
    DMPNN_STEP_BACKWARD = 2,
    DMPNN_STEP_UPDATE = 4
};
typedef struct dmpnn_step_component {
    const int64_t* edge_index; const int64_t* rev_edge_index; const int64_t* batch; size_t plan_bytes; int32_t plan_ready;
    dmpnn_bwd_args bwd;
} dmpnn_step_component;

#define DMPNN_VD_MAX_WIDTH 544
typedef struct dmpnn_vd_args {
    int64_t n_atoms, d_h, d_vd;
    const float* Hv;  int64_t ldhv;
    const float* V_d; int64_t ldvd;
    const float* W_d; const float* b_d;
    float* out; int64_t ldout;
    const float* gout; int64_t ldgout;
    float* gHv; int64_t ldghv;
    float* gW_d; float* gb_d;
    void* ws; size_t ws_bytes;
} dmpnn_vd_args;
size_t dmpnn_vd_ws_bytes(const dmpnn_vd_args* a);
int dmpnn_vd_forward(const dmpnn_vd_args* a, void* stream);
int dmpnn_vd_backward(const dmpnn_vd_args* a, void* stream);

typedef struct dmpnn_step_args {
    const int64_t* edge_index; const int64_t* rev_edge_index; const int64_t* batch; size_t plan_bytes; int32_t plan_ready;
    int32_t stages;
    dmpnn_bwd_args bwd;
    dmpnn_head_args head;
    float* p; const float* g; float* m; float* v; int64_t n_params;
    float lr, beta1, beta2, eps, weight_decay, bias_corr1, sqrt_bias_corr2, grad_scale; const float* dev_scalars;
    float clip_val; int32_t clip_mode; float* clip_ws;
    int32_t n_extra; const dmpnn_step_component* extra;
    const dmpnn_vd_args* vd;
} dmpnn_step_args;
int dmpnn_train_step(const dmpnn_step_args* a, void* stream);

int dmpnn_dropout_keep(uint64_t seed, int32_t site, int64_t row, int64_t col, float p);

int dmpnn_version(void);
int dmpnn_debug_timestamps(void* device_buf);
void dmpnn_debug_lds_poison(int on);
const char* dmpnn_last_error_string(void);
int dmpnn_last_launch_count(void);

#ifdef __cplusplus
}
#endif
#endif
```

Measured before the change: 463.3 M edge-updates/s.

## Fuse tile planning, weight split and forward into one persistent launch

Adds a single-kernel forward path (k_forward_one). Producer blocks build the tile plan and split the weights, then signal readiness through agent-scope atomic flags in the plan workspace, and every block spins until the plan is ready before running the 8-wave tile forward. It is enabled by default when forward_tiles is called with a batch and the geometry fits within the CU count. It removes the separate K0 planning and weight-split launches and their gaps, at the cost of spin-waiting, and it relies on all producer blocks being co-resident to avoid deadlock.

```diff
diff --git a/chemprop_amd/_lib.py b/chemprop_amd/_lib.py
--- a/chemprop_amd/_lib.py
+++ b/chemprop_amd/_lib.py
@@ -18,7 +18,7 @@
 PLAN_NOFFSETS = 15
 
 EXPORTS = [
-    "dmpnn_version", "dmpnn_debug_timestamps", "dmpnn_last_error_string", "dmpnn_last_launch_count", "dmpnn_plan_bytes",
+    "dmpnn_version", "dmpnn_debug_timestamps", "dmpnn_last_error_string", "dmpnn_last_launch_count", "dmpnn_forward_tiles_launch_count", "dmpnn_forward_one_launch_window", "dmpnn_plan_bytes",
     "dmpnn_plan_layout", "dmpnn_prepare", "dmpnn_prepare_light", "dmpnn_prepare_tiles", "dmpnn_message_fwd", "dmpnn_aggregate_fwd",
     "dmpnn_linear_fwd", "dmpnn_linear16_wsplit_bytes", "dmpnn_linear16_ok", "dmpnn_linear16_fwd", "dmpnn_update_fwd", "dmpnn_forward", "dmpnn_forward_can_fuse", "dmpnn_forward_wsplit_bytes", "dmpnn_forward_keep_bits_bytes", "dmpnn_forward_spill_bytes", "dmpnn_backward_ws_bytes", "dmpnn_backward", "dmpnn_message_bwd",
     "dmpnn_aggregate_bwd", "dmpnn_linear_wgrad_ws_bytes", "dmpnn_linear_wgrad",
@@ -258,6 +258,9 @@
     lib.dmpnn_version.restype = C.c_int
     lib.dmpnn_last_error_string.restype = C.c_char_p
     lib.dmpnn_last_launch_count.restype = C.c_int
+    lib.dmpnn_forward_tiles_launch_count.restype = C.c_int
+    lib.dmpnn_forward_one_launch_window.restype = C.c_int
+    lib.dmpnn_forward_one_launch_window.argtypes = [C.POINTER(FwdArgs), C.c_int, C.c_int, C.c_int, C.c_int]
     lib.dmpnn_plan_bytes.restype = C.c_size_t
     lib.dmpnn_plan_bytes.argtypes = [C.c_int64, C.c_int64]
     lib.dmpnn_plan_layout.argtypes = [C.c_int64, C.c_int64, C.POINTER(C.c_int64)]
diff --git a/chemprop_amd/csrc/dmpnn_abi.hip b/chemprop_amd/csrc/dmpnn_abi.hip
--- a/chemprop_amd/csrc/dmpnn_abi.hip
+++ b/chemprop_amd/csrc/dmpnn_abi.hip
@@ -9,6 +9,7 @@
 
 static thread_local char g_err[512] = "";
 static thread_local int g_launches = 0;
+static thread_local int g_tiles_launches = 0;
 
 void set_error(const char* fmt, ...) {
     va_list ap;
@@ -77,6 +78,10 @@
 }
 const char* dmpnn_last_error_string(void) { return g_err; }
 int dmpnn_last_launch_count(void) { return g_launches; }
+int dmpnn_forward_tiles_launch_count(void) { return g_tiles_launches; }
+int dmpnn_forward_one_launch_window(const dmpnn_fwd_args* a, int from_batch, int k0_single, int forced_tile_waves, int n_cu) {
+    return (a && forward_one_launch_window(*a, from_batch != 0, k0_single != 0, forced_tile_waves, n_cu)) ? 1 : 0;
+}
 
 size_t dmpnn_plan_bytes(int64_t n_atoms, int64_t n_edges) {
     if (n_atoms < 0 || n_edges < 0) return 0;
@@ -385,6 +390,25 @@
     DMPNN_CHECK_ARG(a != nullptr && a->plan != nullptr, "forward_tiles: null args / plan");
     void* plan = const_cast<void*>(a->plan);
     bool did_split = false;
+    g_tiles_launches = 0;
+    const int launches_before = g_launches;
+    if (!(tile_row && tile_atom && n_tiles > 0) && batch) {
+        const char* oe = getenv("DMPNN_ONE_LAUNCH");
+        const char* k0e = getenv("DMPNN_K0_SINGLE");
+        const bool one_on = !(oe && oe[0] != 0 && atoi(oe) == 0);
+        if (one_on && check_graph_sizes(a->n_atoms, a->n_edges) == DMPNN_OK && aligned16(plan) && a->edge_index &&
+            plan_bytes >= dmpnn_plan_bytes(a->n_atoms, a->n_edges) && a->wsplit && a->wsplit_bytes >= mega16_fwd_wsplit_bytes(*a) &&
+            forward_one_launch_window(*a, true, k0e && atoi(k0e) != 0, tile_waves_forced(), device_cu_count())) {
+            g_one_ride.batch = batch; g_one_ride.taken = false;
+            const int rc = dmpnn_forward(a, stream);
+            const bool taken = g_one_ride.taken;
+            g_one_ride.batch = nullptr; g_one_ride.taken = false;
+            if (rc != DMPNN_OK) return rc;
+            if (!taken) { set_error("forward_tiles: the one-launch window was taken but the forward did not reach the tile kernel"); return DMPNN_EINVAL; }
+            g_tiles_launches = g_launches;
+            return DMPNN_OK;
+        }
+    }
     if (tile_row && tile_atom && n_tiles > 0) {
         const dmpnn::PlanLayout L = dmpnn::plan_layout(a->n_atoms, a->n_edges);
         const bool ok = a->n_atoms >= 0 && a->n_edges >= 0 && a->n_atoms < (1ll << 31) && a->n_edges < (1ll << 31) &&
@@ -395,10 +419,12 @@
             DMPNN_TRY(dmpnn_prepare_tiles_from_table(tile_row, tile_atom, n_tiles, a->n_atoms, a->n_edges, plan, plan_bytes, stream));
     } else
         DMPNN_TRY(prepare_tiles_and_bounds(a->edge_index, a->rev_edge_index, batch, a->n_atoms, a->n_edges, plan, plan_bytes, nullptr, 0, stream, nullptr, a, &did_split));
-    if (!did_split) return dmpnn_forward(a, stream);
+    const int planning = g_launches - launches_before;
     dmpnn_fwd_args f = *a;
-    f.flags |= DMPNN_F_WSPLIT_READY;
-    return dmpnn_forward(&f, stream);
+    if (did_split) f.flags |= DMPNN_F_WSPLIT_READY;
+    const int rc = dmpnn_forward(&f, stream);
+    g_tiles_launches = planning + g_launches;
+    return rc;
 }
 
 int dmpnn_forward(const dmpnn_fwd_args* a, void* stream) {
diff --git a/chemprop_amd/csrc/dmpnn_mega16.hip b/chemprop_amd/csrc/dmpnn_mega16.hip
--- a/chemprop_amd/csrc/dmpnn_mega16.hip
+++ b/chemprop_amd/csrc/dmpnn_mega16.hip
@@ -1,4 +1,5 @@
 #include <algorithm>
+#include <atomic>
 #include <cstdlib>
 
 #include "dmpnn_mega16_impl.hpp"
@@ -29,6 +30,7 @@
 
 thread_local long long* g_debug_stamps = nullptr;
 thread_local AggRide g_agg_ride = {nullptr, 0, nullptr, nullptr, 0, 0, 0.f, false};
+thread_local OneRide g_one_ride = {nullptr, false};
 
 namespace {
 inline size_t al256(size_t x) { return (x + 255) & ~size_t(255); }
@@ -98,15 +100,26 @@
     return a.msplit && aligned16(a.msplit) && a.msplit_bytes >= bytes;
 }
 
+int tile_waves_forced() {
+    static const int forced = [] { const char* e = getenv("DMPNN_TILE_WAVES"); return e ? atoi(e) : 0; }();
+    return (forced == 4 || forced == 8) ? forced : 0;
+}
+int device_cu_count() {
+    static std::atomic<int> cached[64] = {};
+    int dev = 0;
+    if (hipGetDevice(&dev) != hipSuccess || dev < 0 || dev >= 64) return 256;
+    int n = cached[dev].load(std::memory_order_relaxed);
+    if (n <= 0) {
+        if (hipDeviceGetAttribute(&n, hipDeviceAttributeMultiprocessorCount, dev) != hipSuccess || n <= 0) n = 256;
+        cached[dev].store(n, std::memory_order_relaxed);
+    }
+    return n;
+}
 int tile_waves(const dmpnn_fwd_args& a, int n_tiles) {
-    static const int forced = [] { const char* e = getenv("DMPNN_TILE_WAVES"); return e ? atoi(e) : 0; }();
-    if (forced == 4 || forced == 8) return forced;
+    const int forced = tile_waves_forced();
+    if (forced) return forced;
     if (a.d_h <= 128 || a.d_h > 320) return 4;
-    static const int n_cu = [] {
-        int dev = 0, n = 0;
-        if (hipGetDevice(&dev) != hipSuccess || hipDeviceGetAttribute(&n, hipDeviceAttributeMultiprocessorCount, dev) != hipSuccess || n <= 0) n = 256;
-        return n;
-    }();
+    const int n_cu = device_cu_count();
     if (n_tiles <= n_cu) return 8;
     const int64_t est = std::max<int64_t>((a.n_edges + 39) / 40, (a.n_atoms + 19) / 20);
     return est + est / 16 <= n_cu ? 8 : 4;
@@ -121,7 +134,7 @@
     }
     unsigned char* ws = static_cast<unsigned char*>(a.wsplit);
     const int N = (int)a.d_h, dv = (int)a.d_v, de = (int)a.d_e;
-    if (!(a.flags & DMPNN_F_WSPLIT_READY)) {
+    if (!(a.flags & DMPNN_F_WSPLIT_READY) && !g_one_ride.batch) {
         mega16::SplitArgs sp;
         if (!mega16_split_args(a, &sp)) { set_error("forward(split16): wsplit workspace missing or too small"); return DMPNN_ENOSPC; }
         hipLaunchKernelGGL(mega16::k_split_weights, dim3((unsigned)(((N + 15) / 16) * 4 * sp.n_jobs)), dim3(256), 0, s, sp);
@@ -182,6 +195,14 @@
     const int n_tiles = (a.n_tiles_launch > 0 && a.n_tiles_launch < L.max_mtiles) ? (int)a.n_tiles_launch : (int)L.max_mtiles;
     const bool sa = !(a.act == DMPNN_ACT_TANH || a.act == DMPNN_ACT_ELU), kp = (a.flags & DMPNN_F_KEEP) != 0;
     const int wn = a.d_h <= 64 ? 1 : (a.d_h <= 128 ? 2 : 5);
+    if (g_one_ride.batch) {
+        if (wn != 5 || kp || (a.flags & (DMPNN_F_STORE16 | DMPNN_F_ATOM)) || tile_waves(a, n_tiles) != 8) {
+            set_error("forward(one launch): outside the window (d_h %lld, flags 0x%x)", (long long)a.d_h, a.flags);
+            return DMPNN_EINVAL;
+        }
+        g_one_ride.taken = true;
+        return launch_forward_one(G, sa, a, g_one_ride.batch, s);
+    }
     if (a.flags & DMPNN_F_STORE16) {
         if (wn == 1) return sa ? mega16::launch_mega16<1, true, false, 4, true>(G, n_tiles, s) : mega16::launch_mega16<1, false, false, 4, true>(G, n_tiles, s);
         if (wn == 2) return sa ? mega16::launch_mega16<2, true, false, 4, true>(G, n_tiles, s) : mega16::launch_mega16<2, false, false, 4, true>(G, n_tiles, s);
diff --git a/chemprop_amd/csrc/dmpnn_mega16_impl.hpp b/chemprop_amd/csrc/dmpnn_mega16_impl.hpp
--- a/chemprop_amd/csrc/dmpnn_mega16_impl.hpp
+++ b/chemprop_amd/csrc/dmpnn_mega16_impl.hpp
@@ -163,8 +163,8 @@
 template <int WN>
 constexpr size_t lds_bytes_atom() { return lds_bytes<WN>() + kAtomLds; }
 
-template <int WN, bool SA, bool KEEP, int NW = 4, bool LP = false>
-__global__ __launch_bounds__(64 * NW, 2) void k_mpnn_tile16(Mega16K G) {
+template <int WN, bool SA, bool KEEP, int NW = 4, bool LP = false, bool ONE = false>
+__device__ __forceinline__ void tile16_forward(const Mega16K& G, const int t_in, const int n_slots) {
     static_assert(!(LP && KEEP), "the hi-halves-alone form is inference only");
     static_assert(NW == 4 || (NW == 8 && WN == 5), "the 8-wave form splits 20 column tiles 3+3+3+3+2+2+2+2");
     const mega::MegaK& g = G.m;
@@ -203,7 +203,7 @@
         ++n_stamp;
     };
     stamp();
-    const int t = blockIdx.x;
+    const int t = ONE ? (t_in < n_slots ? t_in : 0) : t_in;
     int rs = g.mtile_row[t], re = g.mtile_row[t + 1];
     int va = g.mtile_atom[t], vb = g.mtile_atom[t + 1];
     int hdr_light = g.flags[DMPNN_HDR_LIGHT], hdr_flags = g.flags[0], hdr_tiles = g.flags[DMPNN_HDR_NMTILES];
@@ -216,7 +216,7 @@
     const int N = g.h, qn = N >> 2;
     const bool lean = hdr_light == 2;
     const bool poison = (hdr_flags & (lean ? kPlanNoMegaLean : g.poison_mask)) != 0 || (lean && g.nE > 0 && (!g.edge_index || !g.rev64)) ||
-                        hdr_tiles > (int)gridDim.x;
+                        hdr_tiles > n_slots;
     if (poison) {
         const float nanv = __int_as_float(0x7fc00000);
         const long long total = (long long)g.nV * N;
@@ -224,6 +224,7 @@
             g.out[(i / N) * g.ldout + (i % N)] = nanv;
         return;
     }
+    if (ONE && t_in >= n_slots) return;
     if (na <= 0 || nrows < 0 || va < 0 || vb > g.nV || rs < 0 || re > g.nE) return;
     if (nrows > BM || na > BA) {
         if (NW > 4 && threadIdx.x >= kThreads) return;
@@ -818,10 +819,11 @@
 #endif
     if (g.depth > 1 && hdr_tiles >= DMPNN_L2_WARM_MIN_TILES && hdr_tiles <= DMPNN_L2_WARM_MAX_TILES && t < 256) {
         launder();
+        const int tw = ONE ? (int)blockIdx.x : t;
         const unsigned nl = (unsigned)(((N + 15) / 16) * G.Wh.nc * 16);
         const rsrc_t rWh = gemm::make_rsrc(G.Wh.p, nl * 128u), rWo = gemm::make_rsrc(G.WoM.p, nl * 128u);
         const unsigned share = (unsigned)(((hdr_tiles < 256 ? hdr_tiles : 256) + 7) >> 3) * (unsigned)KT;
-        unsigned line = (unsigned)(t >> 3) * (unsigned)KT + (unsigned)tid;
+        unsigned line = (unsigned)(tw >> 3) * (unsigned)KT + (unsigned)tid;
 #pragma unroll
         for (int k = 0; k < 2; ++k, line += share) {
             const unsigned oh = line < nl ? line * 128u : kOOB, oo = (line >= nl && line < 2u * nl) ? (line - nl) * 128u : kOOB;
@@ -1020,6 +1022,11 @@
 }
 
 template <int WN, bool SA, bool KEEP, int NW = 4, bool LP = false>
+__global__ __launch_bounds__(64 * NW, 2) void k_mpnn_tile16(Mega16K G) {
+    tile16_forward<WN, SA, KEEP, NW, LP, false>(G, (int)blockIdx.x, (int)gridDim.x);
+}
+
+template <int WN, bool SA, bool KEEP, int NW = 4, bool LP = false>
 int launch_mega16(const Mega16K& g, int n_tiles, hipStream_t s);
 
 #define DMPNN_DEFINE_MEGA16(WN, SA, KEEP) DMPNN_DEFINE_MEGA16_NW(WN, SA, KEEP, 4)
@@ -1044,4 +1051,11 @@
     }
 
 }
-}
+
+struct OneRide { const int64_t* batch; bool taken; };
+extern thread_local OneRide g_one_ride;
+bool forward_one_launch_window(const dmpnn_fwd_args& a, bool from_batch, bool k0_single, int forced_waves, int n_cu);
+int launch_forward_one(const mega16::Mega16K& G, bool simple_act, const dmpnn_fwd_args& a, const int64_t* batch, hipStream_t s);
+int device_cu_count();
+int tile_waves_forced();
+}
diff --git a/chemprop_amd/csrc/dmpnn_prepare.hip b/chemprop_amd/csrc/dmpnn_prepare.hip
--- a/chemprop_amd/csrc/dmpnn_prepare.hip
+++ b/chemprop_amd/csrc/dmpnn_prepare.hip
@@ -283,7 +283,7 @@
     __syncthreads();
 }
 
-template <class RowOf, class Other>
+template <int NT, class RowOf, class Other>
 __device__ __forceinline__ int pack_pieces(int* __restrict__ plan, const PlanLayout& L, const int* X, int np, RowOf&& row_of,
                                            int* Y, int* bad_s, int* spill_s, int nV, int nE, int tid, Other&& other_work,
                                            long long* dbg, int n_st) {
@@ -294,10 +294,10 @@
     int* mrow = plan + L.mtile_row;
     int* matom = plan + L.mtile_atom;
     const int slots = (int)L.max_mtiles + 2;
-    int nx[kSmallItems];
-#pragma unroll
-    for (int j = 0; j < kSmallItems; ++j) {
-        const int p = tid + kSmallThreads * j;
+    int nx[(kSmallMaxAtoms / NT)];
+#pragma unroll
+    for (int j = 0; j < (kSmallMaxAtoms / NT); ++j) {
+        const int p = tid + NT * j;
         nx[j] = np;
         if (p < np) {
             const int v = X[p], r0 = row_of(p);
@@ -315,8 +315,8 @@
     }
     __syncthreads();
 #pragma unroll
-    for (int j = 0; j < kSmallItems; ++j) {
-        const int p = tid + kSmallThreads * j;
+    for (int j = 0; j < (kSmallMaxAtoms / NT); ++j) {
+        const int p = tid + NT * j;
         if (p <= np) Y[p] = (p < np ? nx[j] : np);
     }
     __syncthreads();
@@ -331,7 +331,7 @@
     const int nblk = (np + 63) >> 6;
     const bool walk = *bad_s == 0;
     if (walk) {
-        for (int blk = wave; blk < nblk; blk += kSmallThreads / 64) {
+        for (int blk = wave; blk < nblk; blk += NT / 64) {
             const int base = blk * 64, p = base + lane;
             const int my_nx = p < np ? Y[p] : np;
             const int lim = (base + 64 < np ? base + 64 : np);
@@ -352,7 +352,7 @@
     stamp();
 #endif
     if (walk) {
-        for (int blk = wave; blk < nblk; blk += kSmallThreads / 64) {
+        for (int blk = wave; blk < nblk; blk += NT / 64) {
             int rank = 0;
             for (int b2 = lane; b2 < blk; b2 += 64) rank += blk_cnt[b2];
             for (int off = 32; off > 0; off >>= 1) rank += __shfl_xor(rank, off);
@@ -374,7 +374,7 @@
 #if defined(DMPNN_K0_STAMPS2)
     stamp();
 #endif
-    other_work(tid, kSmallThreads);
+    other_work(tid, NT);
 #if defined(DMPNN_K0_STAMPS2)
     stamp();
 #endif
@@ -383,10 +383,10 @@
     const int n_tiles = ntile_s;
     const bool bad = *bad_s != 0;
     if (bad) {
-        for (int t = tid; t < slots; t += kSmallThreads) { mrow[t] = nE; matom[t] = nV; }
+        for (int t = tid; t < slots; t += NT) { mrow[t] = nE; matom[t] = nV; }
         return -1;
     }
-    for (int t = n_tiles + tid; t < slots; t += kSmallThreads) { mrow[t] = nE; matom[t] = nV; }
+    for (int t = n_tiles + tid; t < slots; t += NT) { mrow[t] = nE; matom[t] = nV; }
     return n_tiles;
 }
 
@@ -445,7 +445,7 @@
     if (tid == 0) X[np] = nV;
     __syncthreads();
     stamp();
-    return pack_pieces(plan, L, X, np, [&](int p) { return rowp[X[p]]; }, Y, bad_s, spill_s, nV, nE, tid, other_work, dbg, n_st);
+    return pack_pieces<kSmallThreads>(plan, L, X, np, [&](int p) { return rowp[X[p]]; }, Y, bad_s, spill_s, nV, nE, tid, other_work, dbg, n_st);
 }
 
 __global__ __launch_bounds__(kSmallThreads) void k_prepare_small(const int64_t* __restrict__ edge_index,
@@ -656,6 +656,7 @@
 }
 
 
+template <int NT>
 __device__ __forceinline__ void tiles_batch_finish(int* fa, int* fe, int* Y, int nm, int* bad_sp, int* flags_sp, int* spill_sp, int* __restrict__ plan,
                                                    const PlanLayout& L, int nV, int nE, long long* dbg, int n_stamp, int* __restrict__ mol_bounds,
                                                    int n_mols_out);
@@ -736,9 +737,10 @@
     if ((flags_s & (PLAN_NO_PIECE_TILES | PLAN_RANGE_ERROR)) && tid == 0) bad_s = 1;
     __syncthreads();
     stamp();
-    tiles_batch_finish(fa, fe, Y, nm, &bad_s, &flags_s, &spill_s, plan, L, nV, nE, dbg, n_stamp, mol_bounds, n_mols_out);
-}
-
+    tiles_batch_finish<kSmallThreads>(fa, fe, Y, nm, &bad_s, &flags_s, &spill_s, plan, L, nV, nE, dbg, n_stamp, mol_bounds, n_mols_out);
+}
+
+template <int NT>
 __device__ __forceinline__ void tiles_batch_finish(int* fa, int* fe, int* Y, int nm, int* bad_sp, int* flags_sp, int* spill_sp, int* __restrict__ plan,
                                                    const PlanLayout& L, int nV, int nE, long long* dbg, int n_stamp, int* __restrict__ mol_bounds,
                                                    int n_mols_out) {
@@ -749,7 +751,7 @@
     };
     int& bad_s = *bad_sp; int& flags_s = *flags_sp; int& spill_s = *spill_sp;
     if (mol_bounds) {
-        for (int m = tid; m < n_mols_out; m += kSmallThreads) {
+        for (int m = tid; m < n_mols_out; m += NT) {
             mol_bounds[m] = m <= nm ? fa[m] : nV;
             mol_bounds[n_mols_out + m] = m + 1 <= nm ? fa[m + 1] : nV;
             mol_bounds[2 * n_mols_out + 4 + m] = 0;
@@ -760,7 +762,7 @@
     TileGeom g;
     g.b0 = kFusedBM; g.n_tiles = 0;
     auto rest = [&](int i0, int n_thr) { write_tiles(plan, L, fe, nV, nE, g, i0, n_thr); };
-    const int n_mtiles = pack_pieces(plan, L, fa, nm, [&](int p) { return fe[p]; }, Y, &bad_s, &spill_s, nV, nE, tid, rest, dbg ? dbg + 16 : nullptr, 3);
+    const int n_mtiles = pack_pieces<NT>(plan, L, fa, nm, [&](int p) { return fe[p]; }, Y, &bad_s, &spill_s, nV, nE, tid, rest, dbg ? dbg + 16 : nullptr, 3);
     stamp();
     if (tid < DMPNN_HDR_WORDS) {
         int v = 0;
@@ -793,9 +795,9 @@
 constexpr unsigned kBoundsTag = 0x6b30a11du;
 constexpr int kBoundsMaxSpins = 4096;
 struct MultiScratch { int64_t aoff, eoff, done, end; int n_bounds; unsigned tag; };
-static MultiScratch multi_scratch(const PlanLayout& L, int64_t nV, int64_t nE) {
+static MultiScratch multi_scratch(const PlanLayout& L, int64_t nV, int64_t nE, int threads = kSmallThreads) {
     MultiScratch S;
-    S.n_bounds = (int)(((nV > nE ? nV : nE) + 1 + kSmallThreads - 1) / kSmallThreads);
+    S.n_bounds = (int)(((nV > nE ? nV : nE) + 1 + threads - 1) / threads);
     S.tag = 0u;
     int64_t o = (L.src + 1) & ~int64_t(1);
     S.aoff = o; o += align4(2 * (nV + 2));
@@ -810,12 +812,13 @@
     __hip_atomic_store(reinterpret_cast<unsigned long long*>(base) + m, ((unsigned long long)tag << 32) | (unsigned)v, __ATOMIC_RELAXED, __HIP_MEMORY_SCOPE_AGENT);
 }
 
+template <int NT>
 __device__ __forceinline__ void tiles_bounds_block(const int64_t* __restrict__ edge_index, const int64_t* __restrict__ batch, int* __restrict__ plan,
                                                    const MultiScratch& S, int nV, int nE, int b) {
     __shared__ int bad_blk;
     if (threadIdx.x == 0) bad_blk = 0;
     __syncthreads();
-    const int i = b * kSmallThreads + (int)threadIdx.x;
+    const int i = b * NT + (int)threadIdx.x;
     const int64_t last = batch[nV - 1];
     const int n_mols = last < 0 ? 0 : (last >= nV ? nV : (int)last + 1);
     int* aoff = plan + S.aoff;
@@ -852,6 +855,7 @@
                            __ATOMIC_RELAXED, __HIP_MEMORY_SCOPE_AGENT);
 }
 
+template <int NT>
 __device__ __forceinline__ void tiles_pack_block(int* lds_i, const int64_t* __restrict__ batch, int* __restrict__ plan, const PlanLayout& L,
                                                  const MultiScratch& S, int nV, int nE, long long* dbg, int* __restrict__ mol_bounds, int n_mols_out) {
     int n_stamp = 0;
@@ -873,7 +877,7 @@
     {
         unsigned long long* a64 = reinterpret_cast<unsigned long long*>(plan + S.aoff);
         unsigned long long* e64 = reinterpret_cast<unsigned long long*>(plan + S.eoff);
-        for (int m = tid; m <= nm; m += kSmallThreads) {
+        for (int m = tid; m <= nm; m += NT) {
             unsigned long long wa = 0ull, we = 0ull;
             int spins = 0;
             for (;;) {
@@ -896,7 +900,7 @@
     stamp();
     {
         int bad = 0;
-        for (int m = tid; m <= nm; m += kSmallThreads) {
+        for (int m = tid; m <= nm; m += NT) {
             const int a = fa[m], e = fe[m];
             if (a < 0 || a > nV || e < 0 || e > nE) bad = 1;
             if (m > 0 && (fa[m - 1] > a || fe[m - 1] > e)) bad = 1;
@@ -909,7 +913,7 @@
     stamp();
     unsigned long long w_early = 0ull;
     if (tid < S.n_bounds) w_early = __hip_atomic_load(done + tid, __ATOMIC_RELAXED, __HIP_MEMORY_SCOPE_AGENT);
-    tiles_batch_finish(fa, fe, Y, nm, &bad_s, &flags_s, &spill_s, plan, L, nV, nE, dbg, n_stamp, mol_bounds, n_mols_out);
+    tiles_batch_finish<NT>(fa, fe, Y, nm, &bad_s, &flags_s, &spill_s, plan, L, nV, nE, dbg, n_stamp, mol_bounds, n_mols_out);
     __shared__ int late_s;
     if (tid == 0) late_s = 0;
     __syncthreads();
@@ -938,9 +942,9 @@
                                                                             mega16::SplitArgs sp) {
     extern __shared__ __attribute__((aligned(16))) int lds_i[];
     const int b = (int)blockIdx.x;
-    if (b < S.n_bounds) tiles_bounds_block(edge_index, batch, plan, S, nV, nE, b);
+    if (b < S.n_bounds) tiles_bounds_block<kSmallThreads>(edge_index, batch, plan, S, nV, nE, b);
     else if (b + 1 < (int)gridDim.x) mega16::split_weights_wave(sp, (b - S.n_bounds) * (kSmallThreads / 64) + (int)(threadIdx.x >> 6), (int)(threadIdx.x & 63));
-    else tiles_pack_block(lds_i, batch, plan, L, S, nV, nE, dbg, mol_bounds, n_mols_out);
+    else tiles_pack_block<kSmallThreads>(lds_i, batch, plan, L, S, nV, nE, dbg, mol_bounds, n_mols_out);
 }
 
 __global__ __launch_bounds__(256) void k_tiles_from_table_split(const int* __restrict__ tile_row, const int* __restrict__ tile_atom, int n_tiles,
@@ -949,6 +953,159 @@
     else mega16::split_weights_wave(sp, ((int)blockIdx.x - 1) * 4 + (int)(threadIdx.x >> 6), (int)(threadIdx.x & 63));
 }
 
+
+constexpr int kOneThreads = 512;
+constexpr int kOneSplitBlocks = 160;
+constexpr int kOneMaxSpins = 1 << 17;
+struct OneK {
+    mega16::Mega16K G;
+    const int64_t* edge_index; const int64_t* batch; int* plan;
+    PlanLayout L; MultiScratch S; mega16::SplitArgs sp;
+    int64_t sdone, ready;
+    int n_slots;
+    int n_prod;
+    long long* dbg;
+};
+static_assert(sizeof(OneK) <= 4096, "kernel argument block");
+
+__device__ __noinline__ int one_launch_roles(const OneK* kp) {
+    const OneK& K = *kp;
+    extern __shared__ __attribute__((aligned(16))) int lds_i[];
+    __shared__ int one_bad_s, one_seen_s;
+    const int b = (int)blockIdx.x, tid = (int)threadIdx.x, grid = (int)gridDim.x, nb = K.S.n_bounds;
+    const int nV = K.G.m.nV, nE = K.G.m.nE;
+    const unsigned tag = K.S.tag;
+    long long* dbg = (K.dbg && b == 0 && tid == 0) ? K.dbg + 112 : nullptr;
+    if (dbg) dbg[0] = (long long)__builtin_readcyclecounter();
+    unsigned long long* sdone = reinterpret_cast<unsigned long long*>(K.plan + K.sdone);
+    unsigned long long* ready = reinterpret_cast<unsigned long long*>(K.plan + K.ready);
+    if (b == nb) {
+        tiles_pack_block<kOneThreads>(lds_i, K.batch, K.plan, K.L, K.S, nV, nE, K.dbg ? K.dbg + 32 : nullptr, nullptr, 0);
+        if (tid == 0) one_bad_s = 0;
+        __syncthreads();
+        for (int i = tid; i < K.n_prod; i += kOneThreads) {
+            if (i == b) continue;
+            unsigned long long w = 0ull;
+            int spins = 0;
+            for (;;) {
+                w = __hip_atomic_load(sdone + i, __ATOMIC_RELAXED, __HIP_MEMORY_SCOPE_AGENT);
+                if ((unsigned)(w >> 32) == tag || ++spins >= kOneMaxSpins) break;
+                __builtin_amdgcn_s_sleep(8);
+            }
+            if ((unsigned)(w >> 32) != tag) atomicOr(&one_bad_s, 1);
+            __hip_atomic_store(sdone + i, 0ull, __ATOMIC_RELAXED, __HIP_MEMORY_SCOPE_AGENT);
+        }
+        __builtin_amdgcn_fence(__ATOMIC_ACQ_REL, "agent");
+        __syncthreads();
+        const unsigned long long word = ((unsigned long long)tag << 32) | (one_bad_s ? 2u : 1u);
+        for (int i = tid; i < grid; i += kOneThreads) __hip_atomic_store(ready + i, word, __ATOMIC_RELAXED, __HIP_MEMORY_SCOPE_AGENT);
+    } else if (b < K.n_prod) {
+        if (b < nb) tiles_bounds_block<kOneThreads>(K.edge_index, K.batch, K.plan, K.S, nV, nE, b);
+        if (dbg) dbg[1] = (long long)__builtin_readcyclecounter();
+        const int n_split = K.n_prod - 1, si0 = b < nb ? b : b - 1, si = si0 >= nb ? si0 - nb : si0 + (n_split - nb);
+        const int waves = ((K.sp.N + 15) & ~15) * K.sp.n_jobs;
+        for (int w = si * (kOneThreads / 64) + (tid >> 6); w < waves; w += n_split * (kOneThreads / 64)) mega16::split_weights_wave(K.sp, w, tid & 63);
+        __builtin_amdgcn_fence(__ATOMIC_RELEASE, "agent");
+        __syncthreads();
+        if (tid == 0) __hip_atomic_store(sdone + b, ((unsigned long long)tag << 32) | 1u, __ATOMIC_RELAXED, __HIP_MEMORY_SCOPE_AGENT);
+        if (dbg) dbg[2] = (long long)__builtin_readcyclecounter();
+    }
+    if (tid == 0) {
+        unsigned long long w = 0ull;
+        int spins = 0;
+        for (;;) {
+            w = __hip_atomic_load(ready + b, __ATOMIC_RELAXED, __HIP_MEMORY_SCOPE_AGENT);
+            if ((unsigned)(w >> 32) == tag || ++spins >= kOneMaxSpins) break;
+            __builtin_amdgcn_s_sleep(8);
+        }
+        one_seen_s = ((unsigned)(w >> 32) == tag && (unsigned)w == 1u) ? 1 : 0;
+        __hip_atomic_store(ready + b, 0ull, __ATOMIC_RELAXED, __HIP_MEMORY_SCOPE_AGENT);
+    }
+    __syncthreads();
+    __builtin_amdgcn_fence(__ATOMIC_ACQUIRE, "agent");
+    if (dbg) dbg[3] = (long long)__builtin_readcyclecounter();
+    return one_seen_s;
+}
+
+template <bool SA>
+__global__ __launch_bounds__(kOneThreads, 2) void k_forward_one(OneK K) {
+    if (!one_launch_roles(spill::fresh_kernargs<OneK>())) {
+        const float nanv = __int_as_float(0x7fc00000);
+        const long long total = (long long)K.G.m.nV * K.G.m.h;
+        for (long long i = (long long)blockIdx.x * kOneThreads + threadIdx.x; i < total; i += (long long)gridDim.x * kOneThreads)
+            K.G.m.out[(i / K.G.m.h) * K.G.m.ldout + (i % K.G.m.h)] = nanv;
+        return;
+    }
+    const int b = (int)blockIdx.x, nb = K.S.n_bounds;
+    const int t = b < nb ? b : (b == nb ? (int)gridDim.x - 1 : b - 1);
+    mega16::tile16_forward<5, SA, false, 8, false, true>(K.G, t, K.n_slots);
+}
+
+}
+
+static unsigned next_launch_tag() {
+    static std::atomic<unsigned> launch_no{0u};
+    unsigned t = kBoundsTag ^ (0x5a5a0000u + launch_no.fetch_add(1u, std::memory_order_relaxed) * 0x9E3779B1u);
+    return t == 0u ? kBoundsTag : t;
+}
+struct OneGeom { MultiScratch S; int64_t sdone, ready, end; int grid, n_slots, n_prod; };
+static OneGeom one_geom(const PlanLayout& L, int64_t nV, int64_t nE, int64_t n_tiles_launch) {
+    OneGeom g;
+    g.S = multi_scratch(L, nV, nE, kOneThreads);
+    g.n_slots = (int)((n_tiles_launch > 0 && n_tiles_launch < L.max_mtiles) ? n_tiles_launch : L.max_mtiles);
+    g.grid = g.n_slots > g.S.n_bounds + 1 + kOneSplitBlocks ? g.n_slots : g.S.n_bounds + 1 + kOneSplitBlocks;
+    int64_t o = g.S.end;
+    g.n_prod = g.S.n_bounds + 1 + kOneSplitBlocks;
+    g.sdone = o; o += 2 * (int64_t)g.grid;
+    g.ready = o; o += 2 * (int64_t)g.grid;
+    g.end = o;
+    return g;
+}
+bool forward_one_launch_window(const dmpnn_fwd_args& a, bool from_batch, bool k0_single, int forced_waves, int n_cu) {
+    const unsigned need = DMPNN_F_FUSED | DMPNN_F_MEGA | DMPNN_F_SPLIT16;
+    if ((a.flags & need) != need || (a.flags & (DMPNN_F_KEEP | DMPNN_F_ATOM | DMPNN_F_STORE16 | DMPNN_F_WSPLIT_READY))) return false;
+    if (!from_batch || k0_single || a.W_d) return false;
+    const int64_t nV = a.n_atoms, nE = a.n_edges;
+    if (nV <= 0 || nE <= 0 || !small_plan_fits(nV, nE)) return false;
+    if (a.d_h <= 128 || a.d_h > 320 || forced_waves == 4 || n_cu <= 0) return false;
+    const PlanLayout L = plan_layout(nV, nE);
+    const OneGeom g = one_geom(L, nV, nE, a.n_tiles_launch);
+    if (forced_waves != 8 && g.n_slots > n_cu) {
+        const int64_t est = (nE + 39) / 40 > (nV + 19) / 20 ? (nE + 39) / 40 : (nV + 19) / 20;
+        if (est + est / 16 > n_cu) return false;
+    }
+    if (g.S.n_bounds + 1 + kOneSplitBlocks > n_cu) return false;
+    if (g.end > L.tile_row) return false;
+    if ((size_t)(3 * (nV + 2)) * 4 + 32 > mega16::lds_bytes<5>()) return false;
+    return true;
+}
+
+int launch_forward_one(const mega16::Mega16K& G, bool simple_act, const dmpnn_fwd_args& a, const int64_t* batch, hipStream_t s) {
+    const int64_t nV = a.n_atoms, nE = a.n_edges;
+    OneK K;
+    memset(&K, 0, sizeof(K));
+    K.G = G;
+    K.edge_index = a.edge_index; K.batch = batch; K.plan = static_cast<int*>(const_cast<void*>(a.plan));
+    K.L = plan_layout(nV, nE);
+    const OneGeom g = one_geom(K.L, nV, nE, a.n_tiles_launch);
+    K.S = g.S; K.S.tag = next_launch_tag();
+    K.sdone = g.sdone; K.ready = g.ready; K.n_slots = g.n_slots;
+    K.n_prod = g.n_prod;
+    K.dbg = g_debug_stamps;
+    if (!mega16_split_args(a, &K.sp)) { set_error("forward(one launch): wsplit workspace missing or too small"); return DMPNN_ENOSPC; }
+    int dev = 0;
+    if (hipGetDevice(&dev) != hipSuccess || dev < 0 || dev >= 64) { set_error("forward(one launch): no current device"); return DMPNN_EHIP; }
+    static bool attr_set[2][64] = {};
+    const void* fn = simple_act ? reinterpret_cast<const void*>(&k_forward_one<true>) : reinterpret_cast<const void*>(&k_forward_one<false>);
+    if (!attr_set[simple_act ? 1 : 0][dev]) {
+        hipError_t e = hipFuncSetAttribute(fn, hipFuncAttributeMaxDynamicSharedMemorySize, (int)mega16::lds_bytes<5>());
+        if (e != hipSuccess) { set_error("hipFuncSetAttribute(k_forward_one): %s", hipGetErrorString(e)); return DMPNN_EHIP; }
+        attr_set[simple_act ? 1 : 0][dev] = true;
+    }
+    if (simple_act) hipLaunchKernelGGL(k_forward_one<true>, dim3((unsigned)g.grid), dim3(kOneThreads), mega16::lds_bytes<5>(), s, K);
+    else hipLaunchKernelGGL(k_forward_one<false>, dim3((unsigned)g.grid), dim3(kOneThreads), mega16::lds_bytes<5>(), s, K);
+    DMPNN_CHECK_LAUNCH("k_forward_one");
+    return DMPNN_OK;
 }
 
 int launch_tiles_from_table_split(const int* tile_row, const int* tile_atom, int64_t n_tiles, int64_t nV, int64_t nE, int* plan, hipStream_t s,
diff --git a/include/dmpnn.h b/include/dmpnn.h
--- a/include/dmpnn.h
+++ b/include/dmpnn.h
@@ -290,6 +290,8 @@
 void dmpnn_debug_lds_poison(int on);
 const char* dmpnn_last_error_string(void);
 int dmpnn_last_launch_count(void);
+int dmpnn_forward_tiles_launch_count(void);
+int dmpnn_forward_one_launch_window(const dmpnn_fwd_args* a, int from_batch, int k0_single, int forced_tile_waves, int n_cu);
 
 #ifdef __cplusplus
 }
```

Result: slower. 181.7 M edge-updates/s (-60.8%).
